# shoeffner/ann3depth

Hardware: AMD Instinct MI355X
Metric: images/sec (640x480->55x74 MSDN train step) (higher is better)
Workload: dtype f32

## Files before the change

ann3depth_amd/_lib.py:

```python
import collections
import ctypes
import os
from ctypes import c_char_p, c_float, c_int, c_int32, c_int64, c_size_t, c_uint8, c_uint32, c_void_p, POINTER

LIB_PATH = os.environ.get('A3D_LIB') or os.path.join(os.path.dirname(os.path.abspath(__file__)), 'liba3d.so')


class A3dError(RuntimeError):
    pass


class ConvDesc(ctypes.Structure):
    _fields_ = [(n, c_int32) for n in ('n', 'h', 'w', 'c', 'k', 'r', 's', 'stride', 'pad_t', 'pad_l', 'ho', 'wo',
                                       'ldx', 'ldy', 'precision', 'storage', 'hints')]


class SecondOutput(ctypes.Structure):
    _fields_ = [('ptr', c_void_p), ('ld', c_int32), ('step', c_int32), ('offset', c_int32), ('bf16', c_int32), ('cols', c_int32)]


class ExampleView(ctypes.Structure):
    _fields_ = [('image_height', c_int64), ('image_width', c_int64), ('image_channels', c_int64),
                ('depth_height', c_int64), ('depth_width', c_int64), ('depth_channels', c_int64),
                ('image', c_void_p), ('image_bytes', c_size_t), ('depth', c_void_p), ('depth_bytes', c_size_t)]
# ... 26 lines not shown
    'a3d_dense_fwd_ws_bytes': (c_size_t, [c_int, c_int, c_int]),
    'a3d_dense_fwd': (c_int, [c_int, c_int, c_int, _P, _P, _P, _P, c_int, _P, _P, c_size_t, _P]),
    'a3d_dense_bwd_data_ws_bytes': (c_size_t, [c_int, c_int, c_int]),
    'a3d_dense_bwd_data': (c_int, [c_int, c_int, c_int, _P, _P, _P, _P, c_int, c_float, _P, c_size_t, _P]),
    'a3d_dense_bwd_filter_ws_bytes': (c_size_t, [c_int, c_int, c_int]),
    'a3d_dense_bwd_filter': (c_int, [c_int, c_int, c_int, _P, _P, _P, _P, _P, c_size_t, _P]),
    'a3d_maxpool2x2_fwd': (c_int, [c_int, c_int, c_int, c_int, _P, _P, c_int, _P, _P]),
    'a3d_maxpool2x2_bwd': (c_int, [c_int, c_int, c_int, c_int, _P, _P, c_int, _P, c_int, _P]),
    'a3d_resize_bilinear_tf1': (c_int, [c_int, c_int, c_int, c_int, _P, c_int, c_int, _P, _P]),
    'a3d_resize_bilinear_tf1_pair': (c_int, [c_int, c_int, c_int, c_int, _P, c_int, c_int, _P, c_int, _P, c_int, c_int, _P, _P]),
    'a3d_resize_bilinear_tf1_ex': (c_int, [c_int, c_int, c_int, c_int, _P, c_int, c_int, c_int, _P, c_int, _P, c_int, c_int, c_int,
                                           _P, _P]),
    'a3d_warp_bilinear_pair': (c_int, [c_int, c_int, c_int, c_int, _P, c_int, c_int, c_int, _P, c_int, _P, c_int, c_int, c_int,
                                       _P, _P, _P]),
    'a3d_extract_patches': (c_int, [c_int, c_int, c_int, c_int, _P, c_int, c_int, _P, _P]),
    'a3d_silog_loss_fwd': (c_int, [c_int, c_int, _P, _P, _P, _P, _P]),
    'a3d_silog_loss_bwd': (c_int, [c_int, c_int, _P, _P, _P, _P, _P]),
    'a3d_dropout_keep_mask': (c_int, [c_size_t, ctypes.c_uint64, ctypes.c_uint64, c_float, _P, _P]),
    'a3d_adam_apply_tf1': (c_int, [c_size_t, _P, _P, _P, _P, c_float, c_float, c_float, c_float, c_float, c_float,
                                   c_float, _P]),
    'a3d_adam_apply_tf1_flag': (c_int, [c_size_t, _P, _P, _P, _P, c_float, c_float, c_float, c_float, c_float, c_float,
                                        c_float, _P, _P]),
    'a3d_dense_fwd_ex': (c_int, [c_int, c_int, c_int, _P, _P, _P, _P, c_int, _P, c_int, c_int, _P, c_size_t, _P]),
    'a3d_dense_bwd_data_ex': (c_int, [c_int, c_int, c_int, _P, _P, _P, _P, c_int, c_float, c_int, c_int, _P, c_size_t, _P]),
    'a3d_dense_fwd_ex2': (c_int, [c_int, c_int, c_int, _P, _P, _P, _P, c_int, c_int, c_int, _P, c_int, c_int, POINTER(SecondOutput), _P,
                                  c_size_t, _P]),
    'a3d_dense_bwd_data_ex2': (c_int, [c_int, c_int, c_int, _P, _P, _P, _P, c_int, c_float, c_int, c_int, POINTER(SecondOutput), _P,
                                       c_size_t, _P]),
    'a3d_conv2d_fwd_ex2': (c_int, [_D, _P, _P, _P, _P, c_int, POINTER(SecondOutput), _P, c_size_t, _P]),
    'a3d_silog_loss_bwd_ex': (c_int, [c_int, c_int, _P, _P, _P, _P, _P, c_int, _P]),
    'a3d_depth_metrics_ws_bytes': (c_size_t, [c_int, c_int, c_int]),
    'a3d_depth_metrics': (c_int, [c_int, c_int, c_int, _P, c_int, c_int, _P, c_int, c_float, c_float, c_float, c_float, _P, _P,
                                  c_size_t, _P]),
    'a3d_cast_bf16': (c_int, [c_size_t, _P, _P, c_int, _P]),
    'a3d_cast_rows': (c_int, [c_size_t, c_int, _P, c_int, c_int, _P, c_int, c_int, _P]),
    'a3d_pad_channels_bf16': (c_int, [c_size_t, c_int, _P, c_int, _P, _P]),
    'a3d_stream_create': (c_int, [c_int, ctypes.POINTER(ctypes.c_void_p)]),
    'a3d_stream_destroy': (c_int, [_P]),
    'a3d_maxpool2x2_fwd_bf16': (c_int, [c_int, c_int, c_int, c_int, _P, c_int, _P, c_int, _P, _P]),
    'a3d_maxpool2x2_bwd_bf16': (c_int, [c_int, c_int, c_int, c_int, _P, c_int, _P, c_int, _P, c_int, _P]),
    'a3d_copy_channel_bf16': (c_int, [c_size_t, _P, c_int, c_int, _P, c_int, c_int, _P]),
    'a3d_maxpool2x2_bwd_idx_bf16': (c_int, [c_int, c_int, c_int, c_int, _P, _P, c_int, _P, c_int, _P, c_int, _P]),
    'a3d_maxpool2x2_bwd_idx_bf16s': (c_int, [c_int, c_int, c_int, c_int, _P, _P, c_int, _P, c_int, _P, c_int, _P]),
    'a3d_dense_bwd_filter_adam_tf1': (c_int, [c_int, c_int, c_int, _P, _P, _P, _P, _P, _P, _P, _P, c_float, c_float, c_float,
                                              c_float, c_float, c_float, _P]),
    'a3d_dense_bwd_filter_adam_tf1_ex': (c_int, [c_int, c_int, c_int, _P, _P, _P, _P, _P, _P, _P, _P, c_float, c_float, c_float,
                                                 c_float, c_float, c_float, c_int, _P]),
    'a3d_superpixel_mean': (c_int, [c_int, c_int, c_int, c_int, _P, c_int, _P, _P]),
    'a3d_superpixel_hist': (c_int, [c_int, c_int, c_int, _P, c_int, _P, _P]),
    'a3d_pair_similarity': (c_int, [c_int, c_int, c_int, _P, c_int, _P, _P, _P, c_int, _P, _P, c_float, _P, _P, _P]),
    'a3d_crf_loss': (c_int, [c_int, c_int, _P, _P, _P, _P, _P, c_int, c_float, _P, _P, _P, _P]),
    'a3d_crf_map': (c_int, [c_int, c_int, _P, _P, _P, _P, c_int, _P, _P, _P]),
    'a3d_sgd_apply': (c_int, [c_size_t, _P, _P, c_float, _P]),
    'a3d_conv2d_pool_fwd': (c_int, [_D, _P, _P, _P, _P, c_int, _P, c_int, _P, c_size_t, _P]),
    'a3d_maxpool2x2_bwd_idx': (c_int, [c_int, c_int, c_int, c_int, _P, _P, c_int, _P, c_int, _P, c_int, _P]),
    'a3d_copy_channel': (c_int, [c_size_t, _P, c_int, c_int, _P, c_int, c_int, _P]),
    'a3d_comm_standin': (c_int, [_P, c_size_t, _P, c_size_t, c_int, c_float, _P]),
    'a3d_timing_enable': (c_int, [c_int]),
    'a3d_timing_collect': (c_int, [POINTER(TimingRecord), c_int]),
    'a3d_timing_select': (c_int, [POINTER(TimingRecord)]),
    'a3d_crc32c': (c_uint32, [_P, c_size_t]),
    'a3d_masked_crc32c': (c_uint32, [_P, c_size_t]),
    'a3d_tfrecord_next': (c_int, [_P, c_size_t, c_int, POINTER(c_size_t), POINTER(c_size_t), POINTER(c_size_t)]),
    'a3d_example_parse': (c_int, [_P, c_size_t, POINTER(ExampleView)]),
    'a3d_decode_raw_plus_half': (c_int, [_P, c_size_t, _P]),
    'a3d_record_decode': (c_int, [_P, c_size_t, c_int, _P, c_size_t, _P, c_size_t, POINTER(ExampleView)]),
    'a3d_record_decode_u8': (c_int, [_P, c_size_t, c_int, _P, _P, c_size_t, _P, _P, c_size_t, POINTER(ExampleView),
                                     POINTER(c_int)]),
    'a3d_records_decode': (c_int, [POINTER(c_void_p), POINTER(c_size_t), c_int, c_int, POINTER(c_int64), _P, _P, _P, _P,
                                   POINTER(c_int32), c_int, POINTER(c_int32)]),
    'a3d_h2d_gather': (c_int, [_P, _P, POINTER(c_int32), c_int, c_int, c_size_t, _P]),
    'a3d_sizeof_conv_desc': (c_size_t, []),
    'a3d_example_write': (c_int64, [_P, c_int, c_int, c_int, _P, c_int, c_int, c_int, _P, c_size_t]),
}

EXT_SIGNATURES = {
    'a3dx_resize_bilinear_tf1_valid': (c_int, [c_int, c_int, c_int, c_int, _P, c_int, c_int, c_int, _P, c_int, _P, c_int, c_int,
                                               c_int, _P, c_float, c_float, _P]),
    'a3dx_warp_bilinear_pair_valid': (c_int, [c_int, c_int, c_int, c_int, _P, c_int, c_int, c_int, _P, c_int, _P, c_int, c_int,
                                              c_int, _P, _P, c_float, c_float, _P]),
    'a3dx_silog_masked_loss_fwd': (c_int, [c_int, c_int, _P, _P, _P, _P, _P]),
    'a3dx_silog_masked_loss_bwd_ex': (c_int, [c_int, c_int, _P, _P, _P, _P, _P, c_int, _P]),
}

PAIR_SIGNATURES = {
    'a3dp_crf_loss_grad': (c_int, [c_int, c_int, _P, _P, _P, _P, _P, c_int, c_float, _P, _P, _P, _P, _P]),
    'a3dp_pair_dense_bwd': (c_int, [c_int, c_int, c_int, _P, _P, _P, _P, _P]),
    'a3dp_sgd_apply_floor': (c_int, [c_size_t, _P, _P, c_float, c_float, _P]),
}

TEXTURE_SIGNATURES = {
    'a3dt_superpixel_lbp_hist': (c_int, [c_int, c_int, c_int, _P, c_int, _P, _P]),
    'a3dt_pair_similarity3': (c_int, [c_int, c_int, c_int, _P, c_int, _P, _P, _P, _P, c_int, _P, _P, c_float, _P, _P, _P]),
}

GRADLOSS_SIGNATURES = {
    'a3dg_silog_grad_loss_fwd': (c_int, [c_int, c_int, c_int, _P, _P, c_int, c_float, _P, _P, _P]),
    'a3dg_silog_grad_loss_bwd_ex': (c_int, [c_int, c_int, c_int, _P, _P, c_int, c_float, _P, _P, _P, c_int, _P]),
}

BERHU_SIGNATURES = {
    'a3dh_berhu_loss_fwd': (c_int, [c_int, c_int, _P, _P, c_int, c_float, _P, _P, _P]),
    'a3dh_berhu_loss_bwd_ex': (c_int, [c_int, c_int, _P, _P, c_int, c_float, _P, _P, _P, c_int, _P]),
}

ALIGN_SIGNATURES = {
    'a3da_depth_align_ws_bytes': (c_size_t, [c_int, c_int, c_int, c_int]),
    'a3da_depth_align': (c_int, [c_int, c_int, c_int, _P, c_int, c_int, _P, c_int, c_float, c_float, c_int, _P, _P, _P, _P,
                                 c_size_t, _P]),
    'a3da_depth_metrics_aligned': (c_int, [c_int, c_int, c_int, _P, c_int, c_int, _P, c_int, c_float, c_float, c_float, c_float,
                                           _P, _P, _P, c_size_t, _P]),
    'a3da_affine_apply': (c_int, [c_int, c_int, _P, _P, _P, _P]),
}

SSI_SIGNATURES = {
    'a3di_ssi_loss_fwd': (c_int, [c_int, c_int, _P, _P, c_int, _P, _P, _P]),
    'a3di_ssi_loss_bwd_ex': (c_int, [c_int, c_int, _P, _P, c_int, _P, _P, _P, c_int, _P]),
}

CRF_VALID_SIGNATURES = {
    'a3dv_superpixel_mean_valid': (c_int, [c_int, c_int, c_int, _P, c_int, c_int, _P, _P, _P]),
    'a3dv_crf_loss_observed': (c_int, [c_int, c_int, _P, _P, _P, _P, _P, c_int, _P, _P, _P, _P, _P, _P, _P]),
}

FCSP_SIGNATURES = {
    'a3df_superpixel_pool_fwd': (c_int, [c_int, c_int, c_int, c_int, _P, c_int, c_int, c_int, c_int, _P, _P, _P, c_int, _P]),
    'a3df_superpixel_pool_bwd': (c_int, [c_int, c_int, c_int, c_int, _P, c_int, c_int, c_int, c_int, _P, _P, _P, c_int, _P]),
}

CRF_BAND_SIGNATURES = {
    'a3db_crf_band_nll': (c_int, [c_int, c_int, c_int, _P, _P, _P, _P, _P, c_int, _P, _P, _P, _P, _P, _P, _P]),
    'a3db_crf_band_map': (c_int, [c_int, c_int, c_int, _P, _P, _P, _P, c_int, _P, _P, _P]),
}

WINO_SIGNATURES = {
    'a3dw_conv2d_bwd_data_prepared_filter_bytes': (c_size_t, [_D]),
    'a3dw_conv2d_bwd_data_prepare_filter': (c_int, [_D, _P, _P, c_size_t, _P]),
}

WINO_GRAD_SIGNATURES = {
    'a3dwg_conv2d_bwd_filter_ws_bytes': (c_size_t, [_D]),
    'a3dwg_conv2d_bwd_filter': (c_int, [_D, _P, _P, _P, _P, _P, c_size_t, _P]),
}

WINO1D_SIGNATURES = {
    'a3dl_conv2d_bwd_data_ws_bytes': (c_size_t, [_D]),
    'a3dl_conv2d_bwd_data': (c_int, [_D, _P, _P, _P, _P, _P, c_size_t, _P]),
    'a3dl_conv2d_bwd_filter_ws_bytes': (c_size_t, [_D]),
    'a3dl_conv2d_bwd_filter': (c_int, [_D, _P, _P, _P, _P, _P, c_size_t, _P]),
    'a3dl_conv2d_bwd_data_prepared_filter_bytes': (c_size_t, [_D]),
    'a3dl_conv2d_bwd_data_prepare_filter': (c_int, [_D, _P, _P, c_size_t, _P]),
}

OPTIM_SIGNATURES = {
    'a3do_momentum_apply': (c_int, [c_size_t, _P, _P, _P, c_float, c_float, c_float, _P]),
    'a3do_dense_bwd_filter_momentum': (c_int, [c_int, c_int, c_int, _P, _P, _P, _P, _P, _P, c_float, c_float, c_float, _P]),
}

CLIP_SIGNATURES = {
    'a3dn_grad_norm_ws_bytes': (c_size_t, [c_size_t]),
    'a3dn_grad_norm_scale': (c_int, [c_size_t, _P, c_float, c_float, _P, _P, c_size_t, _P]),
    'a3dn_momentum_apply_ctl': (c_int, [c_size_t, _P, _P, _P, c_float, c_float, _P, _P]),
    'a3dn_adam_apply_tf1_ctl': (c_int, [c_size_t, _P, _P, _P, _P, c_float, c_float, c_float, c_float, c_float, c_float, _P, _P,
                                        _P]),
    'a3dn_sgd_apply_ctl': (c_int, [c_size_t, _P, _P, c_float, _P, _P]),
    'a3dn_sgd_apply_floor_ctl': (c_int, [c_size_t, _P, _P, c_float, c_float, _P, _P]),
}
CLIP_CTL_BYTES = 32
CLIP_BLOCK_ELEMS, CLIP_MAX_BLOCKS = 4096, 1024


class WinoBwdPool(ctypes.Structure):
    _fields_ = [('argmax', c_void_p), ('y', c_void_p), ('ldy', c_int), ('h2', c_int), ('w2', c_int)]


WINO_BWD_SIGNATURES = {
    'a3dwb_sizeof_pool': (c_size_t, []),
    'a3dwb_conv2d_bwd_ws_bytes': (c_size_t, [_D, c_int, c_int]),
    'a3dwb_conv2d_bwd': (c_int, [_D, _P, _P, _P, _P, _P, _P, _P, ctypes.POINTER(WinoBwdPool), _P, c_size_t, _P]),
}

UPSAMPLE_SIGNATURES = {
    'a3du_joint_bilateral_upsample': (c_int, [c_int, c_int, c_int, _P, c_int, c_int, _P, c_int, _P, _P, _P, _P, c_int, c_float,
                                              c_float, _P, _P]),
}

POSTERIOR_SIGNATURES = {
    'a3dc_crf_band_posterior': (c_int, [c_int, c_int, c_int, _P, _P, _P, _P, _P, c_int, _P, _P, _P, _P, _P]),
}

SLIC_SIGNATURES = {
    'a3ds_label_mean': (c_int, [c_int, c_int, c_int, c_int, _P, c_int, _P, _P, _P, _P]),
    'a3ds_label_hist': (c_int, [c_int, c_int, c_int, _P, c_int, _P, _P, _P]),
    'a3ds_slic_update': (c_int, [c_int, c_int, c_int, _P, c_int, _P, _P, _P, _P]),
    'a3ds_slic_assign': (c_int, [c_int, c_int, c_int, _P, c_int, _P, c_float, _P, _P]),
    'a3ds_slic_segment': (c_int, [c_int, c_int, c_int, _P, c_int, c_int, c_float, _P, _P, _P, _P]),
    'a3ds_pair_similarity': (c_int, [c_int, c_int, _P, _P, _P, _P, _P, c_int, _P, _P, c_float, _P, _P, _P]),
    'a3ds_label_pool_fwd': (c_int, [c_int, c_int, c_int, c_int, _P, c_int, c_int, c_int, c_int, _P, _P, _P, _P, _P, c_int, _P]),
    'a3ds_label_pool_bwd': (c_int, [c_int, c_int, c_int, c_int, _P, c_int, c_int, c_int, c_int, _P, _P, _P, _P, _P, c_int, _P]),
}

Surface = collections.namedtuple('Surface', 'prefix header signatures')
SURFACES = (
    Surface('a3d_', 'a3d.h', SIGNATURES),
    Surface('a3dx_', 'a3d_valid.h', EXT_SIGNATURES),
    Surface('a3dp_', 'a3d_pairwise.h', PAIR_SIGNATURES),
    Surface('a3dt_', 'a3d_texture.h', TEXTURE_SIGNATURES),
    Surface('a3dg_', 'a3d_gradloss.h', GRADLOSS_SIGNATURES),
    Surface('a3dv_', 'a3d_crf_valid.h', CRF_VALID_SIGNATURES),
    Surface('a3df_', 'a3d_fcsp.h', FCSP_SIGNATURES),
    Surface('a3db_', 'a3d_crf_band.h', CRF_BAND_SIGNATURES),
    Surface('a3dw_', 'a3d_wino.h', WINO_SIGNATURES),
    Surface('a3du_', 'a3d_upsample.h', UPSAMPLE_SIGNATURES),
    Surface('a3dc_', 'a3d_posterior.h', POSTERIOR_SIGNATURES),
    Surface('a3dwg_', 'a3d_wino_grad.h', WINO_GRAD_SIGNATURES),
    Surface('a3ds_', 'a3d_slic.h', SLIC_SIGNATURES),
    Surface('a3dwb_', 'a3d_wino_bwd.h', WINO_BWD_SIGNATURES),
    Surface('a3dh_', 'a3d_berhu.h', BERHU_SIGNATURES),
    Surface('a3da_', 'a3d_align.h', ALIGN_SIGNATURES),
    Surface('a3di_', 'a3d_ssi.h', SSI_SIGNATURES),
    Surface('a3dl_', 'a3d_wino1d.h', WINO1D_SIGNATURES),
    Surface('a3do_', 'a3d_optim.h', OPTIM_SIGNATURES),
    Surface('a3dn_', 'a3d_clip.h', CLIP_SIGNATURES),
)

_lib = None


def load():
    global _lib
    if _lib is not None:
        return _lib
    if not os.path.exists(LIB_PATH):
        raise A3dError(f'{LIB_PATH} not found: build it with `python -c "import __graft_entry__ as g; g.build()"` '
                       f'or `make -C ann3depth_amd/csrc` (there is no fallback path)')
    import torch
    lib = ctypes.CDLL(LIB_PATH)
    for name, (res, args) in ((n, sig) for surface in SURFACES for n, sig in surface.signatures.items()):
        try:
            fn = getattr(lib, name)
        except AttributeError as e:
            raise A3dError(f'liba3d.so lacks symbol {name}: stale build?') from e
        fn.restype = res
        fn.argtypes = args
    if lib.a3d_sizeof_conv_desc() != ctypes.sizeof(ConvDesc):
        raise A3dError(f'liba3d.so reads a {lib.a3d_sizeof_conv_desc()}-byte a3d_conv_desc, this binding passes '
                       f'{ctypes.sizeof(ConvDesc)} bytes: stale build?')
    if lib.a3dwb_sizeof_pool() != ctypes.sizeof(WinoBwdPool):
        raise A3dError(f'liba3d.so reads a {lib.a3dwb_sizeof_pool()}-byte a3dwb_pool, this binding passes '
                       f'{ctypes.sizeof(WinoBwdPool)} bytes: stale build?')
    _lib = lib
    return lib


def last_error():
    buf = ctypes.create_string_buffer(512)
    load().a3d_last_error(buf, 512)
    return buf.value.decode(errors='replace')


def check(rc, what):
    if rc != 0:
        raise A3dError(f'{what} failed ({rc}): {last_error()}')
```

ann3depth_amd/csrc/a3d_internal.h:

```cpp
#pragma once
#include <hip/hip_runtime.h>
#include <stddef.h>
#include <stdint.h>

#include <algorithm>

#include "../../include/a3d.h"
#include "igemm_plan.h"

namespace a3d {

int set_error(int code, const char* fmt, ...);

#define A3D_CHECK_ARG(cond, ...)                                 \
  do {                                                           \
    if (!(cond)) return ::a3d::set_error(A3D_EINVAL, __VA_ARGS__); \
  } while (0)

inline void clear_stale_error() { (void)hipGetLastError(); }

inline int check_launch(const char* what) {
  hipError_t e = hipGetLastError();
  if (e != hipSuccess) return set_error(A3D_ELAUNCH, "%s: %s", what, hipGetErrorString(e));
  return A3D_OK;
}

inline unsigned grid_for(size_t total, int per_block = 256, unsigned cap = 8192) {
  size_t g = (total + per_block - 1) / per_block;
  return (unsigned)std::min<size_t>(std::max<size_t>(g, 1), cap);
}

__host__ __device__ inline bool aligned16(const void* p) { return (reinterpret_cast<uintptr_t>(p) & 15) == 0; }

inline size_t up256(size_t b) { return (b + 255) / 256 * 256; }

inline int raise_lds(const void* kern, size_t bytes, bool (&done)[64]) {
  int dev = 0;
  (void)hipGetDevice(&dev);
  if (dev < 0 || dev >= 64 || !done[dev]) {
    hipError_t e = hipFuncSetAttribute(kern, hipFuncAttributeMaxDynamicSharedMemorySize, (int)bytes);
    if (e != hipSuccess) return set_error(A3D_ELAUNCH, "hipFuncSetAttribute: %s", hipGetErrorString(e));
    if (dev >= 0 && dev < 64) done[dev] = true;
  }
  return A3D_OK;
}

struct IgemmParams;
int launch_igemm(int mode, const GemmPlan& plan, int avec, int bvec, IgemmParams& p, void* ws, hipStream_t st);
int take_second_output(IgemmParams& p, const a3d_second_output* o);

struct TimingSlot {
  hipEvent_t start, stop;
  a3d_timing_record rec;
};
bool timing_wanted(const a3d_timing_record& r);
int timing_begin(TimingSlot& slot, hipStream_t st);
void timing_end(TimingSlot& slot, hipStream_t st);
a3d_timing_record timing_record(int mode, int prec, int bm, int bn, int waves_m, int nwaves, int bk, int avec, int bvec, int lds_dma,
                                int m, int n, int k);
template <typename Launch>
int timed_launch(const a3d_timing_record& rec, hipStream_t st, Launch&& launch) {
  if (!timing_wanted(rec)) return launch();
  TimingSlot slot{};
  slot.rec = rec;
  int rc = timing_begin(slot, st);
  if (rc != A3D_OK) return rc;
  rc = launch();
  timing_end(slot, st);
  return rc;
}

bool dense_dw_applicable(int m, int k, int n);
bool dense_stream_applicable(int m, int k, int n);
size_t dense_stream_ws_bytes(int m, int k, int n);
int dense_fwd_stream(int m, int k, int n, const float* x, const float* w, const float* bias, float* y, int act,
                     const uint8_t* keep, float keep_scale, void* ws, size_t ws_bytes, hipStream_t st);
struct ReduceParams;
int launch_splitk_reduce(const ReduceParams& r, hipStream_t st);
int dense_dw_launch(int m, int k, int n, const float* x, const float* dz, float* dw, float* db, hipStream_t st);

size_t colsum_bf16_ws_bytes(int n);
bool colsum_bf16_ok(int n);
int colsum_bf16(const void* dz, int rows, int n, int ld, float* out, void* ws, int* nparts, hipStream_t st);

bool stencil1_applicable(const a3d_conv_desc* d);
size_t stencil1_bwdf_ws_bytes(const a3d_conv_desc* d);
int stencil1_fwd(const a3d_conv_desc* d, const float* x, const float* w, const float* bias, float* y, int act,
                 hipStream_t st);
int stencil1_bwd_filter(const a3d_conv_desc* d, const float* x, const float* dz, float* dw, float* db, void* ws,
                        hipStream_t st);
bool stencil1_bwd_both_applicable(const a3d_conv_desc* d);
size_t stencil1_bwd_both_ws_bytes(const a3d_conv_desc* d);
int stencil1_bwd_both(const a3d_conv_desc* d, const float* x, const float* dz, const float* w, float* dw, float* db,
                      void* dx, int lddx, int dx_bf16, int relu_mask, unsigned* state, void* ws, hipStream_t st);

bool fewch_bwdf_applicable(const a3d_conv_desc* d, bool pooled);
size_t fewch_bwdf_ws_bytes(const a3d_conv_desc* d, bool pooled);
bool fewch_extents_ok(const a3d_conv_desc* d, bool pooled, int ldz, int esz, int ld_arg);
int fewch_bwd_filter(const a3d_conv_desc* d, const float* x, int src, const void* dz, int ldz, const void* pooled_act,
                     const uint8_t* argmax, int ld_arg, float* dw, float* db, void* ws, hipStream_t st);

int fewch_reduce_launch(const float* slabs, int splits, int Mp, int NP, int M, int N, float* dw, float* db, hipStream_t st);
bool fewch16_bwdf_applicable(const a3d_conv_desc* d, bool pooled);
size_t fewch16_bwdf_ws_bytes(const a3d_conv_desc* d, bool pooled);
int fewch16_bwd_filter(const a3d_conv_desc* d, const float* x, bool pooled, const void* dz, int ldz, const void* pooled_act,
                       const uint8_t* argmax, int ld_arg, float* dw, float* db, void* ws, hipStream_t st);

bool conv3_applicable(const a3d_conv_desc* d, unsigned x_off);
size_t conv3_ws_bytes(const a3d_conv_desc* d);
int conv3_pack(const a3d_conv_desc* d, const float* w, float* wp, hipStream_t st);
int conv3_fwd(const a3d_conv_desc* d, const float* x, const float* w, const float* bias, float* y, int act, int pool,
              int ld_out, uint8_t* argmax, void* ws, size_t ws_bytes, hipStream_t st, bool prepared = false);

bool conv3b_applicable(const a3d_conv_desc* d);
size_t conv3b_filter_bytes(const a3d_conv_desc* d);
int conv3b_pack(const a3d_conv_desc* d, const float* w, void* wp, hipStream_t st);
int conv3b_fwd(const a3d_conv_desc* d, const void* x, const float* w, const float* bias, void* y, int act, int pool, int ld_out,
               uint8_t* argmax, void* ws, size_t ws_bytes, hipStream_t st, bool prepared);

struct PlaneBatch;
constexpr int kBM = 128, kBN = 128, kWavesM = 4, kNWaves = 8, kBK = 32;
constexpr int kBlockSlots = 512, kCUs = 256, kMinKTiles = 5;
void plane_tiles(IgemmParams& p, int splits);
int plane_gemm(int mode, int bn, const IgemmParams& p, const PlaneBatch& bt, unsigned blocks, int planes, const char* what, hipStream_t st);
int plane_splits(int planes, int M, int N, size_t pixels, bool larger_on_tie, const char* tuning);

struct WinoGeom {
  int oh, ow, th, tw;
  size_t T;
  int K, N, Kp, Np;
  size_t v_bytes, m_bytes, u_bytes;
  size_t sk_bytes;
};
WinoGeom wino_geom(const a3d_conv_desc* d, bool bwd);
bool wino_applicable(const a3d_conv_desc* d);
int wino_filter(const a3d_conv_desc* d, bool bwd, const float* w, float* U, hipStream_t st);
int wino_input(const a3d_conv_desc* d, bool bwd, const float* src, float* V, hipStream_t st);
int wino_output(const a3d_conv_desc* d, bool bwd, const float* M, float* out, const float* bias, const float* mask, int act,
                hipStream_t st);
a3d_timing_record wino_record(int mode, const WinoGeom& g);
int wino_gemm(IgemmParams& p, const WinoGeom& g, hipStream_t st);

struct WinoGradGeom {
  size_t T;
  int Cp, Kp;
  int splits;
  size_t v_bytes, z_bytes;
  size_t slab_bytes, bias_bytes;
};
int wino_grad_splits(int C, int K, size_t T);
WinoGradGeom wino_grad_geom(const a3d_conv_desc* d);
bool wino_grad_applicable(const a3d_conv_desc* d);
int wino_dz(const a3d_conv_desc* d, const float* dz, float* Z, hipStream_t st);
int wino_dw(const a3d_conv_desc* d, const WinoGradGeom& g, const float* slabs, const float* bparts, float* dw, float* db, hipStream_t st);
a3d_timing_record wino_grad_record(const a3d_conv_desc* d, const WinoGradGeom& g);
int wino_grad_gemm(IgemmParams& p, const WinoGradGeom& g, hipStream_t st);

struct WinoBwdPool {
  const uint8_t* argmax;
  const float* y;
  int ldy, h2, w2;
};
int wino_bwd_transforms(const a3d_conv_desc* d, const float* x, const float* dz, float* Vx, float* Vdz, float* Z, hipStream_t st);
int wino_bwd_gemm(IgemmParams& pf, const WinoGradGeom& gg, IgemmParams& pd, const WinoGeom& g, hipStream_t st);
int wino_bwd_finish(const a3d_conv_desc* d, const WinoGradGeom& gg, const float* slabs, const float* bparts, float* dw, float* db,
                    const float* M, float* dx, const float* mask, const WinoBwdPool* pool, hipStream_t st);

struct Wino1dGeom {
  int R, tw, off;
  size_t Pv, Pm;
  int K, N, Kp, Np;
  int bn, tiles_m, tiles_n, nk, blocks;
  size_t v_bytes, m_bytes, u_bytes;
  size_t sk_bytes;
};
struct Wino1dGradGeom {
  int R, tw;
  size_t Px, Pz;
  int Cp, Kp, splits;
  size_t v_bytes, z_bytes;
  size_t slab_bytes, bias_bytes;
};
int wino1d_bwd_blocks(long tiles, long nk);
int wino1d_grad_splits(int M, int N, size_t pixels);
Wino1dGeom wino1d_geom(const a3d_conv_desc* d);
Wino1dGradGeom wino1d_grad_geom(const a3d_conv_desc* d);
bool wino1d_applicable(const a3d_conv_desc* d);
int wino1d_filter(const a3d_conv_desc* d, const float* w, float* U, hipStream_t st);
int wino1d_input(const float* src, float* V, size_t rows, int W, int c, int ld, int off, int tw, int Cp, hipStream_t st);
int wino1d_dz(const a3d_conv_desc* d, const Wino1dGradGeom& g, const float* dz, float* Z, hipStream_t st);
int wino1d_output(const a3d_conv_desc* d, const Wino1dGeom& g, const float* M, float* dx, const float* mask, hipStream_t st);
int wino1d_dw(const a3d_conv_desc* d, const Wino1dGradGeom& g, const float* slabs, const float* bparts, float* dw, float* db, hipStream_t st);
a3d_timing_record wino1d_record(const Wino1dGeom& g);
a3d_timing_record wino1d_grad_record(const a3d_conv_desc* d, const Wino1dGradGeom& g);
int wino1d_gemm(IgemmParams& p, const Wino1dGeom& g, float* sk, hipStream_t st);
int wino1d_grad_gemm(IgemmParams& p, const Wino1dGradGeom& g, hipStream_t st);

struct Carve {
  uintptr_t at;
  float* take(size_t bytes) {
    float* p = reinterpret_cast<float*>(at);
    at += bytes;
    return p;
  }
};
struct ProductWs { float *U, *V, *M, *sk; };
struct GradWs { float *V, *Z, *slabs, *bparts; };
template <typename Geom>
ProductWs carve_product(Carve& c, const Geom& g, bool prepared) {
  ProductWs w{};
  if (!prepared) w.U = c.take(g.u_bytes);
  w.V = c.take(g.v_bytes);
  w.M = c.take(g.m_bytes);
  w.sk = c.take(g.sk_bytes);
  return w;
}
template <typename Geom>
GradWs carve_grad(Carve& c, const Geom& g) {
  GradWs w{};
  w.V = c.take(g.v_bytes);
  w.Z = c.take(g.z_bytes);
  w.slabs = c.take(g.slab_bytes);
  w.bparts = c.take(g.bias_bytes);
  return w;
}

}
```

ann3depth_amd/csrc/igemm_host.hip:

```cpp
#include <algorithm>
#include <cmath>

#include "../../include/a3d_wino.h"
#include "../../include/a3d_wino_grad.h"
#include "../../include/a3d_wino_bwd.h"
#include "../../include/a3d_wino1d.h"
#include "a3d_internal.h"
#include "igemm.h"
#include "igemm_cfgs.h"

namespace a3d {

int launch_igemm_multi_bwd_d(int avec, int bvec, IgemmMulti& ps, unsigned grid_x, unsigned count, hipStream_t st);
int launch_igemm_bf16_multi_bwd_d(int bn, IgemmMulti& ps, unsigned grid_x, unsigned count, hipStream_t st);


struct RunForm {
  int vec;
  int rl, rlp;
  int kp;
  int np;
  size_t bytes;
};
static bool run_form_ok(const a3d_conv_desc* d, unsigned x_off, RunForm* rf, bool bwd_filter = false) {
  if (d->pad_t || d->pad_l || d->ldx != d->c || d->c % 4 == 0 || d->c > 4) return false;
  const int step = d->stride * d->c, row = d->w * d->c;
  int vec = 0;
  bool anywhere = false;
  if (step % 4 == 0 && row % 4 == 0 && x_off == 0) vec = 4;
  else if (step % 2 == 0 && row % 2 == 0 && (x_off & 7) == 0) vec = 2;
  else if (bwd_filter && d->precision == A3D_PREC_F32 && !d->storage && (x_off & 3) == 0) {
    vec = 2;
    anywhere = true;
  }
  if (vec == 4 && d->precision == A3D_PREC_F32) {
    const int rl = d->s * d->c;
    const int kp4 = d->r * ((rl + 3) / 4 * 4), kp2 = d->r * ((rl + 1) / 2 * 2);
    if ((kp2 + 127) / 128 < (kp4 + 127) / 128) vec = 2;
  }
  if (!vec) return false;
  rf->vec = vec;
  rf->rl = d->s * d->c;
  rf->rlp = (rf->rl + vec - 1) / vec * vec;
  rf->kp = d->r * rf->rlp;
  rf->np = (d->k + 3) / 4 * 4;
  rf->bytes = up256((size_t)rf->kp * rf->np * 4);
  if (anywhere) return (d->wo - 1) * step + rf->rl <= row && (d->ho - 1) * d->stride + d->r <= d->h;
  return (d->wo - 1) * step + rf->rlp <= row;
}

__global__ __launch_bounds__(256) void pad_filter_kernel(const float* w, float* wp, int r, int rl, int rlp, int n, int np) {
  const int total = r * rlp * np;
  for (int i = blockIdx.x * 256 + threadIdx.x; i < total; i += gridDim.x * 256) {
    const int col = i % np, row = i / np;
    const int q = row % rlp, rr = row / rlp;
    wp[i] = (q < rl && col < n) ? w[(size_t)(rr * rl + q) * n + col] : 0.f;
  }
}
__global__ __launch_bounds__(256) void unpad_filter_kernel(const float* wp, float* w, int r, int rl, int rlp, int n) {
  const int total = r * rl * n;
  for (int i = blockIdx.x * 256 + threadIdx.x; i < total; i += gridDim.x * 256) {
    const int col = i % n, row = i / n;
    const int q = row % rl, rr = row / rl;
    w[i] = wp[(size_t)(rr * rlp + q) * n + col];
  }
}

struct Operands {
  bool known = false;
  unsigned x = 0, w = 0, y = 0;
  unsigned aux = 0;
  int act = A3D_ACT_NONE, pool = 0, ld_out = 0;
  bool argmax = false, prepared = false;
  bool db = true;
};
static const Operands kOnGrid{};
static Operands launch_operands(const void* x, const void* w, const void* y, const void* aux) {
  auto off16 = [](const void* p) { return (unsigned)(reinterpret_cast<uintptr_t>(p) & 15); };
  Operands o;
  o.known = true;
  o.x = off16(x); o.w = off16(w); o.y = off16(y); o.aux = off16(aux);
  return o;
}

enum GemmForm { kAsStored, kLdsDma, kRunForm, kBf16Image };
struct Route {
  bool ok = false;
  RunForm rf{};
  GemmProblem g{};
  GemmPlan plan{};
  size_t repack = 0;
  size_t bytes = 0;
};
static size_t upto(size_t need, const Route& r) { return r.ok ? std::max(need, r.bytes) : need; }
static void fit_workspace(Route& r, const Operands& o, size_t ws_bytes, size_t per_split = 0) {
  if (r.bytes <= ws_bytes || !(o.x | o.w | o.y | o.aux) || r.repack > ws_bytes) return;
  r.plan = plan_within(r.g, r.plan, ws_bytes - r.repack, per_split);
  r.bytes = r.repack + r.plan.ws_bytes + (r.plan.splitk > 1 ? (size_t)r.plan.splitk * per_split : 0);
}
#define A3D_CHECK_WS(ws, who) A3D_CHECK_ARG(aligned16(ws), who ": ws must be 16-byte aligned")

static const int kAll16 = A3D_STORE_X_BF16 | A3D_STORE_W_BF16 | A3D_STORE_Y_BF16;
static bool stored16(const a3d_conv_desc* d, int bits) { return (d->storage & bits) == bits; }
static bool ring_ok(const a3d_conv_desc* d, const Operands& o, int both, unsigned out_off, int taps) {
  if (d->precision != A3D_PREC_BF16 || !stored16(d, both) || d->c % 8 || d->k % 8) return false;
  return !o.known || (d->ldx % 8 == 0 && d->ldy % 8 == 0 && taps <= 128 && !out_off);
}

static int ilog2_exact(int v) {
  for (int l = 0; l < 8; ++l)
    if ((1 << l) == v) return l;
  return -1;
}

static int check_desc(const a3d_conv_desc* d) {
  A3D_CHECK_ARG(d != nullptr, "conv: null descriptor");
  A3D_CHECK_ARG(d->n > 0 && d->h > 0 && d->w > 0 && d->c > 0 && d->k > 0 && d->r > 0 && d->s > 0, "conv: bad dims");
  A3D_CHECK_ARG(ilog2_exact(d->stride) >= 0 && d->stride <= 4, "conv: stride %d unsupported (1, 2 or 4)", d->stride);
  A3D_CHECK_ARG(d->pad_t >= 0 && d->pad_l >= 0 && d->pad_t < d->r && d->pad_l < d->s, "conv: bad padding");
  A3D_CHECK_ARG(d->ho > 0 && d->wo > 0, "conv: bad output size");
  A3D_CHECK_ARG((d->ho - 1) * d->stride - d->pad_t < d->h && (d->wo - 1) * d->stride - d->pad_l < d->w,
                "conv: output size inconsistent with input");
  A3D_CHECK_ARG(d->ldx >= d->c && d->ldy >= d->k, "conv: pixel strides smaller than channel counts");
  A3D_CHECK_ARG(d->precision >= A3D_PREC_F32 && d->precision <= A3D_PREC_F32_WINOGRAD, "conv: unknown precision %d", d->precision);
  const double lim = 2147483647.0;
  A3D_CHECK_ARG((double)d->n * d->h * d->w * d->ldx < lim && (double)d->n * d->ho * d->wo * d->ldy < lim &&
                    (double)d->r * d->s * d->c * d->k < lim,
                "conv: tensor too large for 31-bit indexing");
  auto tile_span_ok = [&](double rows_per_image, double image_elems) {
    const double images = std::min((double)d->n, std::floor(255.0 / rows_per_image) + 2.0);
    return images * image_elems * 4.0 < lim;
  };
  A3D_CHECK_ARG(tile_span_ok((double)d->ho * d->wo, (double)d->h * d->w * d->ldx) &&
                    tile_span_ok(std::max(1.0, std::floor((double)d->h / d->stride) * std::floor((double)d->w / d->stride)),
                                 (double)d->ho * d->wo * d->ldy),
                "conv: single images too large for 31-bit byte offsets inside a tile");
  return A3D_OK;
}

#define A3D_AS_F32(d)                                          \
  a3d_conv_desc d##_f32;                                       \
  if ((d) && (d)->precision == A3D_PREC_F32_WINOGRAD) {        \
    d##_f32 = *(d);                                            \
    d##_f32.precision = A3D_PREC_F32;                          \
    (d) = &d##_f32;                                            \
  }

static GemmProblem fwd_problem(const a3d_conv_desc* d) {
  GemmProblem g;
  g.mode = MODE_FWD;
  g.M = d->n * d->ho * d->wo; g.N = d->k; g.K = d->r * d->s * d->c;
  g.avec = (d->c % 4 == 0 && d->ldx % 4 == 0) ? 4 : 1;
  g.bvec = (d->k % 4 == 0) ? 4 : 1;
  return g;
}
static GemmProblem bwd_d_problem(const a3d_conv_desc* d) {
  GemmProblem g;
  g.mode = MODE_BWD_D;
  g.M = d->n * d->h * d->w; g.N = d->c; g.K = d->r * d->s * d->k;
// ... 723 lines not shown
  if (rc != A3D_OK) return rc;
  IgemmParams p = wino_grad_product(g, at.V, at.Z, at.slabs, db ? at.bparts : nullptr);
  rc = timed_launch(wino_grad_record(d, g), st, [&] { return wino_grad_gemm(p, g, st); });
  if (rc != A3D_OK) return rc;
  return wino_dw(d, g, at.slabs, at.bparts, dw, db, st);
}

static bool wino_bwd_takes(const a3d_conv_desc* d) {
  if (!wino_grad_takes(d)) return false;
  const WinoGeom gx = wino_geom(d, false), gd = wino_geom(d, true);
  return gx.th <= gd.th && gx.tw <= gd.tw;
}
static a3d_conv_desc as_winograd(const a3d_conv_desc* d) {
  a3d_conv_desc e = *d;
  e.precision = A3D_PREC_F32_WINOGRAD;
  return e;
}

size_t a3dwb_sizeof_pool(void) { return sizeof(a3dwb_pool); }

size_t a3dwb_conv2d_bwd_ws_bytes(const a3d_conv_desc* d, int w_prepared, int pooled) {
  (void)pooled;
  if (!wino_bwd_takes(d)) return std::max(a3dwg_conv2d_bwd_filter_ws_bytes(d), a3d_conv2d_bwd_data_ws_bytes(d));
  const a3d_conv_desc e = as_winograd(d);
  Carve c{0};
  carve_product(c, wino_geom(&e, true), w_prepared != 0);
  carve_grad(c, wino_grad_geom(&e));
  return c.at;
}

int a3dwb_conv2d_bwd(const a3d_conv_desc* d, const float* x, const float* dz, const float* w_or_U, float* dw, float* db, float* dx,
                     const float* relu_mask, const a3dwb_pool* pool, void* ws, size_t ws_bytes, void* stream) {
  static_assert(sizeof(WinoBwdPool) == sizeof(a3dwb_pool), "WinoBwdPool mirrors a3dwb_pool");
  if (!wino_bwd_takes(d)) {
    A3D_CHECK_ARG(!pool, "conv2d_bwd (Winograd): a pool only where the Winograd routes take the descriptor");
    const int rc = a3dwg_conv2d_bwd_filter(d, x, dz, dw, db, ws, ws_bytes, stream);
    return rc != A3D_OK ? rc : a3d_conv2d_bwd_data(d, dz, w_or_U, dx, relu_mask, ws, ws_bytes, stream);
  }
  A3D_CHECK_ARG(x && dz && w_or_U && dw && dx, "conv2d_bwd (Winograd): null tensor");
  A3D_CHECK_WS(ws, "conv2d_bwd (Winograd)");
  A3D_CHECK_ARG(!(pool && relu_mask), "conv2d_bwd (Winograd): relu_mask and pool exclude each other");
  A3D_CHECK_ARG(!pool || (pool->argmax && pool->y && pool->ldy >= d->c && pool->h2 >= 2 && pool->w2 >= 2 && pool->h2 / 2 == d->h &&
                          pool->w2 / 2 == d->w),
                "conv2d_bwd (Winograd): the pool's halved extents must be the layer's input's");
  const a3d_conv_desc e = as_winograd(d);
  const bool prepared = (d->hints & A3D_HINT_W_PREPARED) != 0;
  const WinoGeom g = wino_geom(&e, true);
  const WinoGradGeom gg = wino_grad_geom(&e);
  Carve c{reinterpret_cast<uintptr_t>(ws)};
  const ProductWs ad = carve_product(c, g, prepared);
  const GradWs af = carve_grad(c, gg);
  const size_t need = c.at - reinterpret_cast<uintptr_t>(ws);
  if (!ws || need > ws_bytes) return set_error(A3D_EWORKSPACE, "conv2d_bwd (Winograd): need %zu workspace bytes", need);
  hipStream_t st = static_cast<hipStream_t>(stream);
  const float* U;
  int rc = transformed_filter("conv2d_bwd (Winograd)", prepared, w_or_U, ad.U, U, [&](float* u) { return wino_filter(&e, true, w_or_U, u, st); });
  if (rc != A3D_OK) return rc;
  rc = wino_bwd_transforms(&e, x, dz, af.V, ad.V, af.Z, st);
  if (rc != A3D_OK) return rc;
  IgemmParams pf = wino_grad_product(gg, af.V, af.Z, af.slabs, db ? af.bparts : nullptr);
  IgemmParams pd = wino_product(g, ad.V, U, ad.M);
  const a3d_timing_record rf = wino_grad_record(&e, gg), rd = wino_record(MODE_BWD_D, g);
  if (timing_wanted(rf) || timing_wanted(rd) || tune_int("A3D_WINO_BWD_PAIR", 1) == 0) {
    rc = timed_launch(rf, st, [&] { return wino_grad_gemm(pf, gg, st); });
    if (rc != A3D_OK) return rc;
    rc = timed_launch(rd, st, [&] { return wino_gemm(pd, g, st); });
  } else {
    rc = wino_bwd_gemm(pf, gg, pd, g, st);
  }
  if (rc != A3D_OK) return rc;
  WinoBwdPool wp{};
  if (pool) wp = WinoBwdPool{pool->argmax, pool->y, pool->ldy, pool->h2, pool->w2};
  return wino_bwd_finish(&e, gg, af.slabs, af.bparts, dw, db, ad.M, dx, relu_mask, pool ? &wp : nullptr, st);
}

static bool wino1d_takes(const a3d_conv_desc* d) { return check_desc(d) == A3D_OK && wino1d_applicable(d); }

static IgemmParams wino1d_product(const a3d_conv_desc* d, const Wino1dGeom& g, const float* V, const float* U, float* M) {
  return plane_product(MODE_FWD, plane_desc(d->n, d->ho, g.tw, d->h, g.Kp, g.Np, g.R, g.R - 1 - d->pad_t), V, U, M, nullptr,
                       (unsigned long long)g.Pv * g.Kp, (unsigned long long)g.R * g.Kp * g.Np, g.R);
}
static IgemmParams wino1d_grad_product(const a3d_conv_desc* d, const Wino1dGradGeom& g, const float* V, const float* Z, float* slabs,
                                       float* bparts) {
  return plane_product(MODE_BWD_F, plane_desc(d->n, d->h, g.tw, d->ho, g.Cp, g.Kp, g.R, d->pad_t), V, Z, slabs, bparts,
                       (unsigned long long)g.Px * g.Cp, (unsigned long long)g.Pz * g.Kp, g.R);
}

size_t a3dl_conv2d_bwd_data_ws_bytes(const a3d_conv_desc* d) {
  if (!wino1d_takes(d)) return a3d_conv2d_bwd_data_ws_bytes(d);
  return product_ws_bytes(wino1d_geom(d), (d->hints & A3D_HINT_W_PREPARED) != 0);
}

int a3dl_conv2d_bwd_data(const a3d_conv_desc* d, const float* dz, const float* w, float* dx, const float* relu_mask, void* ws,
                         size_t ws_bytes, void* stream) {
  if (!wino1d_takes(d)) return a3d_conv2d_bwd_data(d, dz, w, dx, relu_mask, ws, ws_bytes, stream);
  A3D_CHECK_ARG(dz && w && dx, "conv2d_bwd_data (Winograd 1-D): null tensor");
  A3D_CHECK_WS(ws, "conv2d_bwd_data (Winograd 1-D)");
  const bool prepared = (d->hints & A3D_HINT_W_PREPARED) != 0;
  const Wino1dGeom g = wino1d_geom(d);
  Carve c{reinterpret_cast<uintptr_t>(ws)};
  const ProductWs at = carve_product(c, g, prepared);
  const size_t need = c.at - reinterpret_cast<uintptr_t>(ws);
  if (!ws || need > ws_bytes) return set_error(A3D_EWORKSPACE, "conv2d_bwd_data (Winograd 1-D): need %zu workspace bytes", need);
  hipStream_t st = static_cast<hipStream_t>(stream);
  const float* U;
  int rc = transformed_filter("conv2d_bwd_data (Winograd 1-D)", prepared, w, at.U, U, [&](float* u) { return wino1d_filter(d, w, u, st); });
  if (rc != A3D_OK) return rc;
  rc = wino1d_input(dz, at.V, (size_t)d->n * d->ho, d->wo, d->k, d->ldy, g.off, g.tw, g.Kp, st);
  if (rc != A3D_OK) return rc;
  IgemmParams p = wino1d_product(d, g, at.V, U, at.M);
  rc = timed_launch(wino1d_record(g), st, [&] { return wino1d_gemm(p, g, at.sk, st); });
  if (rc != A3D_OK) return rc;
  return wino1d_output(d, g, at.M, dx, relu_mask, st);
}

size_t a3dl_conv2d_bwd_filter_ws_bytes(const a3d_conv_desc* d) {
  if (!wino1d_takes(d)) return a3d_conv2d_bwd_filter_ws_bytes(d);
  return grad_ws_bytes(wino1d_grad_geom(d));
}

int a3dl_conv2d_bwd_filter(const a3d_conv_desc* d, const float* x, const float* dz, float* dw, float* db, void* ws, size_t ws_bytes,
                           void* stream) {
  if (!wino1d_takes(d)) return a3d_conv2d_bwd_filter(d, x, dz, dw, db, ws, ws_bytes, stream);
  A3D_CHECK_ARG(x && dz && dw, "conv2d_bwd_filter (Winograd 1-D): null tensor");
  A3D_CHECK_WS(ws, "conv2d_bwd_filter (Winograd 1-D)");
  const Wino1dGradGeom g = wino1d_grad_geom(d);
  Carve c{reinterpret_cast<uintptr_t>(ws)};
  const GradWs at = carve_grad(c, g);
  const size_t need = c.at - reinterpret_cast<uintptr_t>(ws);
  if (!ws || need > ws_bytes) return set_error(A3D_EWORKSPACE, "conv2d_bwd_filter (Winograd 1-D): need %zu workspace bytes", need);
  hipStream_t st = static_cast<hipStream_t>(stream);
  int rc = wino1d_input(x, at.V, (size_t)d->n * d->h, d->w, d->c, d->ldx, d->pad_l, g.tw, g.Cp, st);
  if (rc != A3D_OK) return rc;
  rc = wino1d_dz(d, g, dz, at.Z, st);
  if (rc != A3D_OK) return rc;
  IgemmParams p = wino1d_grad_product(d, g, at.V, at.Z, at.slabs, db ? at.bparts : nullptr);
  rc = timed_launch(wino1d_grad_record(d, g), st, [&] { return wino1d_grad_gemm(p, g, st); });
  if (rc != A3D_OK) return rc;
  return wino1d_dw(d, g, at.slabs, at.bparts, dw, db, st);
}

size_t a3dl_conv2d_bwd_data_prepared_filter_bytes(const a3d_conv_desc* d) { return wino1d_takes(d) ? wino1d_geom(d).u_bytes : 0; }

int a3dl_conv2d_bwd_data_prepare_filter(const a3d_conv_desc* d, const float* w, void* prepared, size_t prepared_bytes, void* stream) {
  int rc = check_desc(d);
  if (rc != A3D_OK) return rc;
  A3D_CHECK_ARG(w && prepared && aligned16(prepared), "conv2d_bwd_data_prepare_filter (Winograd 1-D): null or misaligned buffer");
  const size_t need = a3dl_conv2d_bwd_data_prepared_filter_bytes(d);
  A3D_CHECK_ARG(need > 0, "conv2d_bwd_data_prepare_filter (Winograd 1-D): the route does not take this descriptor");
  if (prepared_bytes < need) return set_error(A3D_EWORKSPACE, "conv2d_bwd_data_prepare_filter (Winograd 1-D): need %zu bytes", need);
  return wino1d_filter(d, w, static_cast<float*>(prepared), static_cast<hipStream_t>(stream));
}

static a3d_conv_desc dense_desc(int m, int k, int n) {
  a3d_conv_desc d{};
  d.n = m; d.h = 1; d.w = 1; d.c = k; d.k = n; d.r = 1; d.s = 1; d.stride = 1; d.ho = 1; d.wo = 1;
  d.ldx = k; d.ldy = n;
  return d;
}

size_t a3d_dense_fwd_ws_bytes(int m, int k, int n) {
  a3d_conv_desc d = dense_desc(m, k, n);
  if (check_desc(&d) != A3D_OK) return 0;
  return std::max(plan_gemm(fwd_problem(&d), A3D_PREC_F32).ws_bytes, dense_stream_ws_bytes(m, k, n));
}

int a3d_dense_fwd(int m, int k, int n, const float* x, const float* w, const float* bias, float* y, int act,
                  const uint8_t* drop_keep, void* ws, size_t ws_bytes, void* stream) {
  return a3d_dense_fwd_ex(m, k, n, x, w, bias, y, act, drop_keep, A3D_PREC_F32, 0, ws, ws_bytes, stream);
}

int a3d_dense_fwd_ex(int m, int k, int n, const float* x, const float* w, const float* bias, float* y, int act,
                     const uint8_t* drop_keep, int precision, int storage, void* ws, size_t ws_bytes, void* stream) {
  return a3d_dense_fwd_ex2(m, k, n, x, w, bias, y, n, n, act, drop_keep, precision, storage, nullptr, ws, ws_bytes, stream);
}

int a3d_dense_fwd_ex2(int m, int k, int n, const float* x, const float* w, const float* bias, float* y, int ldy, int ncols_y, int act,
                      const uint8_t* drop_keep, int precision, int storage, const a3d_second_output* out2, void* ws,
                      size_t ws_bytes, void* stream) {
  A3D_CHECK_ARG(m > 0 && k > 0 && n > 0, "dense_fwd: bad dims");
  A3D_CHECK_ARG(ncols_y > 0 && ncols_y <= n && ldy >= ncols_y, "dense_fwd: y rows of %d columns at pitch %d from a GEMM of %d", ncols_y, ldy, n);
  A3D_CHECK_ARG((storage & ~(A3D_STORE_W_BF16 | A3D_STORE_X_BF16)) == 0, "dense_fwd: the weights and x may be bf16, y is float32");
  if (precision == A3D_PREC_F32_WINOGRAD) precision = A3D_PREC_F32;
  a3d_conv_desc d = dense_desc(m, k, n);
  d.precision = precision;
  int rc = check_desc(&d);
  if (rc != A3D_OK) return rc;
  A3D_CHECK_ARG(x && w && y, "dense_fwd: null tensor");
  A3D_CHECK_WS(ws, "dense_fwd");
  if (precision == A3D_PREC_F32 && !storage && dense_stream_applicable(m, k, n) && aligned16(x) && !out2 && ldy == n && ncols_y == n &&
      !tune_int("A3D_NO_DENSE_KERNELS", 0))
    return dense_fwd_stream(m, k, n, x, w, bias, y, act, drop_keep, 2.f, ws, ws_bytes, static_cast<hipStream_t>(stream));
  GemmProblem g = fwd_problem(&d);
  if (!aligned16(x)) g.avec = 1;
  if (!aligned16(w)) g.bvec = 1;
  IgemmParams p;
  fill_common(p, g);
  rc = apply_storage(p, precision, storage & A3D_STORE_X_BF16, storage & A3D_STORE_W_BF16, false, k, k, n, n, x, w, y, "x", "w", "y");
  if (rc != A3D_OK) return rc;
  A3D_CHECK_ARG(!p.a16 || aligned16(y), "dense_fwd: beside a bf16 x, y must be 16-byte aligned (the LDS-DMA kernel alone reads a bf16 x)");
  storage_vecs(g, p.a16, p.b16, p.c16);
  g.ring_ok = p.a16 && p.b16 && precision == A3D_PREC_BF16 && k % 8 == 0 && n % 8 == 0 && aligned16(y) && act != A3D_ACT_SIGMOID;
  g.need_reduce = ncols_y != n;
  GemmPlan plan = plan_gemm(g, precision);
  if (!aligned16(x) || !aligned16(w) || !aligned16(y)) plan = plan_within(g, plan, ws ? ws_bytes : 0, 0);
  A3D_CHECK_ARG(!storage || plan.prec == A3D_PREC_BF16, "dense_fwd: bf16 weights need vectorisable operands");
  A3D_CHECK_ARG(!p.a16 || plan.ring, "dense_fwd: a bf16 x is taken by the LDS-DMA kernel only (bf16 weights, k and n multiples of 8)");
  if (plan.ws_bytes > ws_bytes) return set_error(A3D_EWORKSPACE, "dense_fwd: need %zu workspace bytes", plan.ws_bytes);
  p.A = x; p.B = w; p.C = y; p.bias = bias; p.act = act; p.keep = drop_keep; p.mask_scale = 2.f;
  p.npix = m; p.nrsc = k;
  fill_gather(p, &d, k, 1, k);
  p.ldb = n; p.ldc = ldy; p.c_cols = ncols_y == n ? 0 : ncols_y;
  rc = take_second_output(p, out2);
  if (rc != A3D_OK) return rc;
  fill_staging(p, MODE_FWD, (unsigned long long)m * k, (unsigned long long)k * n, 1, 1);
  return launch_igemm(MODE_FWD, plan, g.avec, g.bvec, p, ws, static_cast<hipStream_t>(stream));
}

size_t a3d_dense_bwd_data_ws_bytes(int m, int k, int n) {
  a3d_conv_desc d = dense_desc(m, k, n);
  return a3d_conv2d_bwd_data_ws_bytes(&d);
}

int a3d_dense_bwd_data(int m, int k, int n, const float* dz, const float* w, float* dx, const float* mask,
                       int mask_act, float scale, void* ws, size_t ws_bytes, void* stream) {
  return a3d_dense_bwd_data_ex(m, k, n, dz, w, dx, mask, mask_act, scale, A3D_PREC_F32, 0, ws, ws_bytes, stream);
}

int a3d_dense_bwd_data_ex(int m, int k, int n, const float* dz, const float* w, float* dx, const float* mask, int mask_act,
                          float scale, int precision, int storage, void* ws, size_t ws_bytes, void* stream) {
  return a3d_dense_bwd_data_ex2(m, k, n, dz, w, dx, mask, mask_act, scale, precision, storage, nullptr, ws, ws_bytes, stream);
}

int a3d_dense_bwd_data_ex2(int m, int k, int n, const float* dz, const float* w, float* dx, const float* mask, int mask_act,
                           float scale, int precision, int storage, const a3d_second_output* out2, void* ws, size_t ws_bytes,
                           void* stream) {
  A3D_CHECK_ARG(m > 0 && k > 0 && n > 0, "dense_bwd_data: bad dims");
  if (precision == A3D_PREC_F32_WINOGRAD) precision = A3D_PREC_F32;
  A3D_CHECK_ARG(precision >= A3D_PREC_F32 && precision <= A3D_PREC_BF16, "dense_bwd_data: unknown precision %d", precision);
  A3D_CHECK_ARG(!mask || mask_act == A3D_ACT_RELU || mask_act == A3D_ACT_SIGMOID, "dense_bwd_data: bad mask_act");
  a3d_conv_desc d = dense_desc(m, k, n);
  int rc = check_desc(&d);
  if (rc != A3D_OK) return rc;
  A3D_CHECK_ARG(dz && w && dx, "dense_bwd_data: null tensor");
  A3D_CHECK_WS(ws, "dense_bwd_data");
  GemmProblem g = bwd_d_problem(&d);
  if (!aligned16(dz)) g.avec = 1;
  if (!aligned16(w)) g.bvec = 1;
  IgemmParams p;
  fill_common(p, g);
  rc = apply_storage(p, precision, storage & A3D_STORE_Y_BF16, storage & A3D_STORE_W_BF16, storage & A3D_STORE_X_BF16, n, n, n, n, dz, w,
                     dx, "dz", "w", "dx");
  if (rc != A3D_OK) return rc;
  A3D_CHECK_ARG(!p.c16 || aligned16(mask), "dense_bwd_data: bf16 mask must be 16-byte aligned");
  storage_vecs(g, p.a16, p.b16, p.c16);
  g.ring_ok = p.a16 && p.b16 && precision == A3D_PREC_BF16 && k % 8 == 0 && n % 8 == 0 && aligned16(dx) &&
              (!mask || (aligned16(mask) && mask_act == A3D_ACT_RELU));
  GemmPlan plan = plan_gemm(g, precision);
  if (!aligned16(dz) || !aligned16(w) || !aligned16(dx) || !aligned16(mask)) plan = plan_within(g, plan, ws ? ws_bytes : 0, 0);
  A3D_CHECK_ARG(!storage || plan.prec == A3D_PREC_BF16, "dense_bwd_data: bf16 weights need vectorisable operands");
  A3D_CHECK_ARG(!(p.a16 || p.c16) || plan.ring, "dense_bwd_data: bf16 dz / dx are taken by the LDS-DMA kernel only (bf16 weights, k and n multiples of 8, ReLU mask)");
  if (plan.ws_bytes > ws_bytes) return set_error(A3D_EWORKSPACE, "dense_bwd_data: need %zu workspace bytes", plan.ws_bytes);
  p.A = dz; p.B = w; p.C = dx; p.mask = mask; p.mask_scale = scale; p.mask_act = mask_act;
  p.npix = m; p.nrsc = n;
  fill_gather(p, &d, n, 1, n);
  p.Cn = k;
  p.ldc = k;
  p.S_full = 1;
  rc = take_second_output(p, out2);
  if (rc != A3D_OK) return rc;
  fill_staging(p, MODE_BWD_D, (unsigned long long)m * n, (unsigned long long)k * n, 1, 1);
  return launch_igemm(MODE_BWD_D, plan, g.avec, g.bvec, p, ws, static_cast<hipStream_t>(stream));
}

size_t a3d_dense_bwd_filter_ws_bytes(int m, int k, int n) {
  a3d_conv_desc d = dense_desc(m, k, n);
  return a3d_conv2d_bwd_filter_ws_bytes(&d);
}

int a3d_dense_bwd_filter(int m, int k, int n, const float* x, const float* dz, float* dw, float* db, void* ws,
                         size_t ws_bytes, void* stream) {
  A3D_CHECK_ARG(m > 0 && k > 0 && n > 0, "dense_bwd_filter: bad dims");
  A3D_CHECK_WS(ws, "dense_bwd_filter");
  if (dense_dw_applicable(m, k, n) && (long)k * n >= (1L << 16) && !tune_int("A3D_NO_DENSE_KERNELS", 0)) {
    A3D_CHECK_ARG(x && dz && dw, "dense_bwd_filter: null tensor");
    return dense_dw_launch(m, k, n, x, dz, dw, db, static_cast<hipStream_t>(stream));
  }
  a3d_conv_desc d = dense_desc(m, k, n);
  return a3d_conv2d_bwd_filter(&d, x, dz, dw, db, ws, ws_bytes, stream);
}

}
```

ann3depth_amd/csrc/wino.hip:

```cpp
#include "a3d_internal.h"
#include "igemm.h"
#include "igemm_cfgs.h"

namespace a3d {

typedef float f4 __attribute__((ext_vector_type(4)));

__global__ __launch_bounds__(256) void wino_filter_kernel(const float* w, float* U, int c, int k, int Rp, int Cp, int bwd) {
  const int total = Rp * Cp;
  for (int i = blockIdx.x * 256 + threadIdx.x; i < total; i += gridDim.x * 256) {
    const int col = i % Cp, row = i / Cp;
    const int rows = bwd ? k : c, cols = bwd ? c : k;
    float g[3][3];
#pragma unroll
    for (int r = 0; r < 3; ++r)
#pragma unroll
      for (int s = 0; s < 3; ++s) {
        float v = 0.f;
        if (row < rows && col < cols)
          v = bwd ? w[((size_t)((2 - r) * 3 + (2 - s)) * c + col) * k + row] : w[((size_t)(r * 3 + s) * c + row) * k + col];
        g[r][s] = v;
      }
    float t[4][3];
#pragma unroll
    for (int s = 0; s < 3; ++s) {
      const float a = g[0][s] + g[2][s];
      t[0][s] = g[0][s];
      t[1][s] = (a + g[1][s]) * 0.5f;
      t[2][s] = (a - g[1][s]) * 0.5f;
      t[3][s] = g[2][s];
    }
#pragma unroll
    for (int a4 = 0; a4 < 4; ++a4) {
      const float a = t[a4][0] + t[a4][2];
      const float u[4] = {t[a4][0], (a + t[a4][1]) * 0.5f, (a - t[a4][1]) * 0.5f, t[a4][2]};
#pragma unroll
      for (int b4 = 0; b4 < 4; ++b4) U[(size_t)(a4 * 4 + b4) * total + i] = u[b4];
    }
  }
}


template <bool VEC>
__device__ __forceinline__ void wino_load_window(const float* __restrict__ x, f4 (&d)[4][4], size_t img, int y0, int x0, int h, int w, int c,
                                                 int ld, int cq) {
#pragma unroll
  for (int a = 0; a < 4; ++a)
#pragma unroll
    for (int b = 0; b < 4; ++b) {
      f4 v = f4(0.f);
      const int yy = y0 + a, xx = x0 + b;
      if (yy >= 0 && yy < h && xx >= 0 && xx < w) {
        const float* src = x + ((img * h + yy) * w + xx) * (size_t)ld + cq * 4;
        if (VEC) {
          v = *reinterpret_cast<const f4*>(src);
        } else {
#pragma unroll
          for (int e = 0; e < 4; ++e)
            if (cq * 4 + e < c) v[e] = src[e];
        }
      }
      d[a][b] = v;
    }
}

__device__ __forceinline__ void wino_input_store(const f4 (&d)[4][4], float* __restrict__ V, size_t T, size_t t, int Cp, int cq) {
  f4 r[4][4];
#pragma unroll
  for (int b = 0; b < 4; ++b) {
    r[0][b] = d[0][b] - d[2][b];
    r[1][b] = d[1][b] + d[2][b];
    r[2][b] = d[2][b] - d[1][b];
    r[3][b] = d[1][b] - d[3][b];
  }
#pragma unroll
  for (int a = 0; a < 4; ++a) {
    const f4 v[4] = {r[a][0] - r[a][2], r[a][1] + r[a][2], r[a][2] - r[a][1], r[a][1] - r[a][3]};
#pragma unroll
    for (int b = 0; b < 4; ++b) *reinterpret_cast<f4*>(V + ((size_t)(a * 4 + b) * T + t) * Cp + cq * 4) = v[b];
  }
}

template <bool VEC>
__global__ __launch_bounds__(256) void wino_input_kernel(const float* __restrict__ x, float* __restrict__ V, int h, int w, int c, int ld,
                                                         int th, int tw, int pad_t, int pad_l, int Cp, size_t T) {
  const int cqn = Cp / 4;
  const size_t total = T * (size_t)cqn;
  for (size_t i = (size_t)blockIdx.x * 256 + threadIdx.x; i < total; i += (size_t)gridDim.x * 256) {
    const int cq = (int)(i % cqn);
    const size_t t = i / cqn;
    const int tj = (int)(t % tw), ti = (int)((t / tw) % th);
    const size_t img = t / ((size_t)tw * th);
    f4 d[4][4];
    wino_load_window<VEC>(x, d, img, 2 * ti - pad_t, 2 * tj - pad_l, h, w, c, ld, cq);
    wino_input_store(d, V, T, t, Cp, cq);
  }
}

__device__ __forceinline__ void wino_output_rows(const float* __restrict__ M, f4 (&r)[2][4], size_t T, size_t t, int Np, int cq) {
  f4 m[4][4];
#pragma unroll
  for (int a = 0; a < 4; ++a)
#pragma unroll
    for (int b = 0; b < 4; ++b) m[a][b] = *reinterpret_cast<const f4*>(M + ((size_t)(a * 4 + b) * T + t) * Np + cq * 4);
#pragma unroll
  for (int b = 0; b < 4; ++b) {
    r[0][b] = (m[0][b] + m[1][b]) + m[2][b];
    r[1][b] = (m[1][b] - m[2][b]) - m[3][b];
  }
}

template <bool VEC>
__global__ __launch_bounds__(256) void wino_output_kernel(const float* __restrict__ M, float* __restrict__ out, const float* __restrict__ bias,
                                                          const float* __restrict__ mask, int act, int oh, int ow, int ncols, int ld,
                                                          int th, int tw, int Np, size_t T) {
  const int cqn = Np / 4;
  const size_t total = T * (size_t)cqn;
  for (size_t i = (size_t)blockIdx.x * 256 + threadIdx.x; i < total; i += (size_t)gridDim.x * 256) {
    const int cq = (int)(i % cqn);
    const size_t t = i / cqn;
    const int tj = (int)(t % tw), ti = (int)((t / tw) % th);
    const size_t img = t / ((size_t)tw * th);
    f4 r[2][4];
    wino_output_rows(M, r, T, t, Np, cq);
    f4 bv = f4(0.f);
    if (bias) {
#pragma unroll
      for (int e = 0; e < 4; ++e)
        if (cq * 4 + e < ncols) bv[e] = bias[cq * 4 + e];
    }
#pragma unroll
    for (int a = 0; a < 2; ++a) {
      const f4 y2[2] = {(r[a][0] + r[a][1]) + r[a][2], (r[a][1] - r[a][2]) - r[a][3]};
#pragma unroll
      for (int b = 0; b < 2; ++b) {
        const int oy = 2 * ti + a, ox = 2 * tj + b;
        if (oy >= oh || ox >= ow) continue;
        const size_t o = ((img * oh + oy) * ow + ox) * (size_t)ld + cq * 4;
        f4 v = y2[b] + bv;
        if (act == EPI_RELU) {
#pragma unroll
          for (int e = 0; e < 4; ++e) v[e] = fmaxf(v[e], 0.f);
        } else if (act == EPI_SIGMOID) {
#pragma unroll
          for (int e = 0; e < 4; ++e) v[e] = 1.f / (1.f + expf(-v[e]));
        }
        if (VEC) {
          if (mask) {
            const f4 y = *reinterpret_cast<const f4*>(mask + o);
#pragma unroll
            for (int e = 0; e < 4; ++e) v[e] = apply_act_grad(v[e], y[e], EPI_RELU, 1.f);
          }
          *reinterpret_cast<f4*>(out + o) = v;
        } else {
#pragma unroll
          for (int e = 0; e < 4; ++e)
            if (cq * 4 + e < ncols) out[o + e] = mask ? apply_act_grad(v[e], mask[o + e], EPI_RELU, 1.f) : v[e];
        }
      }
    }
  }
}

template <int MODE, int BN, int WAVES_M, int NWAVES>
__global__ __launch_bounds__(64 * NWAVES, 2 * NWAVES / 4) void plane_gemm_kernel(const IgemmParams p, const PlaneBatch bt) {
  igemm_body<MODE, kBM, BN, WAVES_M, NWAVES, kBK, 4, 4>(plane_params(p, bt, blockIdx.y), gridDim.x, blockIdx.x);
}

template <int MODE, int BN, int WAVES_M, int NWAVES>
static int plane_gemm_as(const IgemmParams& p, const PlaneBatch& bt, unsigned blocks, int planes, const char* what, hipStream_t st) {
  using Cfg = IgemmCfg<MODE, kBM, BN, WAVES_M, NWAVES, kBK, 4, 4>;
  static bool attr_done[64] = {};
  const int rc = raise_lds(reinterpret_cast<const void*>(plane_gemm_kernel<MODE, BN, WAVES_M, NWAVES>), Cfg::LDS_BYTES, attr_done);
  if (rc != A3D_OK) return rc;
  clear_stale_error();
  hipLaunchKernelGGL((plane_gemm_kernel<MODE, BN, WAVES_M, NWAVES>), dim3(blocks, (unsigned)planes), dim3(Cfg::NT), Cfg::LDS_BYTES, st, p, bt);
  return check_launch(what);
}

int plane_gemm(int mode, int bn, const IgemmParams& p, const PlaneBatch& bt, unsigned blocks, int planes, const char* what, hipStream_t st) {
  if (mode == MODE_BWD_F) return plane_gemm_as<MODE_BWD_F, kBN, kWavesM, kNWaves>(p, bt, blocks, planes, what, st);
  if (bn == 96) return plane_gemm_as<MODE_FWD, 96, 4, 4>(p, bt, blocks, planes, what, st);
  return plane_gemm_as<MODE_FWD, kBN, kWavesM, kNWaves>(p, bt, blocks, planes, what, st);
}

void plane_tiles(IgemmParams& p, int splits) {
  const int nk = (p.K + kBK - 1) / kBK;
  p.splitk = splits;
  p.ktiles_per_split = (nk + splits - 1) / splits;
  p.tiles_m = (p.M + kBM - 1) / kBM;
  p.tiles_n = (p.N + kBN - 1) / kBN;
  p.slab = (size_t)p.M * p.N;
}

int plane_splits(int planes, int M, int N, size_t pixels, bool larger_on_tie, const char* tuning) {
  const long blocks1 = (long)planes * ((M + kBM - 1) / kBM) * ((N + kBN - 1) / kBN);
  const long nk = (long)((pixels + kBK - 1) / kBK);
  const long smax = std::max(1L, std::min(kBlockSlots / blocks1, nk / kMinKTiles));
  long s = 1, load = (blocks1 + kCUs - 1) / kCUs;
  for (long t = 2; t <= smax; ++t) {
    const long l = (blocks1 * t + kCUs - 1) / kCUs;
    if (l * s < load * t || (larger_on_tie && l * s == load * t)) { s = t; load = l; }
  }
  const int forced = tune_int(tuning, 0);
  if (forced > 0) s = std::min((long)forced, nk);
  const long per = (nk + s - 1) / s;
  return (int)((nk + per - 1) / per);
}

constexpr int kWinoPlanes = 16;
static PlaneBatch wino_batch(const WinoGeom& g) { return {g.T * (size_t)g.Kp, (size_t)g.Kp * g.Np, g.T * (size_t)g.Np, 0, -1}; }
static PlaneBatch wino_grad_batch(const WinoGradGeom& g) {
  return {g.T * (size_t)g.Cp, g.T * (size_t)g.Kp, (size_t)g.splits * g.Cp * g.Kp, 0, 1 * 4 + 1};
}

WinoGeom wino_geom(const a3d_conv_desc* d, bool bwd) {
  WinoGeom g{};
  g.oh = bwd ? d->h : d->ho;
  g.ow = bwd ? d->w : d->wo;
  g.th = (g.oh + 1) / 2;
  g.tw = (g.ow + 1) / 2;
  g.T = (size_t)d->n * g.th * g.tw;
  g.K = bwd ? d->k : d->c;
  g.N = bwd ? d->c : d->k;
  g.Kp = (g.K + 3) / 4 * 4;
  g.Np = (g.N + 3) / 4 * 4;
  g.v_bytes = up256((size_t)16 * g.T * g.Kp * 4);
  g.m_bytes = up256((size_t)16 * g.T * g.Np * 4);
  g.u_bytes = up256((size_t)16 * g.Kp * g.Np * 4);
  return g;
}

bool wino_applicable(const a3d_conv_desc* d) {
  if (d->precision != A3D_PREC_F32_WINOGRAD || d->storage || d->r != 3 || d->s != 3 || d->stride != 1 || d->pad_t > 1 || d->pad_l > 1)
    return false;
  for (bool bwd : {false, true}) {
    const WinoGeom g = wino_geom(d, bwd);
    if ((double)g.T * std::max(g.Kp, g.Np) * 4.0 >= 2147483647.0 || g.T >= ((size_t)1 << 30)) return false;
  }
  return true;
}

int wino_filter(const a3d_conv_desc* d, bool bwd, const float* w, float* U, hipStream_t st) {
  const WinoGeom g = wino_geom(d, bwd);
  clear_stale_error();
  hipLaunchKernelGGL(wino_filter_kernel, dim3(grid_for((size_t)g.Kp * g.Np)), dim3(256), 0, st, w, U, d->c, d->k, g.Kp, g.Np, bwd ? 1 : 0);
  return check_launch("wino_filter");
}

int wino_input(const a3d_conv_desc* d, bool bwd, const float* src, float* V, hipStream_t st) {
  const WinoGeom g = wino_geom(d, bwd);
  const int h = bwd ? d->ho : d->h, w = bwd ? d->wo : d->w, ld = bwd ? d->ldy : d->ldx;
  const int pad_t = bwd ? 2 - d->pad_t : d->pad_t, pad_l = bwd ? 2 - d->pad_l : d->pad_l;
  const bool vec = g.K % 4 == 0 && ld % 4 == 0 && aligned16(src);
  const dim3 grid(grid_for(g.T * (size_t)(g.Kp / 4), 256, 1u << 20)), block(256);
  clear_stale_error();
  if (vec) hipLaunchKernelGGL(wino_input_kernel<true>, grid, block, 0, st, src, V, h, w, g.K, ld, g.th, g.tw, pad_t, pad_l, g.Kp, g.T);
  else hipLaunchKernelGGL(wino_input_kernel<false>, grid, block, 0, st, src, V, h, w, g.K, ld, g.th, g.tw, pad_t, pad_l, g.Kp, g.T);
  return check_launch("wino_input");
}

int wino_output(const a3d_conv_desc* d, bool bwd, const float* M, float* out, const float* bias, const float* mask, int act,
                hipStream_t st) {
  const WinoGeom g = wino_geom(d, bwd);
  const int ld = bwd ? d->ldx : d->ldy;
  const bool vec = g.N % 4 == 0 && ld % 4 == 0 && aligned16(out) && aligned16(mask);
  const dim3 grid(grid_for(g.T * (size_t)(g.Np / 4), 256, 1u << 20)), block(256);
  clear_stale_error();
  if (vec) hipLaunchKernelGGL(wino_output_kernel<true>, grid, block, 0, st, M, out, bias, mask, act, g.oh, g.ow, g.N, ld, g.th, g.tw, g.Np, g.T);
  else hipLaunchKernelGGL(wino_output_kernel<false>, grid, block, 0, st, M, out, bias, mask, act, g.oh, g.ow, g.N, ld, g.th, g.tw, g.Np, g.T);
  return check_launch("wino_output");
}

a3d_timing_record wino_record(int mode, const WinoGeom& g) {
  return timing_record(mode, A3D_PREC_F32, kBM, kBN, kWavesM, kNWaves, kBK, 4, 4, 0, (int)(16 * g.T), g.N, g.K);
}

int wino_gemm(IgemmParams& p, const WinoGeom& g, hipStream_t st) {
  plane_tiles(p, 1);
  return plane_gemm(MODE_FWD, kBN, p, wino_batch(g), (unsigned)(p.tiles_m * p.tiles_n), kWinoPlanes, "wino_gemm", st);
}



__device__ __forceinline__ void wino_dz_store(const f4 (&y)[2][2], float* __restrict__ Z, size_t T, size_t t, int Kp, int cq) {
  const f4 r[4][2] = {{y[0][0], y[0][1]}, {y[0][0] + y[1][0], y[0][1] + y[1][1]}, {y[0][0] - y[1][0], y[0][1] - y[1][1]},
                      {-y[1][0], -y[1][1]}};
#pragma unroll
  for (int a = 0; a < 4; ++a) {
    const f4 z[4] = {r[a][0], r[a][0] + r[a][1], r[a][0] - r[a][1], -r[a][1]};
#pragma unroll
    for (int b = 0; b < 4; ++b) *reinterpret_cast<f4*>(Z + ((size_t)(a * 4 + b) * T + t) * Kp + cq * 4) = z[b];
  }
}

template <bool VEC>
__global__ __launch_bounds__(256) void wino_dz_kernel(const float* __restrict__ dz, float* __restrict__ Z, int ho, int wo, int k, int ld,
                                                      int th, int tw, int Kp, size_t T) {
  const int cqn = Kp / 4;
  const size_t total = T * (size_t)cqn;
  for (size_t i = (size_t)blockIdx.x * 256 + threadIdx.x; i < total; i += (size_t)gridDim.x * 256) {
    const int cq = (int)(i % cqn);
    const size_t t = i / cqn;
    const int tj = (int)(t % tw), ti = (int)((t / tw) % th);
    const size_t img = t / ((size_t)tw * th);
    f4 y[2][2];
#pragma unroll
    for (int a = 0; a < 2; ++a)
#pragma unroll
      for (int b = 0; b < 2; ++b) {
        f4 v = f4(0.f);
        const int yy = 2 * ti + a, xx = 2 * tj + b;
        if (yy < ho && xx < wo) {
          const float* src = dz + ((img * ho + yy) * wo + xx) * (size_t)ld + cq * 4;
          if (VEC) {
            v = *reinterpret_cast<const f4*>(src);
          } else {
#pragma unroll
            for (int e = 0; e < 4; ++e)
              if (cq * 4 + e < k) v[e] = src[e];
          }
        }
        y[a][b] = v;
      }
    wino_dz_store(y, Z, T, t, Kp, cq);
  }
}

__device__ __forceinline__ void wino_dw_item(size_t i, const float* __restrict__ slabs, const float* __restrict__ bparts, float* __restrict__ dw,
                                             float* __restrict__ db, int c, int k, int Cp, int Kp, int splits) {
  const size_t plane = (size_t)Cp * Kp;
  const int col = (int)(i % k), row = (int)(i / k);
  const size_t at = (size_t)row * Kp + col;
  float m[4][4];
#pragma unroll
  for (int xi = 0; xi < 16; ++xi) m[xi / 4][xi % 4] = slabs[(size_t)xi * splits * plane + at];
  for (int z = 1; z < splits; ++z) {
    float v[16];
#pragma unroll
    for (int xi = 0; xi < 16; ++xi) v[xi] = slabs[((size_t)xi * splits + z) * plane + at];
#pragma unroll
    for (int xi = 0; xi < 16; ++xi) m[xi / 4][xi % 4] += v[xi];
  }
  float t[3][4];
#pragma unroll
  for (int b = 0; b < 4; ++b) {
    const float hs = (m[1][b] + m[2][b]) * 0.5f;
    t[0][b] = m[0][b] + hs;
    t[1][b] = (m[1][b] - m[2][b]) * 0.5f;
// ... 289 lines not shown
```

ann3depth_amd/csrc/wino1d.hip:

```cpp
#include "a3d_internal.h"
#include "igemm.h"
#include "igemm_cfgs.h"
#include "wino1d_mats.h"

namespace a3d {

typedef float f4 __attribute__((ext_vector_type(4)));

template <typename C, int ROWS, int COLS, const C (&Mx)[ROWS][COLS], bool TR, int J, int L, typename T>
__device__ __forceinline__ void w1_dot(const T (&in)[TR ? ROWS : COLS], T& acc) {
  if constexpr (L < (TR ? ROWS : COLS)) {
    constexpr C c = TR ? Mx[L][J] : Mx[J][L];
    if constexpr (c != C(0)) acc += c * in[L];
    w1_dot<C, ROWS, COLS, Mx, TR, J, L + 1, T>(in, acc);
  }
}
template <typename C, int ROWS, int COLS, const C (&Mx)[ROWS][COLS], bool TR, typename T, int J = 0>
__device__ __forceinline__ void w1_apply(const T (&in)[TR ? ROWS : COLS], T (&out)[TR ? COLS : ROWS]) {
  if constexpr (J < (TR ? COLS : ROWS)) {
    T acc = T(0);
    w1_dot<C, ROWS, COLS, Mx, TR, J, 0, T>(in, acc);
    out[J] = acc;
    w1_apply<C, ROWS, COLS, Mx, TR, T, J + 1>(in, out);
  }
}

__global__ __launch_bounds__(256) void wino1d_filter_kernel(const float* __restrict__ w, float* __restrict__ U, int c, int k, int R, int Kp,
                                                            int Np) {
  const size_t plane = (size_t)R * Kp * Np;
  for (size_t i = (size_t)blockIdx.x * 256 + threadIdx.x; i < plane; i += (size_t)gridDim.x * 256) {
    const int col = (int)(i % Np), row = (int)((i / Np) % Kp), r = (int)(i / ((size_t)Np * Kp));
    float g[5], u[8];
#pragma unroll
    for (int s = 0; s < 5; ++s) g[s] = (row < k && col < c) ? w[((size_t)((R - 1 - r) * 5 + (4 - s)) * c + col) * k + row] : 0.f;
    w1_apply<float, 8, 5, kW1G, false, float>(g, u);
#pragma unroll
    for (int xi = 0; xi < 8; ++xi) U[(size_t)xi * plane + i] = u[xi];
  }
}

template <bool VEC>
__global__ __launch_bounds__(256) void wino1d_input_kernel(const float* __restrict__ src, float* __restrict__ V, int W, int c, int ld, int off,
                                                           int tw, int Cp, size_t P) {
  const int cqn = Cp / 4;
  const size_t total = P * (size_t)cqn;
  for (size_t i = (size_t)blockIdx.x * 256 + threadIdx.x; i < total; i += (size_t)gridDim.x * 256) {
    const int cq = (int)(i % cqn);
    const size_t pix = i / cqn, row = pix / tw;
    const int x0 = 4 * (int)(pix % tw) - off;
    f4 d[8], v[8];
#pragma unroll
    for (int b = 0; b < 8; ++b) {
      f4 t = f4(0.f);
      const int xx = x0 + b;
      if (xx >= 0 && xx < W) {
        const float* s = src + (row * W + xx) * (size_t)ld + cq * 4;
        if (VEC) {
          t = *reinterpret_cast<const f4*>(s);
        } else {
#pragma unroll
          for (int e = 0; e < 4; ++e)
            if (cq * 4 + e < c) t[e] = s[e];
        }
      }
      d[b] = t;
    }
    w1_apply<float, 8, 8, kW1BT, false, f4>(d, v);
#pragma unroll
    for (int xi = 0; xi < 8; ++xi) *reinterpret_cast<f4*>(V + ((size_t)xi * P + pix) * Cp + cq * 4) = v[xi];
  }
}

template <bool VEC>
__global__ __launch_bounds__(256) void wino1d_dz_kernel(const float* __restrict__ dz, float* __restrict__ Z, int wo, int k, int ld, int tw, int Kp,
                                                        size_t P) {
  const int cqn = Kp / 4;
  const size_t total = P * (size_t)cqn;
  for (size_t i = (size_t)blockIdx.x * 256 + threadIdx.x; i < total; i += (size_t)gridDim.x * 256) {
    const int cq = (int)(i % cqn);
    const size_t pix = i / cqn, row = pix / tw;
    const int x0 = 4 * (int)(pix % tw);
    f4 y[4], z[8];
#pragma unroll
    for (int b = 0; b < 4; ++b) {
      f4 t = f4(0.f);
      if (x0 + b < wo) {
        const float* s = dz + (row * wo + x0 + b) * (size_t)ld + cq * 4;
        if (VEC) {
          t = *reinterpret_cast<const f4*>(s);
        } else {
#pragma unroll
          for (int e = 0; e < 4; ++e)
            if (cq * 4 + e < k) t[e] = s[e];
        }
      }
      y[b] = t;
    }
    w1_apply<float, 4, 8, kW1AT, true, f4>(y, z);
#pragma unroll
    for (int xi = 0; xi < 8; ++xi) *reinterpret_cast<f4*>(Z + ((size_t)xi * P + pix) * Kp + cq * 4) = z[xi];
  }
}

template <bool VEC>
__global__ __launch_bounds__(256) void wino1d_output_kernel(const float* __restrict__ M, float* __restrict__ out, const float* __restrict__ mask,
                                                            int w, int ncols, int ld, int tw, int Np, size_t P) {
  const int cqn = Np / 4;
  const size_t total = P * (size_t)cqn;
  for (size_t i = (size_t)blockIdx.x * 256 + threadIdx.x; i < total; i += (size_t)gridDim.x * 256) {
    const int cq = (int)(i % cqn);
    const size_t pix = i / cqn, row = pix / tw;
    const int x0 = 4 * (int)(pix % tw);
    f4 m[8], y[4];
#pragma unroll
    for (int xi = 0; xi < 8; ++xi) m[xi] = *reinterpret_cast<const f4*>(M + ((size_t)xi * P + pix) * Np + cq * 4);
    w1_apply<float, 4, 8, kW1AT, false, f4>(m, y);
#pragma unroll
    for (int b = 0; b < 4; ++b) {
      if (x0 + b >= w) continue;
      const size_t o = (row * w + x0 + b) * (size_t)ld + cq * 4;
      f4 v = y[b];
      if (VEC) {
        if (mask) {
          const f4 a = *reinterpret_cast<const f4*>(mask + o);
#pragma unroll
          for (int e = 0; e < 4; ++e) v[e] = apply_act_grad(v[e], a[e], EPI_RELU, 1.f);
        }
        *reinterpret_cast<f4*>(out + o) = v;
      } else {
#pragma unroll
        for (int e = 0; e < 4; ++e)
          if (cq * 4 + e < ncols) out[o + e] = mask ? apply_act_grad(v[e], mask[o + e], EPI_RELU, 1.f) : v[e];
      }
    }
  }
}

__global__ __launch_bounds__(256) void wino1d_dw_kernel(const float* __restrict__ slabs, const float* __restrict__ bparts, float* __restrict__ dw,
                                                        float* __restrict__ db, int c, int k, int R, int Cp, int Kp, int splits) {
  const size_t total = (size_t)R * c * k, plane = (size_t)R * Cp * Kp;
  for (size_t i = (size_t)blockIdx.x * 256 + threadIdx.x; i < total; i += (size_t)gridDim.x * 256) {
    const int col = (int)(i % k), row = (int)((i / k) % c), r = (int)(i / ((size_t)k * c));
    const size_t at = ((size_t)r * Cp + row) * Kp + col;
    double m[8], g[5];
#pragma unroll
    for (int xi = 0; xi < 8; ++xi) m[xi] = (double)slabs[(size_t)xi * splits * plane + at];
    for (int z = 1; z < splits; ++z) {
      float v[8];
#pragma unroll
      for (int xi = 0; xi < 8; ++xi) v[xi] = slabs[((size_t)xi * splits + z) * plane + at];
#pragma unroll
      for (int xi = 0; xi < 8; ++xi) m[xi] += (double)v[xi];
    }
    w1_apply<double, 8, 5, kW1Gd, true, double>(m, g);
#pragma unroll
    for (int s = 0; s < 5; ++s) dw[((size_t)(r * 5 + s) * c + row) * k + col] = (float)g[s];
    if (db && r == 0 && row == 0) {
      float s = bparts[col];
      for (int z = 1; z < splits; ++z) s += bparts[(size_t)z * Kp + col];
      db[col] = s;
    }
  }
}

constexpr int kPlanes = 8;
static PlaneBatch wino1d_batch(const Wino1dGeom& g) {
  return {g.Pv * (size_t)g.Kp, (size_t)g.R * g.Kp * g.Np, g.Pm * (size_t)g.Np, (size_t)2 * g.blocks * 128 * g.bn, -1};
}
static PlaneBatch wino1d_grad_batch(const Wino1dGradGeom& g) {
  return {g.Px * (size_t)g.Cp, g.Pz * (size_t)g.Kp, (size_t)g.splits * g.R * g.Cp * g.Kp, 0, 1};
}

template <int BN, int WAVES_M, int NWAVES>
__global__ __launch_bounds__(256) void wino1d_fixup_kernel(const IgemmParams p, const uint32_t nblk, const PlaneBatch bt) {
  igemm_fixup_body<MODE_FWD, kBM, BN, WAVES_M, NWAVES>(plane_params(p, bt, blockIdx.z), nblk, blockIdx.x, blockIdx.y);
}

constexpr int kMinShare = 4;
int wino1d_bwd_blocks(long tiles, long nk) {
  long b = std::max(1L, std::min((long)(kBlockSlots / kPlanes), tiles * nk / kMinShare));
  const int forced = tune_int("A3D_WINO1D_BLOCKS", 0);
  if (forced > 0) b = std::min((long)forced, std::min(tiles * nk, 128L));
  return (int)b;
}

int wino1d_grad_splits(int M, int N, size_t pixels) { return plane_splits(kPlanes, M, N, pixels, true, "A3D_WINO1D_GRAD_SPLIT"); }

Wino1dGeom wino1d_geom(const a3d_conv_desc* d) {
  Wino1dGeom g{};
  g.R = d->r;
  g.tw = (d->w + 3) / 4;
  g.off = 4 - d->pad_l;
  g.Pv = (size_t)d->n * d->ho * g.tw;
  g.Pm = (size_t)d->n * d->h * g.tw;
  g.K = d->k; g.N = d->c;
  g.Kp = (g.K + 3) / 4 * 4;
  g.Np = (g.N + 3) / 4 * 4;
  g.bn = g.Np <= 96 ? 96 : 128;
  g.tiles_m = (int)((g.Pm + 127) / 128);
  g.tiles_n = (g.Np + g.bn - 1) / g.bn;
  g.nk = (g.R * g.Kp + kBK - 1) / kBK;
  g.blocks = wino1d_bwd_blocks((long)g.tiles_m * g.tiles_n, g.nk);
  g.v_bytes = up256((size_t)kPlanes * g.Pv * g.Kp * 4);
  g.m_bytes = up256((size_t)kPlanes * g.Pm * g.Np * 4);
  g.u_bytes = up256((size_t)kPlanes * g.R * g.Kp * g.Np * 4);
  g.sk_bytes = up256((size_t)kPlanes * 2 * g.blocks * 128 * g.bn * 4);
  return g;
}

Wino1dGradGeom wino1d_grad_geom(const a3d_conv_desc* d) {
  Wino1dGradGeom g{};
  g.R = d->r;
  g.tw = (d->wo + 3) / 4;
  g.Px = (size_t)d->n * d->h * g.tw;
  g.Pz = (size_t)d->n * d->ho * g.tw;
  g.Cp = (d->c + 3) / 4 * 4;
  g.Kp = (d->k + 3) / 4 * 4;
  g.splits = wino1d_grad_splits(g.R * g.Cp, g.Kp, g.Pz);
  g.v_bytes = up256((size_t)kPlanes * g.Px * g.Cp * 4);
  g.z_bytes = up256((size_t)kPlanes * g.Pz * g.Kp * 4);
  g.slab_bytes = up256((size_t)kPlanes * g.splits * g.R * g.Cp * g.Kp * 4);
  g.bias_bytes = up256((size_t)g.splits * g.Kp * 4);
  return g;
}

bool wino1d_applicable(const a3d_conv_desc* d) {
  if (d->precision != A3D_PREC_F32 || d->storage || d->s != 5 || d->stride != 1 || d->pad_l > 4) return false;
  const Wino1dGeom g = wino1d_geom(d);
  const Wino1dGradGeom gg = wino1d_grad_geom(d);
  const double lim = 2147483647.0;
  for (double bytes : {(double)g.Pv * g.Kp, (double)g.Pm * g.Np, (double)g.R * g.Kp * g.Np, (double)gg.Px * gg.Cp, (double)gg.Pz * gg.Kp,
                       (double)g.R * gg.Cp * gg.Kp})
    if (bytes * 4.0 >= lim) return false;
  return true;
}

int wino1d_filter(const a3d_conv_desc* d, const float* w, float* U, hipStream_t st) {
  const Wino1dGeom g = wino1d_geom(d);
  clear_stale_error();
  hipLaunchKernelGGL(wino1d_filter_kernel, dim3(grid_for((size_t)g.R * g.Kp * g.Np)), dim3(256), 0, st, w, U, d->c, d->k, g.R, g.Kp, g.Np);
  return check_launch("wino1d_filter");
}

int wino1d_input(const float* src, float* V, size_t rows, int W, int c, int ld, int off, int tw, int Cp, hipStream_t st) {
  const size_t P = rows * tw;
  const bool vec = c % 4 == 0 && ld % 4 == 0 && aligned16(src);
  const dim3 grid(grid_for(P * (size_t)(Cp / 4), 256, 1u << 20)), block(256);
  clear_stale_error();
  if (vec) hipLaunchKernelGGL(wino1d_input_kernel<true>, grid, block, 0, st, src, V, W, c, ld, off, tw, Cp, P);
  else hipLaunchKernelGGL(wino1d_input_kernel<false>, grid, block, 0, st, src, V, W, c, ld, off, tw, Cp, P);
  return check_launch("wino1d_input");
}

int wino1d_dz(const a3d_conv_desc* d, const Wino1dGradGeom& g, const float* dz, float* Z, hipStream_t st) {
  const bool vec = d->k % 4 == 0 && d->ldy % 4 == 0 && aligned16(dz);
  const dim3 grid(grid_for(g.Pz * (size_t)(g.Kp / 4), 256, 1u << 20)), block(256);
  clear_stale_error();
  if (vec) hipLaunchKernelGGL(wino1d_dz_kernel<true>, grid, block, 0, st, dz, Z, d->wo, d->k, d->ldy, g.tw, g.Kp, g.Pz);
  else hipLaunchKernelGGL(wino1d_dz_kernel<false>, grid, block, 0, st, dz, Z, d->wo, d->k, d->ldy, g.tw, g.Kp, g.Pz);
  return check_launch("wino1d_dz");
}

int wino1d_output(const a3d_conv_desc* d, const Wino1dGeom& g, const float* M, float* dx, const float* mask, hipStream_t st) {
  const bool vec = g.N % 4 == 0 && d->ldx % 4 == 0 && aligned16(dx) && aligned16(mask);
  const dim3 grid(grid_for(g.Pm * (size_t)(g.Np / 4), 256, 1u << 20)), block(256);
  clear_stale_error();
  if (vec) hipLaunchKernelGGL(wino1d_output_kernel<true>, grid, block, 0, st, M, dx, mask, d->w, g.N, d->ldx, g.tw, g.Np, g.Pm);
  else hipLaunchKernelGGL(wino1d_output_kernel<false>, grid, block, 0, st, M, dx, mask, d->w, g.N, d->ldx, g.tw, g.Np, g.Pm);
  return check_launch("wino1d_output");
}

int wino1d_dw(const a3d_conv_desc* d, const Wino1dGradGeom& g, const float* slabs, const float* bparts, float* dw, float* db, hipStream_t st) {
  clear_stale_error();
  hipLaunchKernelGGL(wino1d_dw_kernel, dim3(grid_for((size_t)g.R * d->c * d->k, 256, 1u << 20)), dim3(256), 0, st, slabs, bparts, dw, db, d->c,
                     d->k, g.R, g.Cp, g.Kp, g.splits);
  return check_launch("wino1d_dw");
}

a3d_timing_record wino1d_record(const Wino1dGeom& g) {
  return timing_record(MODE_BWD_D, A3D_PREC_F32, 128, g.bn, 4, g.bn == 96 ? 4 : 8, kBK, 4, 4, 0, (int)(kPlanes * g.Pm), g.N, g.R * g.K);
}
a3d_timing_record wino1d_grad_record(const a3d_conv_desc* d, const Wino1dGradGeom& g) {
  a3d_timing_record r = timing_record(MODE_BWD_F, A3D_PREC_F32, kBM, kBN, kWavesM, kNWaves, kBK, 4, 4, 0, g.R * d->c, d->k, (int)(kPlanes * g.Pz));
  r.splitk = g.splits;
  return r;
}

int wino1d_gemm(IgemmParams& p, const Wino1dGeom& g, float* sk, hipStream_t st) {
  p.splitk = 1;
  p.ktiles_per_split = g.nk;
  p.tiles_m = g.tiles_m;
  p.tiles_n = g.tiles_n;
  p.slab = (size_t)p.M * p.N;
  p.streamk = 1;
  p.sk_ws = sk;
  p.div_nk = make_fastdiv((uint32_t)g.nk);
  const PlaneBatch bt = wino1d_batch(g);
  const int rc = plane_gemm(MODE_FWD, g.bn, p, bt, (unsigned)g.blocks, kPlanes, "wino1d_gemm", st);
  if (rc != A3D_OK) return rc;
  const dim3 grid((unsigned)(g.tiles_m * g.tiles_n), (128 * g.bn / 256 + 3) / 4, kPlanes);
  if (g.bn == 96) hipLaunchKernelGGL((wino1d_fixup_kernel<96, 4, 4>), grid, dim3(256), 0, st, p, (uint32_t)g.blocks, bt);
  else hipLaunchKernelGGL((wino1d_fixup_kernel<kBN, kWavesM, kNWaves>), grid, dim3(256), 0, st, p, (uint32_t)g.blocks, bt);
  return check_launch("wino1d_fixup");
}

int wino1d_grad_gemm(IgemmParams& p, const Wino1dGradGeom& g, hipStream_t st) {
  plane_tiles(p, g.splits);
  return plane_gemm(MODE_BWD_F, kBN, p, wino1d_grad_batch(g), (unsigned)(p.tiles_m * p.tiles_n * p.splitk), kPlanes, "wino1d_grad_gemm", st);
}

}
```

ann3depth_amd/models.py:

```python
import collections
import contextlib
import ctypes
import math
import os

import numpy as np
import torch

from . import _lib, augment as augment_, ops
from ._lib import ConvDesc
from .feed import DeviceFeed

NET_H, NET_W = 228, 304
OUT_H, OUT_W = 55, 74
SAMPLES_COARSE = 2000000
SAMPLES_FINE = 1500000

ConvSpec = collections.namedtuple('ConvSpec', 'name cin cout k stride padding relu')

MSDN_CONVS = [
    ConvSpec('coarse/conv/conv2d_0', 3, 96, 11, 4, 'VALID', True),
    ConvSpec('coarse/conv/conv2d_1', 96, 256, 5, 1, 'SAME', True),
    ConvSpec('coarse/conv/conv2d_2', 256, 384, 3, 1, 'SAME', True),
    ConvSpec('coarse/conv/conv2d_3', 384, 384, 3, 1, 'SAME', True),
# ... 222 lines not shown
        if not grad_weight >= 0:
            raise ValueError(f'grad_weight {grad_weight!r}: the weight of the gradient-matching term is a number >= 0')
        if objective != 'silog' and grad_weight > 0:
            raise ValueError(f"objective {objective!r} with grad_weight {grad_weight!r}: the gradient-matching term is defined "
                             f'on log differences and belongs to the silog objective')
        self.grad_weight = grad_weight
        self.valid_range = check_valid_range(valid_range)
        self._loss = msdn_loss_launches(objective, berhu_fraction, grad_weight, self.valid_range is not None)
        vars(self).update(self._loss.attrs)
        self.keep_dense_grads = keep_dense_grads or reducer is not None or batchsize > 64 or clip_norm is not None
        self.bf16s = precision == 'bf16s'
        self._c4_32_fresh = False
        if self.bf16s:
            precision = 'bf16'
        self.precision = precision
        self.B = B = batchsize
        self.device = torch.device(device)
        self.global_step = global_step
        self.reducer = reducer
        dev = self.device
        self.overlap = overlap
        self._shared_desc = {}
        self._prep = {}
        self._alone = ()
        self._deferred = None
        self._m_sharded = False
        self.dense_exchange = None
        if reducer is not None:
            want = os.environ.get('A3D_DP_DENSE', 'scatter')
            if want not in ('scatter', 'allreduce'):
                raise ValueError(f'A3D_DP_DENSE={want!r}: scatter or allreduce')
            scatter = want == 'scatter' and clip_norm is None
            self.dense_exchange = 'reduce_scatter' if (scatter and reducer.inplace_ok(dev)) else 'all_reduce'
            if scatter and self.dense_exchange == 'all_reduce':
                print('MSDNReplica: in-place reduce-scatter failed its self-check on this backend; the dense bucket is '
                      'all-reduced instead', flush=True)
        self._dense_pieces = None
        self._poison = None
        self._poison_seen = []
        self.fuse_pool = precision == 'fp32'
        self.side = None
        if self.overlap and dev.type == 'cuda':
            handle = ctypes.c_void_p()
            with torch.cuda.device(dev):
                ops.check(_lib.load().a3d_stream_create(1, ctypes.byref(handle)), 'a3d_stream_create')
            self.side = torch.cuda.ExternalStream(handle.value, device=dev)
            self._side_handle = handle.value
        shapes = collections.OrderedDict()
        for c in MSDN_CONVS:
            shapes[c.name + '/kernel'] = (c.k, c.k, c.cin, c.cout)
            shapes[c.name + '/bias'] = (c.cout,)
        for n, i, o in MSDN_DENSES:
            shapes[n + '/kernel'] = (i, o)
            shapes[n + '/bias'] = (o,)
        self.shapes = shapes
        self.groups = collections.OrderedDict()
        self.group_of = {}
        for gname, (lr, scopes) in MSDN_OPTIMIZERS.items():
            gshapes = collections.OrderedDict((n, s) for n, s in shapes.items()
                                              if any(n.startswith(sc + '/') for sc in scopes))
            world = reducer.world_size if (reducer is not None and gname == 'CoarseDense') else 1
            self.groups[gname] = ParamGroup(gname, lr if lr_scale == 1.0 else lr * lr_scale, gshapes, dev, beta2=beta2,
                                            multiple=world, optimizer=optimizer, momentum=momentum, clip_norm=clip_norm)
            for n in gshapes:
                self.group_of[n] = gname
        if params is None:
            rng = np.random.default_rng(seed)
            params = {n: (glorot_uniform(rng, s) if n.endswith('/kernel') else np.zeros(s, np.float32))
                      for n, s in shapes.items()}
        self.load_params(params)

        def buf(*shape):
            return torch.empty(shape, device=dev)

        def abuf(*shape):
            return torch.empty(shape, device=dev, dtype=torch.bfloat16 if self.bf16s else torch.float32)
        self.conv = {c.name: c for c in MSDN_CONVS}
        self.x = buf(B, NET_H, NET_W, 3)
        self.t = buf(B, OUT_H, OUT_W, 1)
        self.c0 = None if self.bf16s else buf(B, 55, 74, 96)
        self.c1 = None if self.bf16s else buf(B, 27, 37, 256)
        self.p0 = abuf(B, 27, 37, 96); self.p1 = abuf(B, 13, 18, 256)
        self.c2 = abuf(B, 13, 18, 384); self.c3 = abuf(B, 13, 18, 384); self.c4 = abuf(B, 6, 8, 256)
        self.drop = buf(B, 4096)
        self.coarse = buf(B, OUT_H, OUT_W, 1)
        self.f1 = buf(B, 110, 148, 63) if not self.bf16s else None
        self.cat = abuf(B, OUT_H, OUT_W, 64)
        self.f2 = buf(B, OUT_H, OUT_W, 64)
        self.fine = buf(B, OUT_H, OUT_W, 1)
        width, name = self._loss.width, self._loss.name
        self.loss_out_c = buf(width); self.loss_out_f = buf(width)
        self.loss_coarse = self.loss_out_c[:1]; self.loss_fine = self.loss_out_f[:1]
        if width >= 2:
            self.loss_pair_c = self.loss_out_c[:2]; self.loss_pair_f = self.loss_out_f[:2]
        if width == 4:
            setattr(self, f'loss_{name}_c', self.loss_out_c); setattr(self, f'loss_{name}_f', self.loss_out_f)
        self.a0 = torch.empty((B, 27, 37, 96), dtype=torch.uint8, device=dev)
        self.a1 = torch.empty((B, 13, 18, 256), dtype=torch.uint8, device=dev)
        self.af1 = torch.empty((B, OUT_H, OUT_W, 63), dtype=torch.uint8, device=dev)
        self.pooled_fwd = None
        self.ws_c = self._loss.ws(B, dev); self.ws_f = self._loss.ws(B, dev)
        self.t_one = buf(B, 1, 1, 1) if valid_range is not None else None
        self.dz1 = buf(B, OUT_H * OUT_W); self.dz0 = buf(B, 4096)
        self.dc4 = abuf(B, 6, 8, 256); self.dc3 = abuf(B, 13, 18, 384); self.dc2 = abuf(B, 13, 18, 384)
        self.dp1 = abuf(B, 13, 18, 256); self.dc1 = abuf(B, 27, 37, 256)
        self.dp0 = abuf(B, 27, 37, 96); self.dc0 = None
        self.dfine = buf(B, OUT_H, OUT_W, 1); self.df2 = abuf(B, OUT_H, OUT_W, 64)
        self.dcat = abuf(B, OUT_H, OUT_W, 64); self.df1 = None
        if self.bf16s:
            self.c4_32 = buf(B, 6, 8, 256)
            self.dz0_16 = torch.empty((B, 4096), device=dev, dtype=torch.bfloat16)
            self.dense_bf16_x = B <= 64
            if not self.dense_bf16_x:
                self.dc4_32 = buf(B, 6, 8, 256)
            NP = (OUT_H * OUT_W + 7) // 8 * 8
            self.w1pad = torch.zeros((4096, NP), device=dev, dtype=torch.bfloat16)
            self.b1pad = torch.zeros((1, NP), device=dev)
            self.drop16 = torch.empty((B, 4096), device=dev, dtype=torch.bfloat16)
            self.dz1_16 = torch.zeros((B, NP), device=dev, dtype=torch.bfloat16)
        def D(*a):
            return ops.conv_desc(*a, precision=precision)
        self.d = {
            'coarse/conv/conv2d_0': D(B, NET_H, NET_W, 3, 96, 11, 11, 4, 'VALID'),
            'coarse/conv/conv2d_1': D(B, 27, 37, 96, 256, 5, 5, 1, 'SAME'),
            'coarse/conv/conv2d_2': D(B, 13, 18, 256, 384, 3, 3, 1, 'SAME'),
            'coarse/conv/conv2d_3': D(B, 13, 18, 384, 384, 3, 3, 1, 'SAME'),
            'coarse/conv/conv2d_4': D(B, 13, 18, 384, 256, 3, 3, 2, 'VALID'),
            'fine/first/conv2d': D(B, NET_H, NET_W, 3, 63, 9, 9, 2, 'VALID'),
            'fine/second/conv2d': D(B, OUT_H, OUT_W, 64, 64, 5, 5, 1, 'SAME'),
            'fine/third': D(B, OUT_H, OUT_W, 64, 1, 5, 5, 1, 'SAME'),
        }
        self.d_wino = {}
        if precision == 'fp32' and dev.type == 'cuda':
            for n in self.WINO_LAYERS:
                d = self.d[n]
                if d.n * -(-d.ho // 2) * -(-d.wo // 2) >= self.WINO_MIN_TILES:
                    e = self.d_wino[n] = ConvDesc.from_buffer_copy(d)
                    e.precision = ops.PREC['fp32w']
        self.wino_grad = set()
        if precision == 'fp32' and dev.type == 'cuda':
            for n in self.WINO_GRAD_LAYERS:
                d = self.d[n]
                if d.n * -(-d.ho // 2) * -(-d.wo // 2) >= self.WINO_GRAD_MIN_TILES:
                    self.wino_grad.add(n)
        self.wino1d_bwd_d, self.wino1d_bwd_f = set(), set()
        if precision == 'fp32' and dev.type == 'cuda':
            for n in self.WINO1D_LAYERS:
                d = self.d[n]
                rows = d.n * d.h * -(-d.w // 4)
                if rows >= self.WINO1D_BWD_D_MIN_ROWS:
                    self.wino1d_bwd_d.add(n)
                if rows >= self.WINO1D_BWD_F_MIN_ROWS:
                    self.wino1d_bwd_f.add(n)
        self.d_few = {}
        if dev.type == 'cuda':
            few_prec = 'bf16' if self.bf16s else 'fp32'
            for n, dd in (('coarse/conv/conv2d_0', ops.conv_desc(B, NET_H, NET_W, 3, 96, 11, 11, 4, 'VALID', precision=few_prec)),
                          ('fine/first/conv2d', ops.conv_desc(B, NET_H, NET_W, 3, 63, 9, 9, 2, 'VALID', precision=few_prec))):
                if ops.conv2d_bwd_filter_pooled_supported(dd):
                    self.d_few[n] = dd
        self.store = {}
        self.wcopy = {}
        if self.bf16s:
            X, W, Y = ops.STORE_X, ops.STORE_W, ops.STORE_Y
            for n in ('coarse/conv/conv2d_1', 'coarse/conv/conv2d_2', 'coarse/conv/conv2d_3', 'coarse/conv/conv2d_4'):
                self.store[n] = {'fwd': X | W | Y, 'bwd_d': X | W | Y, 'bwd_f': X | Y}
            self.store['coarse/conv/conv2d_0'] = {'bwd_f': Y}
            self.d['fine/first/conv2d'].precision = ops.PREC['fp32']
            self.store['fine/second/conv2d'] = {'fwd': X | W, 'bwd_d': W | X | Y, 'bwd_f': X | Y}
            self.x4 = torch.empty((B, NET_H, NET_W, 4), device=dev, dtype=torch.bfloat16)
            self.w0_4 = torch.zeros((11, 11, 4, 96), device=dev)
            self.d0_4 = ops.with_storage(ops.conv_desc(B, NET_H, NET_W, 4, 96, 11, 11, 4, 'VALID', ldy=96, precision='bf16'),
                                         X | Y)
            self.w4 = torch.zeros((9, 9, 4, 63), device=dev)
            self.d4 = ops.with_storage(ops.conv_desc(B, NET_H, NET_W, 4, 63, 9, 9, 2, 'VALID', ldy=64, precision='bf16'),
                                       X | Y)
            for n in list(self.store) + ['coarse/dense/dense_0']:
                if n == 'coarse/dense/dense_0' or self.store[n].get('fwd', 0) & W:
                    self.wcopy[n] = torch.empty(self.shapes[n + '/kernel'], device=dev, dtype=torch.bfloat16)
            self.refresh_weight_copies()

    def __del__(self):
        handle, self._side_handle = getattr(self, '_side_handle', None), None
        if handle:
            try:
                torch.cuda.synchronize(self.device)
                ops.drop_workspace(handle)
                _lib.load().a3d_stream_destroy(handle)
            except Exception:
                pass

    SHARE_CU = ('fine/first/conv2d', 'fine/second/conv2d')
    WINO_LAYERS = ('coarse/conv/conv2d_2', 'coarse/conv/conv2d_3')
    WINO_MIN_TILES = 504
    WINO_GRAD_LAYERS = WINO_LAYERS
    WINO_GRAD_MIN_TILES = 504
    WINO_BWD_CHAIN = True

    WINO1D_LAYERS = ('coarse/conv/conv2d_1',)
    WINO1D_BWD_D_MIN_ROWS = 2160
    WINO1D_BWD_F_MIN_ROWS = 2160

    def _desc(self, name, which):
        d = self.d[name]
        bits = self.store.get(name, {}).get(which, 0)
        if which == 'fwd' and self.side is not None and name in self.SHARE_CU and name not in self._alone:
            key = (name, bits)
            if key not in self._shared_desc:
                e = ops.with_storage(d, bits)
                e.hints = ops.HINT_SHARE_CU
                self._shared_desc[key] = e
            return self._shared_desc[key]
        return ops.with_storage(d, bits) if bits else d

    def _w(self, name, which='fwd'):
        if name in self.wcopy and (name not in self.store or self.store[name][which] & ops.STORE_W):
            return self.wcopy[name]
        return self._v(name + '/kernel')

    def _prepared(self, key, desc, w, which='fwd'):
        if self.device.type != 'cuda':
            return desc, w
        pf = self._prep.get(key)
        if pf is None:
            pf = self._prep[key] = ops.PreparedFilter(desc, self.device, which)
            pf.source = w
            if pf.ok:
                pf.refresh(w)
        return (pf.desc_prepared, pf.buf) if pf.ok else (desc, w)

    def _refresh_prepared(self):
        for pf in self._prep.values():
            if pf.ok:
                pf.refresh(pf.source)

    def refresh_weight_copies(self):
        for n, c in self.wcopy.items():
            ops.cast_bf16(self._v(n + '/kernel'), c)
        if self.bf16s:
            self.w4[:, :, :3, :] = self._v('fine/first/conv2d/kernel')
            self.w0_4[:, :, :3, :] = self._v('coarse/conv/conv2d_0/kernel')
            n = 'coarse/dense/dense_1'
            ops.cast_rows(self._v(n + '/kernel'), self.w1pad)
            ops.cast_rows(self._v(n + '/bias').view(1, -1), self.b1pad)

    def _weights_moved(self, *groups):
        if not all(g.frozen() for g in groups):
            if self.wcopy:
                self.refresh_weight_copies()
            self._refresh_prepared()

    def settle(self):
        if self._deferred is not None:
            works, group, scale = self._deferred
            self._deferred = None
            if works and isinstance(works[0], tuple):
                self._poll_poison()
                for work, a, b in works:
                    self.reducer.wait(work)
                    group.apply_slice(a, b, scale, poisoned=self._poison)
                group.advance()
                self._m_sharded = True
                self._watch_poison()
                return
            for work in works:
                self.reducer.wait(work)
            group.apply(scale)
            self._weights_moved(group)

    def _dense_buckets(self):
        if self._dense_pieces is None:
            gd = self.groups['CoarseDense']
            q = self.reducer.world_size * ParamGroup.ALIGN
            c = -(-gd.offsets['coarse/dense/dense_1/kernel'][0] // q) * q
            third = -(-(c // 3) // q) * q
            self._dense_pieces = ([(c, gd.count)], [(0, third), (third, 2 * third), (2 * third, c)])
        return self._dense_pieces

    def _my_slice(self, a, b):
        n = (b - a) // self.reducer.world_size
        return a + self.reducer.rank * n, a + (self.reducer.rank + 1) * n

    def _watch_poison(self):
        red = self.reducer
        work = red.any(self._poison)
        red.wait(work)
        if not hasattr(self, '_poison_ring'):
            ring = torch.empty(4, dtype=torch.int32)
            self._poison_ring = (ring.pin_memory() if self.device.type == 'cuda' else ring, 0)
        ring, nxt = self._poison_ring
        self._poison_ring = (ring, (nxt + 1) % 4)
        host = ring[nxt:nxt + 1]
        host.copy_(self._poison, non_blocking=True)
        ev = None
        if self.device.type == 'cuda':
            ev = torch.cuda.Event()
            ev.record()
        self._poison_seen.append((ev, host))

    def _poll_poison(self, block=False):
        while self._poison_seen and (block or len(self._poison_seen) >= 2):
            ev, host = self._poison_seen.pop(0)
            if ev is not None:
                ev.synchronize()
            if int(host.item()):
                self._resync()

    def _resync(self):
        gd = self.groups['CoarseDense']
        early, late = self._dense_buckets()
        for a, b in early + late:
            for buf in (gd.var, gd.v, gd.m):
                self.reducer.all_gather(buf[a:b])
        self._poison.zero_()
        self._poison_seen = []
        self._m_sharded = False

    def gather_state(self):
        self.settle()
        if self._m_sharded:
            self._poll_poison(block=True)
        if self._m_sharded:
            gd = self.groups['CoarseDense']
            early, late = self._dense_buckets()
            for a, b in early + late:
                self.reducer.all_gather(gd.m[a:b])
            self._m_sharded = False

    def load_params(self, params):
        self.settle()
        for n, shp in self.shapes.items():
            g = self.groups[self.group_of[n]]
            a = np.asarray(params[n], np.float32)
            assert a.shape == tuple(shp), (n, a.shape, shp)
            g.view(g.var, n).copy_(torch.from_numpy(np.ascontiguousarray(a)))
        if getattr(self, 'wcopy', None):
            self.refresh_weight_copies()
        if getattr(self, '_prep', None):
            self._refresh_prepared()

    def _v(self, name):
        g = self.groups[self.group_of[name]]
        return g.view(g.var, name)

    def _g(self, name):
        g = self.groups[self.group_of[name]]
        return g.view(g.grad, name)

    def var(self, name):
        self.settle()
        return self._v(name)

    def grad(self, name):
        self.settle()
# ... 151 lines not shown
        win = out[:, :2 * ph, :2 * pw, :].reshape(full.shape[0], ph, 2, pw, 2, c)
        a = arg.long()
        for pos in range(4):
            win[:, :, pos >> 1, :, pos & 1, :] = torch.where(a == pos, pooled[..., :c], torch.zeros_like(pooled[..., :c]))
        return out

    def _conv_pool(self, name, x, y_pooled, argmax=None):
        d, w = self._fwd_operands(name)
        ops.conv2d_pool_fwd(d, x, w, self._v(name + '/bias'), y_pooled, 'relu', argmax)

    def _fine_first_image_form(self, argmax=None):
        d, w = self._prepared(('fine/first/image', 0, 0, 0), self.d4, self.w4)
        ops.conv2d_pool_fwd(d, self.x4, w, self._v('fine/first/conv2d/bias'), self.cat, 'relu', argmax)

    def forward(self, images, depths, keep_mask, join=True, phase=None, warp=None):
        if depths is None:
            pass
        elif self.valid_range is not None:
            lo, hi = self.valid_range
            if warp is not None:
                ops.warp_bilinear_pair_valid(images, self.x, depths, self.t, warp, lo, hi)
            elif images.shape[:3] == depths.shape[:3]:
                ops.resize_bilinear_tf1_pair_valid(images, self.x, depths, self.t, lo, hi)
            else:
                ops.resize_bilinear_tf1(images, self.x)
                ops.resize_bilinear_tf1_valid(depths, self.t, lo, hi, scratch=self.t_one)
        elif warp is not None:
            ops.warp_bilinear_pair(images, self.x, depths, self.t, warp)
        elif images.shape[:3] == depths.shape[:3]:
            ops.resize_bilinear_tf1_pair(images, self.x, depths, self.t)
        else:
            ops.resize_bilinear_tf1(images, self.x)
            ops.resize_bilinear_tf1(depths, self.t)
        B = self.B
        self.dropout_on = keep_mask is not None
        self._alone = ('fine/second/conv2d',) if phase == 2 else ()
        if self.bf16s:
            ops.pad_channels_bf16(self.x, self.x4)
        fused = self.fuse_pool and phase in (1, 2, 3)
        self.pooled_fwd = phase if fused else None
        lean_fine = fused
        if fused:
            train = phase == 1
            self._conv_pool('coarse/conv/conv2d_0', self.x, self.p0, self.a0 if train else None)
            self._conv_pool('coarse/conv/conv2d_1', self.p0, self.p1, self.a1 if train else None)
        elif self.bf16s:
            d, w = self._prepared(('conv2d_0/image', 0, 0, 0), self.d0_4, self.w0_4)
            ops.conv2d_pool_fwd(d, self.x4, w, self._v('coarse/conv/conv2d_0/bias'), self.p0, 'relu', self.a0)
            self._conv_pool('coarse/conv/conv2d_1', self.p0, self.p1, self.a1)
        else:
            self._conv('coarse/conv/conv2d_0', self.x, self.c0)
            ops.maxpool2x2_fwd(self.c0, self.p0)
            self._conv('coarse/conv/conv2d_1', self.p0, self.c1)
            ops.maxpool2x2_fwd(self.c1, self.p1)
        def fine_first():
            with self._beside():
                if lean_fine:
                    self._conv_pool('fine/first/conv2d', self.x, self.cat, self.af1 if phase == 2 else None)
                elif self.bf16s:
                    self._fine_first_image_form(None if phase in (1, 3) else self.af1)
                else:
                    self._conv('fine/first/conv2d', self.x, self.f1)
        self._conv('coarse/conv/conv2d_2', self.p1, self.c2)
        self._conv('coarse/conv/conv2d_3', self.c2, self.c3)
        fine_first()
        self._c4_32_fresh = False
        if self.bf16s and self.dense_bf16_x and phase == 1:
            n4 = 'coarse/conv/conv2d_4'
            ops.conv2d_fwd(self._desc(n4, 'fwd'), self.c3, self._w(n4), self._v(n4 + '/bias'), self.c4, 'relu',
                           out2=ops.second_output(self.c4_32.view(-1, 256)))
            self._c4_32_fresh = True
        else:
            self._conv('coarse/conv/conv2d_4', self.c3, self.c4)
        if not self._sharded_in_flight():
            self.settle()
        w, b = self._kb('coarse/dense/dense_0')
        if self.bf16s and self.dense_bf16_x:
            ops.dense_fwd_ex(self.c4.view(B, -1), self.wcopy['coarse/dense/dense_0'], b, self.drop, 'relu',
                             drop_keep=keep_mask, precision='bf16', storage=ops.STORE_W | ops.STORE_X,
                             out2=ops.second_output(self.drop16))
        elif self.bf16s:
            ops.cast_bf16(self.c4, self.c4_32)
            ops.dense_fwd_ex(self.c4_32.view(B, -1), self.wcopy['coarse/dense/dense_0'], b, self.drop, 'relu',
                             drop_keep=keep_mask, precision='bf16', storage=ops.STORE_W)
        else:
            ops.dense_fwd(self.c4.view(B, -1), w, b, self.drop, 'relu', drop_keep=keep_mask)
        w, b = self._kb('coarse/dense/dense_1')
        cat_done = self.bf16s and self.dense_bf16_x
        if cat_done:
            ops.dense_fwd_ex(self.drop16, self.w1pad, self.b1pad, self.coarse.view(B, -1), None, precision='bf16',
                             storage=ops.STORE_W | ops.STORE_X, n=self.w1pad.shape[1],
                             out2=ops.second_output(self.cat, cols=OUT_H * OUT_W, step=64, offset=63, ld=OUT_H * OUT_W))
        else:
            ops.dense_fwd(self.drop, w, b, self.coarse.view(B, -1))
        with self._beside():
            if cat_done:
                pass
            elif lean_fine or self.bf16s:
                ops.copy_channel(self.coarse, 0, self.cat, 63)
            else:
                ops.maxpool2x2_fwd(self.f1, self.cat, extra=self.coarse)
            self._conv('fine/second/conv2d', self.cat, self.f2)
            self._conv('fine/third', self.f2, self.fine)
            if depths is not None:
                self._loss_fwd(self.fine, self.loss_out_f, self.ws_f)
        if depths is not None:
            self._loss_fwd(self.coarse, self.loss_out_c, self.ws_c)
        if join:
            self._join()

    def predict(self, images, n=None):
        B = self.B
        n = images.shape[0] if n is None else int(n)
        check_rows('predict', n, B, f'a batch of {images.shape[0]} images', images.shape[0])
        ops.resize_bilinear_tf1(images[:n], self.x[:n])
        if n < B:
            self.x[n:].zero_()
        self.forward(images, None, None, join=True, phase=3)
        return self.coarse.view(B, OUT_H, OUT_W), self.fine.view(B, OUT_H, OUT_W)

    def _loss_fwd(self, out, loss, ws):
        self._loss.fwd(out, self.t, loss, ws)

    def _loss_bwd(self, out, ws, dout, dout16=None):
        self._loss.bwd(out, self.t, ws, dout, dout16)

    def _sharded_in_flight(self):
        d = self._deferred
        return d is not None and bool(d[0]) and isinstance(d[0][0], tuple)

    def _fused_dense_adam(self):
        return not self.keep_dense_grads and self.groups['CoarseDense'].frozen()

    def _fused_dense_momentum(self):
        return not self.keep_dense_grads and self.optimizer == 'momentum'

    def _bwd_data(self, name, dz, dx, relu_mask=None):
        d, w = self._desc(name, 'bwd_d'), self._w(name, 'bwd_d')
        if name in self.d_wino:
            d, w = self._prepared((name, 'bwd_d', 'fp32w'), self.d_wino[name], w, 'bwd_d')
        if name in self.wino1d_bwd_d:
            d, w = self._prepared((name, 'bwd_d', 'wino1d'), d, w, 'bwd_d_wino1d')
            ops.conv2d_bwd_data_wino1d(d, dz, w, dx, relu_mask=relu_mask)
            return
        ops.conv2d_bwd_data(d, dz, w, dx, relu_mask=relu_mask)

    def _wino_chain(self, name):
        return self.WINO_BWD_CHAIN and name in self.d_wino and name in self.wino_grad

    def _bwd_wino(self, name, x, dz, dx, relu_mask=None, pool=None):
        d, w = self._prepared((name, 'bwd_d', 'fp32w'), self.d_wino[name], self._w(name, 'bwd_d'), 'bwd_d')
        ops.conv2d_bwd_wino(d, x, dz, w, self._g(name + '/kernel'), self._g(name + '/bias'), dx, relu_mask=relu_mask, pool=pool)

    def _bwd_filter(self, name, x, dz):
        if name in self.d:
            call = ops.conv2d_bwd_filter_wino if name in self.wino_grad else ops.conv2d_bwd_filter
            if name in self.wino1d_bwd_f:
                call = ops.conv2d_bwd_filter_wino1d
            call(self._desc(name, 'bwd_f'), x, dz, self._g(name + '/kernel'), self._g(name + '/bias'))
        elif self._fused_dense_adam():
            g = self.groups[self.group_of[name + '/kernel']]
            kw = [g.view(buf, name + '/kernel') for buf in (g.var, g.m, g.v)]
            kb = [g.view(buf, name + '/bias') for buf in (g.var, g.m, g.v)]
            ops.dense_bwd_filter_adam_tf1(x, dz, *kw, *kb, g.lr, g.beta1, g.beta2, float(g.beta1_power),
                                          float(g.beta2_power), 1.0, precision='bf16' if self.bf16s else 'fp32')
        elif self._fused_dense_momentum():
            g = self.groups[self.group_of[name + '/kernel']]
            slots = [g.view(buf, name + which) for which in ('/kernel', '/bias') for buf in (g.var, g.m)]
            ops.dense_bwd_filter_momentum(x, dz, *slots, g.lr, g.momentum, 1.0)
        else:
            ops.dense_bwd_filter(x, dz, self._g(name + '/kernel'), self._g(name + '/bias'))

    def backward_coarse(self, after_dense=None, after_conv2=None, after_dense1=None):
        B = self.B
        bf16_x = self.bf16s and self.dense_bf16_x
        self._loss_bwd(self.coarse, self.ws_c, self.dz1.view(B, OUT_H, OUT_W, 1),
                       dout16=self.dz1_16 if bf16_x else None)
        self.settle()
        n = 'coarse/dense/dense_1'
        late = self._fused_dense_momentum()
        if not late:
            self._bwd_filter(n, self.drop, self.dz1)
        if after_dense1 is not None:
            after_dense1()
        if bf16_x:
            ops.dense_bwd_data_ex(self.dz1_16, self.w1pad, self.dz0, mask=self.drop, scale=2.0 if self.dropout_on else 1.0,
                                  precision='bf16', storage=ops.STORE_W | ops.STORE_Y,
                                  out2=ops.second_output(self.dz0_16))
        else:
            ops.dense_bwd_data(self.dz1, self._v(n + '/kernel'), self.dz0, mask=self.drop, scale=2.0 if self.dropout_on else 1.0)
        if late:
            self._bwd_filter(n, self.drop, self.dz1)
        n = 'coarse/dense/dense_0'
        if bf16_x and not self._c4_32_fresh:
            ops.cast_bf16(self.c4, self.c4_32)
        flat = (self.c4_32 if self.bf16s else self.c4).view(B, -1)
        if not late:
            self._bwd_filter(n, flat, self.dz0)
        if bf16_x:
            ops.dense_bwd_data_ex(self.dz0_16, self.wcopy[n], self.dc4.view(B, -1), mask=self.c4.view(B, -1), scale=1.0,
                                  precision='bf16', storage=ops.STORE_W | ops.STORE_X | ops.STORE_Y)
        elif self.bf16s:
            ops.dense_bwd_data_ex(self.dz0, self.wcopy[n], self.dc4_32.view(B, -1), mask=flat, scale=1.0, precision='bf16',
                                  storage=ops.STORE_W)
            ops.cast_bf16(self.dc4_32, self.dc4)
        else:
            ops.dense_bwd_data(self.dz0, self._v(n + '/kernel'), self.dc4.view(B, -1), mask=flat, scale=1.0)
        if late:
            self._bwd_filter(n, flat, self.dz0)
        if after_dense is not None:
            after_dense()
        n = 'coarse/conv/conv2d_4'
        self._bwd_filter(n, self.c3, self.dc4)
        self._bwd_data(n, self.dc4, self.dc3, relu_mask=self.c3)
        self._join()
        dw = self._bwd_filter
        pooled = self.pooled_fwd == 1 or self.bf16s
        n = 'coarse/conv/conv2d_3'
        if self._wino_chain(n):
            self._bwd_wino(n, self.c2, self.dc3, self.dc2, relu_mask=self.c2)
        else:
            dw(n, self.c2, self.dc3)
            self._bwd_data(n, self.dc3, self.dc2, relu_mask=self.c2)
        n = 'coarse/conv/conv2d_2'
        if self._wino_chain(n):
            self._bwd_wino(n, self.p1, self.dc2, self.dc1 if pooled else self.dp1, pool=(self.a1, self.p1) if pooled else None)
            if after_conv2 is not None:
                after_conv2()
            if not pooled:
                ops.maxpool2x2_bwd(self.c1, self.dp1, self.dc1, relu_mask=True)
        else:
            dw(n, self.p1, self.dc2)
            if after_conv2 is not None:
                after_conv2()
            self._bwd_data(n, self.dc2, self.dp1)
            if pooled:
                ops.maxpool2x2_bwd_idx(self.a1, self.p1, self.dp1, self.dc1, relu_mask=True)
            else:
                ops.maxpool2x2_bwd(self.c1, self.dp1, self.dc1, relu_mask=True)
        n = 'coarse/conv/conv2d_1'
        dw(n, self.p0, self.dc1)
        self._bwd_data(n, self.dc1, self.dp0)
        n = 'coarse/conv/conv2d_0'
        if pooled and n in self.d_few:
            ops.conv2d_bwd_filter_pooled(self.d_few[n], self.x, self.dp0, self.p0, self.a0, self._g(n + '/kernel'),
                                         self._g(n + '/bias'))
            return
        if self.dc0 is None:
            self.dc0 = torch.empty((self.B, 55, 74, 96), device=self.device, dtype=self.dp0.dtype)
        if pooled:
            ops.maxpool2x2_bwd_idx(self.a0, self.p0, self.dp0, self.dc0, relu_mask=True)
        else:
            ops.maxpool2x2_bwd(self.c0, self.dp0, self.dc0, relu_mask=True)
        dw(n, self.x, self.dc0)

    def backward_fine(self):
        self._join()
        self._loss_bwd(self.fine, self.ws_f, self.dfine)
        n = 'fine/third'
        if ops.conv2d_bwd_both_supported(self.d[n]):
            ops.conv2d_bwd_both(self.d[n], self.f2, self.dfine, self._v(n + '/kernel'), self._g(n + '/kernel'),
                                self._g(n + '/bias'), self.df2, relu_mask=True)
        else:
            assert not self.bf16s, 'bf16 storage: df2 is a bf16 tensor only the fused backward writes'
            self._bwd_filter(n, self.f2, self.dfine)
            self._bwd_data(n, self.dfine, self.df2, relu_mask=self.f2)
        n = 'fine/second/conv2d'
        self._bwd_filter(n, self.cat, self.df2)
        self._bwd_data(n, self.df2, self.dcat)
        n = 'fine/first/conv2d'
        if (self.pooled_fwd == 2 or self.bf16s) and n in self.d_few:
            ops.conv2d_bwd_filter_pooled(self.d_few[n], self.x, self.dcat, self.cat, self.af1, self._g(n + '/kernel'),
                                         self._g(n + '/bias'))
            return
        if self.df1 is None:
            self.df1 = torch.empty((self.B, 110, 148, 63), device=self.device)
        if self.pooled_fwd == 2 or self.bf16s:
            ops.maxpool2x2_bwd_idx(self.af1, self.cat, self.dcat, self.df1, relu_mask=True)
        else:
            ops.maxpool2x2_bwd(self.f1, self.dcat, self.df1, relu_mask=True)
        self._bwd_filter(n, self.x, self.df1)

    def step(self, images, depths, keep_mask, warp=None):
        if keep_mask is not None and keep_mask.dtype != torch.uint8:
            keep_mask = keep_mask.to(torch.uint8)
        phase = phase_of(self.global_step, self.B)
        self.forward(images, depths, keep_mask, join=False, phase=phase, warp=warp)
        red = self.reducer
        scale = 1.0 / red.world_size if red is not None else 1.0
        if phase == 1:
            gc, gd = self.groups['CoarseConv'], self.groups['CoarseDense']
            if red is None:
                fused = self._fused_dense_adam() or self._fused_dense_momentum()
                self.backward_coarse()
                gc.apply(scale)
                if fused:
                    gd.advance()
                else:
                    gd.apply(scale)
                self._weights_moved(gc, gd)
            else:
                handle, tail = [], []
                cut = gc.offsets['coarse/conv/conv2d_2/kernel'][0]
                if gd.frozen() and self.dense_exchange == 'reduce_scatter':
                    early, late = self._dense_buckets()
                    if self._poison is None:
                        self._poison = torch.zeros(1, dtype=torch.int32, device=self.device)

                    def scatter(pieces):
                        for a, b in pieces:
                            work, _ = red.reduce_scatter(gd.grad[a:b])
                            handle.append((work,) + self._my_slice(a, b))
                    after_dense1, after_dense = (lambda: scatter(early)), (lambda: scatter(late))
                else:
                    d1 = gd.offsets['coarse/dense/dense_1/kernel'][0]
                    third = -(-(d1 // 3) // ParamGroup.ALIGN) * ParamGroup.ALIGN
                    pieces0 = [(0, third), (third, 2 * third), (2 * third, d1)]
                    after_dense1 = lambda: handle.append(red.start(gd.grad[d1:]))
                    after_dense = lambda: handle.extend(red.start(gd.grad[a:b]) for a, b in pieces0)
                self.backward_coarse(after_dense1=after_dense1, after_dense=after_dense,
                                     after_conv2=lambda: tail.append(red.start(gc.grad[cut:], urgent=True)))
                head = red.start(gc.grad[:cut], urgent=True)
                red.wait(tail[0])
                red.wait(head)
                gc.apply(scale)
                self._weights_moved(gc)
                self._deferred = (handle, gd, scale)
        elif phase == 2:
            ga, gb = self.groups['FineA'], self.groups['FineB']
            self.backward_fine()
            if red is not None:
                red.start(ga.grad)
                red.start(gb.grad)
                red.finish()
            ga.apply(scale)
            gb.apply(scale)
            self._weights_moved(ga, gb)
        self._join()
        self.global_step += 1
        return {'coarse_loss': self.loss_coarse, 'fine_loss': self.loss_fine, 'phase': phase}


DCNF_IMG_H, DCNF_IMG_W = 240, 320
DCNF_PATCH, DCNF_SP = 100, 40
DCNF_PREFIX = 'unary/unary_layers/'
DCNF_CONVS = [('conv2d', 3, 64, 11), ('conv2d_1', 64, 256, 5), ('conv2d_2', 256, 256, 3),
              ('conv2d_3', 256, 256, 3), ('conv2d_4', 256, 256, 3)]
DCNF_POOL_AFTER = ('conv2d', 'conv2d_1', 'conv2d_4')
DCNF_DENSES = [('dense', 12544, 128, 'relu'), ('dense_1', 128, 16, 'sigmoid'), ('dense_2', 16, 1, None)]


class DCNFUnary:

    def __init__(self, batchsize, device='cuda', params=None, seed=3000, precision='fp32'):
        self.B = batchsize
        self.device = dev = torch.device(device)
        self.rows, _ = ops.same_pad(DCNF_IMG_H, DCNF_PATCH, DCNF_SP)
        self.cols, _ = ops.same_pad(DCNF_IMG_W, DCNF_PATCH, DCNF_SP)
        self.P = P = batchsize * self.rows * self.cols
        shapes = collections.OrderedDict()
        for n, ci, co, k in DCNF_CONVS:
            shapes[DCNF_PREFIX + n + '/kernel'] = (k, k, ci, co)
            shapes[DCNF_PREFIX + n + '/bias'] = (co,)
        for n, i, o, _ in DCNF_DENSES:
            shapes[DCNF_PREFIX + n + '/kernel'] = (i, o)
            shapes[DCNF_PREFIX + n + '/bias'] = (o,)
        self.shapes = shapes
        self.group = ParamGroup('unary', 0.1, shapes, dev, slots=False)
        if params is None:
            rng = np.random.default_rng(seed)
            params = {n: (glorot_uniform(rng, s) if n.endswith('/kernel') else np.zeros(s, np.float32))
                      for n, s in shapes.items()}
        for n, s in shapes.items():
            self.group.view(self.group.var, n).copy_(torch.from_numpy(np.ascontiguousarray(params[n], np.float32)))

        def buf(*shape):
            return torch.empty(shape, device=dev)
        self.resized = buf(batchsize, DCNF_IMG_H, DCNF_IMG_W, 3)
        self.act = collections.OrderedDict()
        self.dact = {}
        self.desc = {}
        self.fuse_pool = precision == 'fp32'
        self.argmax, self.conv_hw = {}, {}
        self.few_pooled = False
        self.act['x'] = buf(P, DCNF_PATCH, DCNF_PATCH, 3)
        h = DCNF_PATCH
        for n, ci, co, k in DCNF_CONVS:
            self.desc[n] = ops.conv_desc(P, h, h, ci, co, k, k, 1, 'VALID', precision=precision)
            h = h - k + 1
            self.conv_hw[n] = h
            if not (self.fuse_pool and n in DCNF_POOL_AFTER):
                self.act[n] = buf(P, h, h, co)
            if n in DCNF_POOL_AFTER:
                h //= 2
                self.act[n + '/pool'] = buf(P, h, h, co)
                if self.fuse_pool:
                    self.argmax[n] = torch.empty((P, h, h, co), dtype=torch.uint8, device=dev)
        for n, i, o, _ in DCNF_DENSES:
            self.act[n] = buf(P, o)
        self.z = self.act['dense_2']
        self.few_pooled = (self.fuse_pool and dev.type == 'cuda'
                           and ops.conv2d_bwd_filter_pooled_supported(self.desc['conv2d']))

    def var(self, name):
        return self.group.view(self.group.var, DCNF_PREFIX + name)

    def grad(self, name):
        return self.group.view(self.group.grad, DCNF_PREFIX + name)

    def forward(self, images, record_argmax=True):
        ops.resize_bilinear_tf1(images, self.resized)
        return self.forward_resized(record_argmax)

    def forward_resized(self, record_argmax=True):
        ops.extract_patches(self.resized, DCNF_PATCH, DCNF_SP, self.act['x'])
        t = self._forward_convs(self.act['x'], record_argmax)
        self._forward_denses(t.view(self.P, -1))
        return self.z.view(self.B, self.rows * self.cols, 1)

    def _forward_convs(self, t, record_argmax):
        for n, _, _, _ in DCNF_CONVS:
            if self.fuse_pool and n in DCNF_POOL_AFTER:
# ... 711 lines not shown
```

ann3depth_amd/ops.py:

```python
import collections
import ctypes
import math

import torch

from . import _lib
from ._lib import ConvDesc, check

ACT = {None: 0, 'relu': 1, 'sigmoid': 2}
PREC = {'fp32': 0, 'f32': 0, 'bf16x3': 1, 'bf16': 2, 'fp32w': 3}


def _ptr(t):
    return None if t is None else ctypes.c_void_p(t.data_ptr())


def _stream():
    return ctypes.c_void_p(torch.cuda.current_stream().cuda_stream)


class Workspace:

    def __init__(self):
        self.buf = None
# ... 26 lines not shown


def same_pad(in_size, k, stride):
    out = -(-in_size // stride)
    pad = max((out - 1) * stride + k - in_size, 0)
    return out, pad // 2


STORE_X, STORE_W, STORE_Y = 1, 2, 4


HINT_SHARE_CU = 1
HINT_W_PREPARED = 2


class PreparedFilter:

    def __init__(self, desc, device, which='fwd'):
        lib = _lib.load()
        self.stem = {'fwd': 'a3d_conv2d_fwd', 'bwd_d': 'a3dw_conv2d_bwd_data', 'bwd_d_wino1d': 'a3dl_conv2d_bwd_data'}[which]
        nbytes = getattr(lib, self.stem + '_prepared_filter_bytes')(ctypes.byref(desc))
        self.ok = nbytes > 0
        self.desc = desc
        if self.ok:
            self.buf = torch.empty(nbytes, dtype=torch.uint8, device=device)
            self.desc_prepared = ConvDesc.from_buffer_copy(desc)
            self.desc_prepared.hints = desc.hints | HINT_W_PREPARED

    def refresh(self, w):
        name = self.stem + '_prepare_filter'
        check(getattr(_lib.load(), name)(ctypes.byref(self.desc), _ptr(w), _ptr(self.buf), self.buf.numel(), _stream()), name)


def conv_desc(n, h, w, c, k, r, s, stride, padding, ldx=None, ldy=None, precision='fp32', storage=0, hints=0):
    padding = padding.upper()
    if padding == 'SAME':
        ho, pt = same_pad(h, r, stride)
        wo, pl = same_pad(w, s, stride)
    elif padding == 'VALID':
        ho, pt = (h - r) // stride + 1, 0
        wo, pl = (w - s) // stride + 1, 0
    else:
        raise ValueError(padding)
    return ConvDesc(n=n, h=h, w=w, c=c, k=k, r=r, s=s, stride=stride, pad_t=pt, pad_l=pl, ho=ho, wo=wo,
                    ldx=ldx or c, ldy=ldy or k, precision=PREC[precision], storage=storage, hints=hints)


def second_output(t, cols=None, step=1, offset=0, ld=None):
    if t is None:
        return None
    ld = t.shape[-1] if ld is None else ld
    o = _lib.SecondOutput(t.data_ptr(), ld, step, offset, int(t.dtype == torch.bfloat16), ld if cols is None else cols)
    o._keep = t
    return o


def _o2(out2):
    return None if out2 is None else ctypes.byref(out2)


def conv2d_fwd(d, x, w, bias, y, act=None, out2=None):
    lib = _lib.load()
    ws, n = _ws().get(lib.a3d_conv2d_fwd_ws_bytes(ctypes.byref(d)), x.device)
    if out2 is not None:
        check(lib.a3d_conv2d_fwd_ex2(ctypes.byref(d), _ptr(x), _ptr(w), _ptr(bias), _ptr(y), ACT[act], _o2(out2), ws, n, _stream()),
              'a3d_conv2d_fwd_ex2')
        return y
    check(lib.a3d_conv2d_fwd(ctypes.byref(d), _ptr(x), _ptr(w), _ptr(bias), _ptr(y), ACT[act], ws, n, _stream()),
          'a3d_conv2d_fwd')
    return y


def conv2d_pool_fwd(d, x, w, bias, y_pooled, act='relu', argmax=None):
    lib = _lib.load()
    ws, n = _ws().get(lib.a3d_conv2d_fwd_ws_bytes(ctypes.byref(d)), x.device)
    check(lib.a3d_conv2d_pool_fwd(ctypes.byref(d), _ptr(x), _ptr(w), _ptr(bias), _ptr(y_pooled), y_pooled.shape[-1],
                                  _ptr(argmax), ACT[act], ws, n, _stream()), 'a3d_conv2d_pool_fwd')
    return y_pooled


def maxpool2x2_bwd_idx(argmax, y_pooled, dy, dx, relu_mask=True):
    n, h, w, c = dx.shape
    if y_pooled.dtype == torch.bfloat16 and dx.dtype == torch.bfloat16:
        assert dy.dtype == torch.bfloat16
        name = 'a3d_maxpool2x2_bwd_idx_bf16s'
    elif y_pooled.dtype == torch.bfloat16:
        assert dy.dtype == torch.bfloat16 and dx.dtype == torch.float32
        name = 'a3d_maxpool2x2_bwd_idx_bf16'
    else:
        name = 'a3d_maxpool2x2_bwd_idx'
    check(getattr(_lib.load(), name)(n, h, w, c, _ptr(argmax), _ptr(y_pooled), y_pooled.shape[-1], _ptr(dy), dy.shape[-1],
                                     _ptr(dx), int(relu_mask), _stream()), name)
    return dx


def copy_channel(src, c_src, dst, c_dst):
    npix = src.numel() // src.shape[-1]
    assert dst.numel() // dst.shape[-1] == npix
    fn = _lib.load().a3d_copy_channel_bf16 if dst.dtype == torch.bfloat16 else _lib.load().a3d_copy_channel
    check(fn(npix, _ptr(src), src.shape[-1], c_src, _ptr(dst), dst.shape[-1], c_dst, _stream()), 'a3d_copy_channel')
    return dst


def conv2d_bwd_data(d, dz, w, dx, relu_mask=None):
    lib = _lib.load()
    ws, n = _ws().get(lib.a3d_conv2d_bwd_data_ws_bytes(ctypes.byref(d)), dz.device)
    check(lib.a3d_conv2d_bwd_data(ctypes.byref(d), _ptr(dz), _ptr(w), _ptr(dx), _ptr(relu_mask), ws, n, _stream()),
          'a3d_conv2d_bwd_data')
    return dx


def conv2d_bwd_filter(d, x, dz, dw, db=None):
    lib = _lib.load()
    ws, n = _ws().get(lib.a3d_conv2d_bwd_filter_ws_bytes(ctypes.byref(d)), x.device)
    check(lib.a3d_conv2d_bwd_filter(ctypes.byref(d), _ptr(x), _ptr(dz), _ptr(dw), _ptr(db), ws, n, _stream()),
          'a3d_conv2d_bwd_filter')
    return dw, db


def conv2d_bwd_filter_wino(d, x, dz, dw, db=None):
    lib = _lib.load()
    ws, n = _ws().get(lib.a3dwg_conv2d_bwd_filter_ws_bytes(ctypes.byref(d)), x.device)
    check(lib.a3dwg_conv2d_bwd_filter(ctypes.byref(d), _ptr(x), _ptr(dz), _ptr(dw), _ptr(db), ws, n, _stream()),
          'a3dwg_conv2d_bwd_filter')
    return dw, db


def conv2d_bwd_data_wino1d(d, dz, w, dx, relu_mask=None):
    lib = _lib.load()
    ws, n = _ws().get(lib.a3dl_conv2d_bwd_data_ws_bytes(ctypes.byref(d)), dz.device)
    check(lib.a3dl_conv2d_bwd_data(ctypes.byref(d), _ptr(dz), _ptr(w), _ptr(dx), _ptr(relu_mask), ws, n, _stream()),
          'a3dl_conv2d_bwd_data')
    return dx


def conv2d_bwd_filter_wino1d(d, x, dz, dw, db=None):
    lib = _lib.load()
    ws, n = _ws().get(lib.a3dl_conv2d_bwd_filter_ws_bytes(ctypes.byref(d)), x.device)
    check(lib.a3dl_conv2d_bwd_filter(ctypes.byref(d), _ptr(x), _ptr(dz), _ptr(dw), _ptr(db), ws, n, _stream()),
          'a3dl_conv2d_bwd_filter')
    return dw, db


def conv2d_bwd_wino(d, x, dz, w, dw, db, dx, relu_mask=None, pool=None):
    lib = _lib.load()
    prepared = int(bool(d.hints & HINT_W_PREPARED))
    ws, n = _ws().get(lib.a3dwb_conv2d_bwd_ws_bytes(ctypes.byref(d), prepared, int(pool is not None)), x.device)
    pp = None
    if pool is not None:
        argmax, y = pool
        pp = ctypes.byref(_lib.WinoBwdPool(_ptr(argmax), _ptr(y), y.shape[-1], dx.shape[1], dx.shape[2]))
    check(lib.a3dwb_conv2d_bwd(ctypes.byref(d), _ptr(x), _ptr(dz), _ptr(w), _ptr(dw), _ptr(db), _ptr(dx), _ptr(relu_mask), pp,
                               ws, n, _stream()), 'a3dwb_conv2d_bwd')
    return dw, db, dx


def conv2d_bwd_filter_pooled_supported(d):
    return _lib.load().a3d_conv2d_bwd_filter_pooled_ws_bytes(ctypes.byref(d)) > 0


def conv2d_bwd_filter_pooled(d, x, dpool, pooled, argmax, dw, db=None):
    lib = _lib.load()
    ws, n = _ws().get(lib.a3d_conv2d_bwd_filter_pooled_ws_bytes(ctypes.byref(d)), x.device)
    assert pooled is None or (pooled.dtype == dpool.dtype and pooled.shape[-1] == dpool.shape[-1])
    check(lib.a3d_conv2d_bwd_filter_pooled(ctypes.byref(d), _ptr(x), _ptr(dpool), dpool.shape[-1], _ptr(pooled), _ptr(argmax),
                                           argmax.shape[-1], int(dpool.dtype == torch.bfloat16), _ptr(dw), _ptr(db), ws, n,
                                           _stream()), 'a3d_conv2d_bwd_filter_pooled')
    return dw, db


_BOTH_STATE = {}


def conv2d_bwd_both_supported(d):
    return bool(_lib.load().a3d_conv2d_bwd_both_supported(ctypes.byref(d)))


def conv2d_bwd_both(d, x, dz, w, dw, db, dx, relu_mask=True):
    lib = _lib.load()
    key = (torch.cuda.current_stream().cuda_stream, x.device)
    state = _BOTH_STATE.get(key)
    if state is None:
        state = _BOTH_STATE[key] = torch.zeros(64, dtype=torch.int32, device=x.device)
    ws, n = _ws().get(lib.a3d_conv2d_bwd_both_ws_bytes(ctypes.byref(d)), x.device)
    check(lib.a3d_conv2d_bwd_both(ctypes.byref(d), _ptr(x), _ptr(dz), _ptr(w), _ptr(dw), _ptr(db), _ptr(dx), dx.shape[-1],
                                  int(dx.dtype == torch.bfloat16), int(bool(relu_mask)), _ptr(state), ws, n, _stream()),
          'a3d_conv2d_bwd_both')
    return dw, db, dx


def dense_fwd(x, w, bias, y, act=None, drop_keep=None):
    m, k = x.shape
    n = w.shape[1]
    lib = _lib.load()
    ws, nb = _ws().get(lib.a3d_dense_fwd_ws_bytes(m, k, n), x.device)
    check(lib.a3d_dense_fwd(m, k, n, _ptr(x), _ptr(w), _ptr(bias), _ptr(y), ACT[act], _ptr(drop_keep), ws, nb,
                            _stream()), 'a3d_dense_fwd')
    return y


def dense_bwd_data(dz, w, dx, mask=None, scale=1.0, mask_act='relu'):
    m, n = dz.shape
    k = w.shape[0]
    lib = _lib.load()
    ws, nb = _ws().get(lib.a3d_dense_bwd_data_ws_bytes(m, k, n), dz.device)
    check(lib.a3d_dense_bwd_data(m, k, n, _ptr(dz), _ptr(w), _ptr(dx), _ptr(mask), ACT[mask_act], scale, ws, nb,
                                 _stream()),
          'a3d_dense_bwd_data')
    return dx


def dense_bwd_filter(x, dz, dw, db=None):
    m, k = x.shape
    n = dz.shape[1]
    lib = _lib.load()
    ws, nb = _ws().get(lib.a3d_dense_bwd_filter_ws_bytes(m, k, n), x.device)
    check(lib.a3d_dense_bwd_filter(m, k, n, _ptr(x), _ptr(dz), _ptr(dw), _ptr(db), ws, nb, _stream()),
          'a3d_dense_bwd_filter')
    return dw, db


def maxpool2x2_fwd(x, y, extra=None):
    n, h, w, c = x.shape
    check(_lib.load().a3d_maxpool2x2_fwd(n, h, w, c, _ptr(x), _ptr(y), y.shape[-1], _ptr(extra), _stream()),
          'a3d_maxpool2x2_fwd')
    return y


def maxpool2x2_bwd(x, dy, dx, relu_mask=True):
    n, h, w, c = x.shape
    check(_lib.load().a3d_maxpool2x2_bwd(n, h, w, c, _ptr(x), _ptr(dy), dy.shape[-1], _ptr(dx), int(relu_mask),
                                         _stream()), 'a3d_maxpool2x2_bwd')
    return dx


def _pair_args(x0, y0, x1=None, y1=None):
    def one(x, y):
        if x is None:
            return 0, None, 0, 0, 0, None
        return x.shape[3], _ptr(x), int(x.dtype == torch.uint8), y.shape[1], y.shape[2], _ptr(y)
    return tuple(x0.shape[:3]) + one(x0, y0) + one(x1, y1)


def resize_bilinear_tf1(x, y):
    n, h, w, c = x.shape
    if x.dtype == torch.uint8:
        check(_lib.load().a3d_resize_bilinear_tf1_ex(*_pair_args(x, y), _stream()), 'a3d_resize_bilinear_tf1_ex')
        return y
    check(_lib.load().a3d_resize_bilinear_tf1(n, h, w, c, _ptr(x), y.shape[1], y.shape[2], _ptr(y), _stream()),
          'a3d_resize_bilinear_tf1')
    return y


def resize_bilinear_tf1_pair(x0, y0, x1, y1):
    n, h, w, c0 = x0.shape
    assert x1.shape[:3] == (n, h, w)
    if x0.dtype == torch.uint8 or x1.dtype == torch.uint8:
        check(_lib.load().a3d_resize_bilinear_tf1_ex(*_pair_args(x0, y0, x1, y1), _stream()), 'a3d_resize_bilinear_tf1_ex')
        return
    check(_lib.load().a3d_resize_bilinear_tf1_pair(n, h, w, c0, _ptr(x0), y0.shape[1], y0.shape[2], _ptr(y0), x1.shape[3],
                                                   _ptr(x1), y1.shape[1], y1.shape[2], _ptr(y1), _stream()),
          'a3d_resize_bilinear_tf1_pair')


WARP_STRIDE = 12


def _check_pair(who, x0, y0, x1, y1, table):
    if x0.dim() != 4 or y0.dim() != 4 or y0.shape[0] != x0.shape[0] or y0.shape[3] != x0.shape[3]:
        raise ValueError(f'{who}: {tuple(x0.shape)} -> {tuple(y0.shape)}')
    n, h, w, c0 = x0.shape
    if (x1 is None) != (y1 is None):
        raise ValueError(f'{who}: x1 and y1 go together')
    if x1 is not None and (x1.dim() != 4 or tuple(x1.shape[:3]) != (n, h, w) or y1.dim() != 4
                           or y1.shape[0] != n or y1.shape[3] != x1.shape[3]):
        raise ValueError(f'{who}: second tensor {tuple(x1.shape)} -> {tuple(y1.shape)} beside '
                         f'{tuple(x0.shape)}')
    if table is not None and (tuple(table.shape) != (n, WARP_STRIDE) or table.dtype != torch.float32):
        raise ValueError(f'{who}: table {tuple(table.shape)} {table.dtype}, want [{n}, {WARP_STRIDE}] float32')
    for name, t, dtypes in (('x0', x0, (torch.float32, torch.uint8)), ('y0', y0, (torch.float32,)),
                            ('x1', x1, (torch.float32, torch.uint8)), ('y1', y1, (torch.float32,)),
                            ('table', table, (torch.float32,))):
        if t is None:
            continue
        if t.dtype not in dtypes:
            raise ValueError(f'{who}: {name} is {t.dtype}')
        if not t.is_cuda or t.device != x0.device:
            raise ValueError(f'{who}: {name} is on {t.device}, x0 on {x0.device}')
        if not t.is_contiguous():
            raise ValueError(f'{who}: {name} is not contiguous')
    return n, h, w, c0


def warp_bilinear_pair(x0, y0, x1, y1, table):
    if table is None:
        raise ValueError('warp_bilinear_pair: no table')
    _check_pair('warp_bilinear_pair', x0, y0, x1, y1, table)
    check(_lib.load().a3d_warp_bilinear_pair(*_pair_args(x0, y0, x1, y1), _ptr(table), _stream()), 'a3d_warp_bilinear_pair')


def _valid_range(who, x1, min_depth, max_depth):
    if x1 is None:
        raise ValueError(f'{who}: the depth map x1 is required')
    lo, hi = float(min_depth), float(max_depth)
    if not lo <= hi:
        raise ValueError(f'{who}: min_depth {lo}, max_depth {hi}')
# ... 1032 lines not shown
```

Baseline: 13800.

## Fuse Winograd 1-D conv backward data and filter into one chained call

Adds a combined Winograd 1-D backward entry point that runs the x, dz and dz-transposed input transforms in a single kernel, then the filter-gradient and data-gradient GEMMs, and finally one kernel that both reduces the dW split-K slabs and applies the output transform with ReLU masking for dx. It is enabled for coarse conv2d_1 and fine/second/conv2d, and adds narrower 64-wide plane GEMM tile variants for these shapes. The aim is to cut kernel launches and redundant reads of dz across the separate backward-filter and backward-data paths. The trade-off is extra workspace, and the smaller tiles may lower per-block efficiency.

After: 13870, median of 6. About the same (+0.5%).

```diff
diff --git a/ann3depth_amd/_lib.py b/ann3depth_amd/_lib.py
--- a/ann3depth_amd/_lib.py
+++ b/ann3depth_amd/_lib.py
@@ -202,6 +202,11 @@
     'a3dl_conv2d_bwd_data_prepare_filter': (c_int, [_D, _P, _P, c_size_t, _P]),
 }
 
+WINO1D_BWD_SIGNATURES = {
+    'a3dlb_conv2d_bwd_ws_bytes': (c_size_t, [_D, c_int]),
+    'a3dlb_conv2d_bwd': (c_int, [_D, _P, _P, _P, _P, _P, _P, _P, _P, c_size_t, _P]),
+}
+
 OPTIM_SIGNATURES = {
     'a3do_momentum_apply': (c_int, [c_size_t, _P, _P, _P, c_float, c_float, c_float, _P]),
     'a3do_dense_bwd_filter_momentum': (c_int, [c_int, c_int, c_int, _P, _P, _P, _P, _P, _P, c_float, c_float, c_float, _P]),
@@ -270,6 +275,7 @@
     Surface('a3da_', 'a3d_align.h', ALIGN_SIGNATURES),
     Surface('a3di_', 'a3d_ssi.h', SSI_SIGNATURES),
     Surface('a3dl_', 'a3d_wino1d.h', WINO1D_SIGNATURES),
+    Surface('a3dlb_', 'a3d_wino1d_bwd.h', WINO1D_BWD_SIGNATURES),
     Surface('a3do_', 'a3d_optim.h', OPTIM_SIGNATURES),
     Surface('a3dn_', 'a3d_clip.h', CLIP_SIGNATURES),
 )
diff --git a/ann3depth_amd/csrc/a3d_internal.h b/ann3depth_amd/csrc/a3d_internal.h
--- a/ann3depth_amd/csrc/a3d_internal.h
+++ b/ann3depth_amd/csrc/a3d_internal.h
@@ -121,9 +121,9 @@
 struct PlaneBatch;
 constexpr int kBM = 128, kBN = 128, kWavesM = 4, kNWaves = 8, kBK = 32;
 constexpr int kBlockSlots = 512, kCUs = 256, kMinKTiles = 5;
-void plane_tiles(IgemmParams& p, int splits);
+void plane_tiles(IgemmParams& p, int splits, int bm = kBM, int bn = kBN);
 int plane_gemm(int mode, int bn, const IgemmParams& p, const PlaneBatch& bt, unsigned blocks, int planes, const char* what, hipStream_t st);
-int plane_splits(int planes, int M, int N, size_t pixels, bool larger_on_tie, const char* tuning);
+int plane_splits(int planes, int M, int N, size_t pixels, bool larger_on_tie, const char* tuning, int bm = kBM, int bn = kBN);
 
 struct WinoGeom {
   int oh, ow, th, tw;
@@ -178,13 +178,14 @@
   int R, tw;
   size_t Px, Pz;
   int Cp, Kp, splits;
+  int bm, bn;
   size_t v_bytes, z_bytes;
   size_t slab_bytes, bias_bytes;
 };
 int wino1d_bwd_blocks(long tiles, long nk);
-int wino1d_grad_splits(int M, int N, size_t pixels);
-Wino1dGeom wino1d_geom(const a3d_conv_desc* d);
-Wino1dGradGeom wino1d_grad_geom(const a3d_conv_desc* d);
+int wino1d_grad_splits(int M, int N, size_t pixels, int bm = kBM, int bn = kBN);
+Wino1dGeom wino1d_geom(const a3d_conv_desc* d, bool narrow = false);
+Wino1dGradGeom wino1d_grad_geom(const a3d_conv_desc* d, bool narrow = false);
 bool wino1d_applicable(const a3d_conv_desc* d);
 int wino1d_filter(const a3d_conv_desc* d, const float* w, float* U, hipStream_t st);
 int wino1d_input(const float* src, float* V, size_t rows, int W, int c, int ld, int off, int tw, int Cp, hipStream_t st);
@@ -195,6 +196,10 @@
 a3d_timing_record wino1d_grad_record(const a3d_conv_desc* d, const Wino1dGradGeom& g);
 int wino1d_gemm(IgemmParams& p, const Wino1dGeom& g, float* sk, hipStream_t st);
 int wino1d_grad_gemm(IgemmParams& p, const Wino1dGradGeom& g, hipStream_t st);
+int wino1d_bwd_transforms(const a3d_conv_desc* d, const Wino1dGeom& g, const Wino1dGradGeom& gg, const float* x, const float* dz, float* Vx,
+                          float* Vdz, float* Z, hipStream_t st);
+int wino1d_bwd_finish(const a3d_conv_desc* d, const Wino1dGeom& g, const Wino1dGradGeom& gg, const float* slabs, const float* bparts, float* dw,
+                      float* db, const float* M, float* dx, const float* mask, hipStream_t st);
 
 struct Carve {
   uintptr_t at;
diff --git a/ann3depth_amd/csrc/igemm_host.hip b/ann3depth_amd/csrc/igemm_host.hip
--- a/ann3depth_amd/csrc/igemm_host.hip
+++ b/ann3depth_amd/csrc/igemm_host.hip
@@ -5,6 +5,7 @@
 #include "../../include/a3d_wino_grad.h"
 #include "../../include/a3d_wino_bwd.h"
 #include "../../include/a3d_wino1d.h"
+#include "../../include/a3d_wino1d_bwd.h"
 #include "a3d_internal.h"
 #include "igemm.h"
 #include "igemm_cfgs.h"
@@ -1034,6 +1035,48 @@
   return wino1d_filter(d, w, static_cast<float*>(prepared), static_cast<hipStream_t>(stream));
 }
 
+static bool wino1d_bwd_narrow() { return tune_int("A3D_WINO1D_WIDE", 0) == 0; }
+
+size_t a3dlb_conv2d_bwd_ws_bytes(const a3d_conv_desc* d, int w_prepared) {
+  if (!wino1d_takes(d)) return std::max(a3d_conv2d_bwd_filter_ws_bytes(d), a3d_conv2d_bwd_data_ws_bytes(d));
+  const bool narrow = wino1d_bwd_narrow();
+  Carve c{0};
+  carve_product(c, wino1d_geom(d, narrow), w_prepared != 0);
+  carve_grad(c, wino1d_grad_geom(d, narrow));
+  return c.at;
+}
+
+int a3dlb_conv2d_bwd(const a3d_conv_desc* d, const float* x, const float* dz, const float* w_or_U, float* dw, float* db, float* dx,
+                     const float* relu_mask, void* ws, size_t ws_bytes, void* stream) {
+  if (!wino1d_takes(d)) {
+    const int rc = a3d_conv2d_bwd_filter(d, x, dz, dw, db, ws, ws_bytes, stream);
+    return rc != A3D_OK ? rc : a3d_conv2d_bwd_data(d, dz, w_or_U, dx, relu_mask, ws, ws_bytes, stream);
+  }
+  A3D_CHECK_ARG(x && dz && w_or_U && dw && dx, "conv2d_bwd (Winograd 1-D): null tensor");
+  A3D_CHECK_WS(ws, "conv2d_bwd (Winograd 1-D)");
+  const bool prepared = (d->hints & A3D_HINT_W_PREPARED) != 0, narrow = wino1d_bwd_narrow();
+  const Wino1dGeom g = wino1d_geom(d, narrow);
+  const Wino1dGradGeom gg = wino1d_grad_geom(d, narrow);
+  Carve c{reinterpret_cast<uintptr_t>(ws)};
+  const ProductWs ad = carve_product(c, g, prepared);
+  const GradWs af = carve_grad(c, gg);
+  const size_t need = c.at - reinterpret_cast<uintptr_t>(ws);
+  if (!ws || need > ws_bytes) return set_error(A3D_EWORKSPACE, "conv2d_bwd (Winograd 1-D): need %zu workspace bytes", need);
+  hipStream_t st = static_cast<hipStream_t>(stream);
+  const float* U;
+  int rc = transformed_filter("conv2d_bwd (Winograd 1-D)", prepared, w_or_U, ad.U, U, [&](float* u) { return wino1d_filter(d, w_or_U, u, st); });
+  if (rc != A3D_OK) return rc;
+  rc = wino1d_bwd_transforms(d, g, gg, x, dz, af.V, ad.V, af.Z, st);
+  if (rc != A3D_OK) return rc;
+  IgemmParams pf = wino1d_grad_product(d, gg, af.V, af.Z, af.slabs, db ? af.bparts : nullptr);
+  rc = timed_launch(wino1d_grad_record(d, gg), st, [&] { return wino1d_grad_gemm(pf, gg, st); });
+  if (rc != A3D_OK) return rc;
+  IgemmParams pd = wino1d_product(d, g, ad.V, U, ad.M);
+  rc = timed_launch(wino1d_record(g), st, [&] { return wino1d_gemm(pd, g, ad.sk, st); });
+  if (rc != A3D_OK) return rc;
+  return wino1d_bwd_finish(d, g, gg, af.slabs, af.bparts, dw, db, ad.M, dx, relu_mask, st);
+}
+
 static a3d_conv_desc dense_desc(int m, int k, int n) {
   a3d_conv_desc d{};
   d.n = m; d.h = 1; d.w = 1; d.c = k; d.k = n; d.r = 1; d.s = 1; d.stride = 1; d.ho = 1; d.wo = 1;
diff --git a/ann3depth_amd/csrc/wino.hip b/ann3depth_amd/csrc/wino.hip
--- a/ann3depth_amd/csrc/wino.hip
+++ b/ann3depth_amd/csrc/wino.hip
@@ -162,39 +162,41 @@
   }
 }
 
-template <int MODE, int BN, int WAVES_M, int NWAVES>
+template <int MODE, int BM, int BN, int WAVES_M, int NWAVES>
 __global__ __launch_bounds__(64 * NWAVES, 2 * NWAVES / 4) void plane_gemm_kernel(const IgemmParams p, const PlaneBatch bt) {
-  igemm_body<MODE, kBM, BN, WAVES_M, NWAVES, kBK, 4, 4>(plane_params(p, bt, blockIdx.y), gridDim.x, blockIdx.x);
-}
-
-template <int MODE, int BN, int WAVES_M, int NWAVES>
+  igemm_body<MODE, BM, BN, WAVES_M, NWAVES, kBK, 4, 4>(plane_params(p, bt, blockIdx.y), gridDim.x, blockIdx.x);
+}
+
+template <int MODE, int BM, int BN, int WAVES_M, int NWAVES>
 static int plane_gemm_as(const IgemmParams& p, const PlaneBatch& bt, unsigned blocks, int planes, const char* what, hipStream_t st) {
-  using Cfg = IgemmCfg<MODE, kBM, BN, WAVES_M, NWAVES, kBK, 4, 4>;
+  using Cfg = IgemmCfg<MODE, BM, BN, WAVES_M, NWAVES, kBK, 4, 4>;
   static bool attr_done[64] = {};
-  const int rc = raise_lds(reinterpret_cast<const void*>(plane_gemm_kernel<MODE, BN, WAVES_M, NWAVES>), Cfg::LDS_BYTES, attr_done);
+  const int rc = raise_lds(reinterpret_cast<const void*>(plane_gemm_kernel<MODE, BM, BN, WAVES_M, NWAVES>), Cfg::LDS_BYTES, attr_done);
   if (rc != A3D_OK) return rc;
   clear_stale_error();
-  hipLaunchKernelGGL((plane_gemm_kernel<MODE, BN, WAVES_M, NWAVES>), dim3(blocks, (unsigned)planes), dim3(Cfg::NT), Cfg::LDS_BYTES, st, p, bt);
+  hipLaunchKernelGGL((plane_gemm_kernel<MODE, BM, BN, WAVES_M, NWAVES>), dim3(blocks, (unsigned)planes), dim3(Cfg::NT), Cfg::LDS_BYTES, st, p, bt);
   return check_launch(what);
 }
 
 int plane_gemm(int mode, int bn, const IgemmParams& p, const PlaneBatch& bt, unsigned blocks, int planes, const char* what, hipStream_t st) {
-  if (mode == MODE_BWD_F) return plane_gemm_as<MODE_BWD_F, kBN, kWavesM, kNWaves>(p, bt, blocks, planes, what, st);
-  if (bn == 96) return plane_gemm_as<MODE_FWD, 96, 4, 4>(p, bt, blocks, planes, what, st);
-  return plane_gemm_as<MODE_FWD, kBN, kWavesM, kNWaves>(p, bt, blocks, planes, what, st);
-}
-
-void plane_tiles(IgemmParams& p, int splits) {
+  if (mode == MODE_BWD_F && bn == 64) return plane_gemm_as<MODE_BWD_F, 64, 64, 2, 4>(p, bt, blocks, planes, what, st);
+  if (mode == MODE_BWD_F) return plane_gemm_as<MODE_BWD_F, kBM, kBN, kWavesM, kNWaves>(p, bt, blocks, planes, what, st);
+  if (bn == 64) return plane_gemm_as<MODE_FWD, kBM, 64, 4, 8>(p, bt, blocks, planes, what, st);
+  if (bn == 96) return plane_gemm_as<MODE_FWD, kBM, 96, 4, 4>(p, bt, blocks, planes, what, st);
+  return plane_gemm_as<MODE_FWD, kBM, kBN, kWavesM, kNWaves>(p, bt, blocks, planes, what, st);
+}
+
+void plane_tiles(IgemmParams& p, int splits, int bm, int bn) {
   const int nk = (p.K + kBK - 1) / kBK;
   p.splitk = splits;
   p.ktiles_per_split = (nk + splits - 1) / splits;
-  p.tiles_m = (p.M + kBM - 1) / kBM;
-  p.tiles_n = (p.N + kBN - 1) / kBN;
+  p.tiles_m = (p.M + bm - 1) / bm;
+  p.tiles_n = (p.N + bn - 1) / bn;
   p.slab = (size_t)p.M * p.N;
 }
 
-int plane_splits(int planes, int M, int N, size_t pixels, bool larger_on_tie, const char* tuning) {
-  const long blocks1 = (long)planes * ((M + kBM - 1) / kBM) * ((N + kBN - 1) / kBN);
+int plane_splits(int planes, int M, int N, size_t pixels, bool larger_on_tie, const char* tuning, int bm, int bn) {
+  const long blocks1 = (long)planes * ((M + bm - 1) / bm) * ((N + bn - 1) / bn);
   const long nk = (long)((pixels + kBK - 1) / kBK);
   const long smax = std::max(1L, std::min(kBlockSlots / blocks1, nk / kMinKTiles));
   long s = 1, load = (blocks1 + kCUs - 1) / kCUs;
diff --git a/ann3depth_amd/csrc/wino1d.hip b/ann3depth_amd/csrc/wino1d.hip
--- a/ann3depth_amd/csrc/wino1d.hip
+++ b/ann3depth_amd/csrc/wino1d.hip
@@ -39,6 +39,92 @@
   }
 }
 
+template <bool VEC, int COLS>
+__device__ __forceinline__ void w1_load_cols(const float* __restrict__ src, f4 (&d)[COLS], size_t row, int x0, int W, int c, int ld, int cq) {
+#pragma unroll
+  for (int b = 0; b < COLS; ++b) {
+    f4 t = f4(0.f);
+    const int xx = x0 + b;
+    if (xx >= 0 && xx < W) {
+      const float* s = src + (row * W + xx) * (size_t)ld + cq * 4;
+      if (VEC) {
+        t = *reinterpret_cast<const f4*>(s);
+      } else {
+#pragma unroll
+        for (int e = 0; e < 4; ++e)
+          if (cq * 4 + e < c) t[e] = s[e];
+      }
+    }
+    d[b] = t;
+  }
+}
+__device__ __forceinline__ void w1_input_store(const f4 (&d)[8], float* __restrict__ V, size_t P, size_t pix, int Cp, int cq) {
+  f4 v[8];
+  w1_apply<float, 8, 8, kW1BT, false, f4>(d, v);
+#pragma unroll
+  for (int xi = 0; xi < 8; ++xi) *reinterpret_cast<f4*>(V + ((size_t)xi * P + pix) * Cp + cq * 4) = v[xi];
+}
+__device__ __forceinline__ void w1_dz_store(const f4 (&y)[4], float* __restrict__ Z, size_t P, size_t pix, int Kp, int cq) {
+  f4 z[8];
+  w1_apply<float, 4, 8, kW1AT, true, f4>(y, z);
+#pragma unroll
+  for (int xi = 0; xi < 8; ++xi) *reinterpret_cast<f4*>(Z + ((size_t)xi * P + pix) * Kp + cq * 4) = z[xi];
+}
+template <bool VEC>
+__device__ __forceinline__ void w1_output_item(size_t i, const float* __restrict__ M, float* __restrict__ out, const float* __restrict__ mask,
+                                               int w, int ncols, int ld, int tw, int Np, size_t P) {
+  const int cqn = Np / 4;
+  const int cq = (int)(i % cqn);
+  const size_t pix = i / cqn, row = pix / tw;
+  const int x0 = 4 * (int)(pix % tw);
+  f4 m[8], y[4];
+#pragma unroll
+  for (int xi = 0; xi < 8; ++xi) m[xi] = *reinterpret_cast<const f4*>(M + ((size_t)xi * P + pix) * Np + cq * 4);
+  w1_apply<float, 4, 8, kW1AT, false, f4>(m, y);
+#pragma unroll
+  for (int b = 0; b < 4; ++b) {
+    if (x0 + b >= w) continue;
+    const size_t o = (row * w + x0 + b) * (size_t)ld + cq * 4;
+    f4 v = y[b];
+    if (VEC) {
+      if (mask) {
+        const f4 a = *reinterpret_cast<const f4*>(mask + o);
+#pragma unroll
+        for (int e = 0; e < 4; ++e) v[e] = apply_act_grad(v[e], a[e], EPI_RELU, 1.f);
+      }
+      *reinterpret_cast<f4*>(out + o) = v;
+    } else {
+#pragma unroll
+      for (int e = 0; e < 4; ++e)
+        if (cq * 4 + e < ncols) out[o + e] = mask ? apply_act_grad(v[e], mask[o + e], EPI_RELU, 1.f) : v[e];
+    }
+  }
+}
+__device__ __forceinline__ void w1_dw_item(size_t i, const float* __restrict__ slabs, const float* __restrict__ bparts, float* __restrict__ dw,
+                                           float* __restrict__ db, int c, int k, int R, int Cp, int Kp, int splits) {
+  const size_t plane = (size_t)R * Cp * Kp;
+  const int col = (int)(i % k), row = (int)((i / k) % c), r = (int)(i / ((size_t)k * c));
+  const size_t at = ((size_t)r * Cp + row) * Kp + col;
+  double m[8], g[5];
+#pragma unroll
+  for (int xi = 0; xi < 8; ++xi) m[xi] = (double)slabs[(size_t)xi * splits * plane + at];
+  for (int z = 1; z < splits; ++z) {
+    float v[8];
+#pragma unroll
+    for (int xi = 0; xi < 8; ++xi) v[xi] = slabs[((size_t)xi * splits + z) * plane + at];
+#pragma unroll
+    for (int xi = 0; xi < 8; ++xi) m[xi] += (double)v[xi];
+  }
+  w1_apply<double, 8, 5, kW1Gd, true, double>(m, g);
+#pragma unroll
+  for (int s = 0; s < 5; ++s) dw[((size_t)(r * 5 + s) * c + row) * k + col] = (float)g[s];
+  if (db && r == 0 && row == 0) {
+    float s = bparts[col];
+    for (int z = 1; z < splits; ++z) s += bparts[(size_t)z * Kp + col];
+    db[col] = s;
+  }
+}
+
 template <bool VEC>
 __global__ __launch_bounds__(256) void wino1d_input_kernel(const float* __restrict__ src, float* __restrict__ V, int W, int c, int ld, int off,
                                                            int tw, int Cp, size_t P) {
@@ -46,28 +132,10 @@
   const size_t total = P * (size_t)cqn;
   for (size_t i = (size_t)blockIdx.x * 256 + threadIdx.x; i < total; i += (size_t)gridDim.x * 256) {
     const int cq = (int)(i % cqn);
-    const size_t pix = i / cqn, row = pix / tw;
-    const int x0 = 4 * (int)(pix % tw) - off;
-    f4 d[8], v[8];
-#pragma unroll
-    for (int b = 0; b < 8; ++b) {
-      f4 t = f4(0.f);
-      const int xx = x0 + b;
-      if (xx >= 0 && xx < W) {
-        const float* s = src + (row * W + xx) * (size_t)ld + cq * 4;
-        if (VEC) {
-          t = *reinterpret_cast<const f4*>(s);
-        } else {
-#pragma unroll
-          for (int e = 0; e < 4; ++e)
-            if (cq * 4 + e < c) t[e] = s[e];
-        }
-      }
-      d[b] = t;
-    }
-    w1_apply<float, 8, 8, kW1BT, false, f4>(d, v);
-#pragma unroll
-    for (int xi = 0; xi < 8; ++xi) *reinterpret_cast<f4*>(V + ((size_t)xi * P + pix) * Cp + cq * 4) = v[xi];
+    const size_t pix = i / cqn;
+    f4 d[8];
+    w1_load_cols<VEC, 8>(src, d, pix / tw, 4 * (int)(pix % tw) - off, W, c, ld, cq);
+    w1_input_store(d, V, P, pix, Cp, cq);
   }
 }
 
@@ -78,89 +146,26 @@
   const size_t total = P * (size_t)cqn;
   for (size_t i = (size_t)blockIdx.x * 256 + threadIdx.x; i < total; i += (size_t)gridDim.x * 256) {
     const int cq = (int)(i % cqn);
-    const size_t pix = i / cqn, row = pix / tw;
-    const int x0 = 4 * (int)(pix % tw);
-    f4 y[4], z[8];
-#pragma unroll
-    for (int b = 0; b < 4; ++b) {
-      f4 t = f4(0.f);
-      if (x0 + b < wo) {
-        const float* s = dz + (row * wo + x0 + b) * (size_t)ld + cq * 4;
-        if (VEC) {
-          t = *reinterpret_cast<const f4*>(s);
-        } else {
-#pragma unroll
-          for (int e = 0; e < 4; ++e)
-            if (cq * 4 + e < k) t[e] = s[e];
-        }
-      }
-      y[b] = t;
-    }
-    w1_apply<float, 4, 8, kW1AT, true, f4>(y, z);
-#pragma unroll
-    for (int xi = 0; xi < 8; ++xi) *reinterpret_cast<f4*>(Z + ((size_t)xi * P + pix) * Kp + cq * 4) = z[xi];
+    const size_t pix = i / cqn;
+    f4 y[4];
+    w1_load_cols<VEC, 4>(dz, y, pix / tw, 4 * (int)(pix % tw), wo, k, ld, cq);
+    w1_dz_store(y, Z, P, pix, Kp, cq);
   }
 }
 
 template <bool VEC>
 __global__ __launch_bounds__(256) void wino1d_output_kernel(const float* __restrict__ M, float* __restrict__ out, const float* __restrict__ mask,
                                                             int w, int ncols, int ld, int tw, int Np, size_t P) {
-  const int cqn = Np / 4;
-  const size_t total = P * (size_t)cqn;
-  for (size_t i = (size_t)blockIdx.x * 256 + threadIdx.x; i < total; i += (size_t)gridDim.x * 256) {
-    const int cq = (int)(i % cqn);
-    const size_t pix = i / cqn, row = pix / tw;
-    const int x0 = 4 * (int)(pix % tw);
-    f4 m[8], y[4];
-#pragma unroll
-    for (int xi = 0; xi < 8; ++xi) m[xi] = *reinterpret_cast<const f4*>(M + ((size_t)xi * P + pix) * Np + cq * 4);
-    w1_apply<float, 4, 8, kW1AT, false, f4>(m, y);
-#pragma unroll
-    for (int b = 0; b < 4; ++b) {
-      if (x0 + b >= w) continue;
-      const size_t o = (row * w + x0 + b) * (size_t)ld + cq * 4;
-      f4 v = y[b];
-      if (VEC) {
-        if (mask) {
-          const f4 a = *reinterpret_cast<const f4*>(mask + o);
-#pragma unroll
-          for (int e = 0; e < 4; ++e) v[e] = apply_act_grad(v[e], a[e], EPI_RELU, 1.f);
-        }
-        *reinterpret_cast<f4*>(out + o) = v;
-      } else {
-#pragma unroll
-        for (int e = 0; e < 4; ++e)
-          if (cq * 4 + e < ncols) out[o + e] = mask ? apply_act_grad(v[e], mask[o + e], EPI_RELU, 1.f) : v[e];
-      }
-    }
-  }
+  const size_t total = P * (size_t)(Np / 4);
+  for (size_t i = (size_t)blockIdx.x * 256 + threadIdx.x; i < total; i += (size_t)gridDim.x * 256)
+    w1_output_item<VEC>(i, M, out, mask, w, ncols, ld, tw, Np, P);
 }
 
 __global__ __launch_bounds__(256) void wino1d_dw_kernel(const float* __restrict__ slabs, const float* __restrict__ bparts, float* __restrict__ dw,
                                                         float* __restrict__ db, int c, int k, int R, int Cp, int Kp, int splits) {
-  const size_t total = (size_t)R * c * k, plane = (size_t)R * Cp * Kp;
-  for (size_t i = (size_t)blockIdx.x * 256 + threadIdx.x; i < total; i += (size_t)gridDim.x * 256) {
-    const int col = (int)(i % k), row = (int)((i / k) % c), r = (int)(i / ((size_t)k * c));
-    const size_t at = ((size_t)r * Cp + row) * Kp + col;
-    double m[8], g[5];
-#pragma unroll
-    for (int xi = 0; xi < 8; ++xi) m[xi] = (double)slabs[(size_t)xi * splits * plane + at];
-    for (int z = 1; z < splits; ++z) {
-      float v[8];
-#pragma unroll
-      for (int xi = 0; xi < 8; ++xi) v[xi] = slabs[((size_t)xi * splits + z) * plane + at];
-#pragma unroll
-      for (int xi = 0; xi < 8; ++xi) m[xi] += (double)v[xi];
-    }
-    w1_apply<double, 8, 5, kW1Gd, true, double>(m, g);
-#pragma unroll
-    for (int s = 0; s < 5; ++s) dw[((size_t)(r * 5 + s) * c + row) * k + col] = (float)g[s];
-    if (db && r == 0 && row == 0) {
-      float s = bparts[col];
-      for (int z = 1; z < splits; ++z) s += bparts[(size_t)z * Kp + col];
-      db[col] = s;
-    }
-  }
+  const size_t total = (size_t)R * c * k;
+  for (size_t i = (size_t)blockIdx.x * 256 + threadIdx.x; i < total; i += (size_t)gridDim.x * 256)
+    w1_dw_item(i, slabs, bparts, dw, db, c, k, R, Cp, Kp, splits);
 }
 
 constexpr int kPlanes = 8;
@@ -184,9 +189,11 @@
   return (int)b;
 }
 
-int wino1d_grad_splits(int M, int N, size_t pixels) { return plane_splits(kPlanes, M, N, pixels, true, "A3D_WINO1D_GRAD_SPLIT"); }
-
-Wino1dGeom wino1d_geom(const a3d_conv_desc* d) {
+int wino1d_grad_splits(int M, int N, size_t pixels, int bm, int bn) {
+  return plane_splits(kPlanes, M, N, pixels, true, "A3D_WINO1D_GRAD_SPLIT", bm, bn);
+}
+
+Wino1dGeom wino1d_geom(const a3d_conv_desc* d, bool narrow) {
   Wino1dGeom g{};
   g.R = d->r;
   g.tw = (d->w + 3) / 4;
@@ -196,7 +203,7 @@
   g.K = d->k; g.N = d->c;
   g.Kp = (g.K + 3) / 4 * 4;
   g.Np = (g.N + 3) / 4 * 4;
-  g.bn = g.Np <= 96 ? 96 : 128;
+  g.bn = narrow && g.Np <= 64 ? 64 : g.Np <= 96 ? 96 : 128;
   g.tiles_m = (int)((g.Pm + 127) / 128);
   g.tiles_n = (g.Np + g.bn - 1) / g.bn;
   g.nk = (g.R * g.Kp + kBK - 1) / kBK;
@@ -208,7 +215,7 @@
   return g;
 }
 
-Wino1dGradGeom wino1d_grad_geom(const a3d_conv_desc* d) {
+Wino1dGradGeom wino1d_grad_geom(const a3d_conv_desc* d, bool narrow) {
   Wino1dGradGeom g{};
   g.R = d->r;
   g.tw = (d->wo + 3) / 4;
@@ -216,7 +223,8 @@
   g.Pz = (size_t)d->n * d->ho * g.tw;
   g.Cp = (d->c + 3) / 4 * 4;
   g.Kp = (d->k + 3) / 4 * 4;
-  g.splits = wino1d_grad_splits(g.R * g.Cp, g.Kp, g.Pz);
+  g.bm = g.bn = narrow && g.Kp <= 64 ? 64 : kBM;
+  g.splits = wino1d_grad_splits(g.R * g.Cp, g.Kp, g.Pz, g.bm, g.bn);
   g.v_bytes = up256((size_t)kPlanes * g.Px * g.Cp * 4);
   g.z_bytes = up256((size_t)kPlanes * g.Pz * g.Kp * 4);
   g.slab_bytes = up256((size_t)kPlanes * g.splits * g.R * g.Cp * g.Kp * 4);
@@ -281,7 +289,9 @@
   return timing_record(MODE_BWD_D, A3D_PREC_F32, 128, g.bn, 4, g.bn == 96 ? 4 : 8, kBK, 4, 4, 0, (int)(kPlanes * g.Pm), g.N, g.R * g.K);
 }
 a3d_timing_record wino1d_grad_record(const a3d_conv_desc* d, const Wino1dGradGeom& g) {
-  a3d_timing_record r = timing_record(MODE_BWD_F, A3D_PREC_F32, kBM, kBN, kWavesM, kNWaves, kBK, 4, 4, 0, g.R * d->c, d->k, (int)(kPlanes * g.Pz));
+  const bool nar = g.bn == 64;
+  a3d_timing_record r = timing_record(MODE_BWD_F, A3D_PREC_F32, g.bm, g.bn, nar ? 2 : kWavesM, nar ? 4 : kNWaves, kBK, 4, 4, 0, g.R * d->c, d->k,
+                                      (int)(kPlanes * g.Pz));
   r.splitk = g.splits;
   return r;
 }
@@ -299,14 +309,111 @@
   const int rc = plane_gemm(MODE_FWD, g.bn, p, bt, (unsigned)g.blocks, kPlanes, "wino1d_gemm", st);
   if (rc != A3D_OK) return rc;
   const dim3 grid((unsigned)(g.tiles_m * g.tiles_n), (128 * g.bn / 256 + 3) / 4, kPlanes);
-  if (g.bn == 96) hipLaunchKernelGGL((wino1d_fixup_kernel<96, 4, 4>), grid, dim3(256), 0, st, p, (uint32_t)g.blocks, bt);
+  if (g.bn == 64) hipLaunchKernelGGL((wino1d_fixup_kernel<64, 4, 8>), grid, dim3(256), 0, st, p, (uint32_t)g.blocks, bt);
+  else if (g.bn == 96) hipLaunchKernelGGL((wino1d_fixup_kernel<96, 4, 4>), grid, dim3(256), 0, st, p, (uint32_t)g.blocks, bt);
   else hipLaunchKernelGGL((wino1d_fixup_kernel<kBN, kWavesM, kNWaves>), grid, dim3(256), 0, st, p, (uint32_t)g.blocks, bt);
   return check_launch("wino1d_fixup");
 }
 
 int wino1d_grad_gemm(IgemmParams& p, const Wino1dGradGeom& g, hipStream_t st) {
-  plane_tiles(p, g.splits);
-  return plane_gemm(MODE_BWD_F, kBN, p, wino1d_grad_batch(g), (unsigned)(p.tiles_m * p.tiles_n * p.splitk), kPlanes, "wino1d_grad_gemm", st);
-}
-
-}
+  plane_tiles(p, g.splits, g.bm, g.bn);
+  return plane_gemm(MODE_BWD_F, g.bn, p, wino1d_grad_batch(g), (unsigned)(p.tiles_m * p.tiles_n * p.splitk), kPlanes, "wino1d_grad_gemm", st);
+}
+
+
+struct Wino1dBwdXform {
+  const float *x, *dz;
+  float *Vx, *Vdz, *Z;
+  int w, c, ldx, xtw, xoff, Cp;
+  int wo, k, ldy, dtw, doff, Kp;
+  size_t Px, Pd, Pz, x_items;
+};
+template <bool VEC>
+__global__ __launch_bounds__(256) void wino1d_bwd_transform_kernel(const Wino1dBwdXform q) {
+  const int cqx = q.Cp / 4, cqd = q.Kp / 4;
+  const size_t total = q.x_items + q.Pd * (size_t)cqd;
+  for (size_t i = (size_t)blockIdx.x * 256 + threadIdx.x; i < total; i += (size_t)gridDim.x * 256) {
+    f4 d[8];
+    if (i < q.x_items) {
+      const int cq = (int)(i % cqx);
+      const size_t pix = i / cqx;
+      w1_load_cols<VEC, 8>(q.x, d, pix / q.xtw, 4 * (int)(pix % q.xtw) - q.xoff, q.w, q.c, q.ldx, cq);
+      w1_input_store(d, q.Vx, q.Px, pix, q.Cp, cq);
+      continue;
+    }
+    const size_t j = i - q.x_items;
+    const int cq = (int)(j % cqd);
+    const size_t pix = j / cqd, row = pix / q.dtw;
+    const int t = (int)(pix % q.dtw);
+    w1_load_cols<VEC, 8>(q.dz, d, row, 4 * t - q.doff, q.wo, q.k, q.ldy, cq);
+    w1_input_store(d, q.Vdz, q.Pd, pix, q.Kp, cq);
+    if (t < q.xtw) {
+      f4 y[4];
+#pragma unroll
+      for (int b = 0; b < 4; ++b) {
+        y[b] = d[b];
+#pragma unroll
+        for (int o = 1; o <= 4; ++o)
+          if (q.doff == o) y[b] = d[o + b];
+      }
+      w1_dz_store(y, q.Z, q.Pz, row * q.xtw + t, q.Kp, cq);
+    }
+  }
+}
+
+int wino1d_bwd_transforms(const a3d_conv_desc* d, const Wino1dGeom& g, const Wino1dGradGeom& gg, const float* x, const float* dz, float* Vx,
+                          float* Vdz, float* Z, hipStream_t st) {
+  if (gg.tw > g.tw) {
+    int rc = wino1d_input(x, Vx, (size_t)d->n * d->h, d->w, d->c, d->ldx, d->pad_l, gg.tw, gg.Cp, st);
+    if (rc == A3D_OK) rc = wino1d_dz(d, gg, dz, Z, st);
+    return rc != A3D_OK ? rc : wino1d_input(dz, Vdz, (size_t)d->n * d->ho, d->wo, d->k, d->ldy, g.off, g.tw, g.Kp, st);
+  }
+  Wino1dBwdXform q{};
+  q.x = x; q.dz = dz; q.Vx = Vx; q.Vdz = Vdz; q.Z = Z;
+  q.w = d->w; q.c = d->c; q.ldx = d->ldx; q.xtw = gg.tw; q.xoff = d->pad_l; q.Cp = gg.Cp;
+  q.wo = d->wo; q.k = d->k; q.ldy = d->ldy; q.dtw = g.tw; q.doff = g.off; q.Kp = g.Kp;
+  q.Px = gg.Px; q.Pd = g.Pv; q.Pz = gg.Pz; q.x_items = gg.Px * (size_t)(gg.Cp / 4);
+  const bool vec = d->c % 4 == 0 && d->ldx % 4 == 0 && aligned16(x) && d->k % 4 == 0 && d->ldy % 4 == 0 && aligned16(dz);
+  const dim3 grid(grid_for(q.x_items + g.Pv * (size_t)(g.Kp / 4), 256, 1u << 20)), block(256);
+  clear_stale_error();
+  if (vec) hipLaunchKernelGGL(wino1d_bwd_transform_kernel<true>, grid, block, 0, st, q);
+  else hipLaunchKernelGGL(wino1d_bwd_transform_kernel<false>, grid, block, 0, st, q);
+  return check_launch("wino1d_bwd_transform");
+}
+
+struct Wino1dBwdFinish {
+  const float *slabs, *bparts;
+  float *dw, *db;
+  int c, k, R, Cp, Kp, splits;
+  const float* M;
+  float* dx;
+  const float* mask;
+  int w, ncols, ld, tw, Np;
+  size_t P, dw_items;
+};
+template <bool VEC>
+__global__ __launch_bounds__(256) void wino1d_bwd_finish_kernel(const Wino1dBwdFinish q) {
+  const size_t total = q.dw_items + q.P * (size_t)(q.Np / 4);
+  for (size_t i = (size_t)blockIdx.x * 256 + threadIdx.x; i < total; i += (size_t)gridDim.x * 256) {
+    if (i < q.dw_items) w1_dw_item(i, q.slabs, q.bparts, q.dw, q.db, q.c, q.k, q.R, q.Cp, q.Kp, q.splits);
+    else w1_output_item<VEC>(i - q.dw_items, q.M, q.dx, q.mask, q.w, q.ncols, q.ld, q.tw, q.Np, q.P);
+  }
+}
+
+int wino1d_bwd_finish(const a3d_conv_desc* d, const Wino1dGeom& g, const Wino1dGradGeom& gg, const float* slabs, const float* bparts, float* dw,
+                      float* db, const float* M, float* dx, const float* mask, hipStream_t st) {
+  Wino1dBwdFinish q{};
+  q.slabs = slabs; q.bparts = bparts; q.dw = dw; q.db = db;
+  q.c = d->c; q.k = d->k; q.R = gg.R; q.Cp = gg.Cp; q.Kp = gg.Kp; q.splits = gg.splits;
+  q.M = M; q.dx = dx; q.mask = mask;
+  q.w = d->w; q.ncols = g.N; q.ld = d->ldx; q.tw = g.tw; q.Np = g.Np;
+  q.P = g.Pm; q.dw_items = (size_t)gg.R * d->c * d->k;
+  const bool vec = g.N % 4 == 0 && d->ldx % 4 == 0 && aligned16(dx) && aligned16(mask);
+  const dim3 grid(grid_for(q.dw_items + g.Pm * (size_t)(g.Np / 4), 256, 1u << 20)), block(256);
+  clear_stale_error();
+  if (vec) hipLaunchKernelGGL(wino1d_bwd_finish_kernel<true>, grid, block, 0, st, q);
+  else hipLaunchKernelGGL(wino1d_bwd_finish_kernel<false>, grid, block, 0, st, q);
+  return check_launch("wino1d_bwd_finish");
+}
+
+}
diff --git a/ann3depth_amd/models.py b/ann3depth_amd/models.py
--- a/ann3depth_amd/models.py
+++ b/ann3depth_amd/models.py
@@ -398,6 +398,12 @@
                     self.wino1d_bwd_d.add(n)
                 if rows >= self.WINO1D_BWD_F_MIN_ROWS:
                     self.wino1d_bwd_f.add(n)
+        self.wino1d_chain = set()
+        if precision == 'fp32' and dev.type == 'cuda':
+            for n in self.WINO1D_CHAIN_LAYERS:
+                d = self.d[n]
+                if d.n * d.h * -(-d.w // 4) >= self.WINO1D_CHAIN_MIN_ROWS:
+                    self.wino1d_chain.add(n)
         self.d_few = {}
         if dev.type == 'cuda':
             few_prec = 'bf16' if self.bf16s else 'fp32'
@@ -446,6 +452,9 @@
     WINO1D_LAYERS = ('coarse/conv/conv2d_1',)
     WINO1D_BWD_D_MIN_ROWS = 2160
     WINO1D_BWD_F_MIN_ROWS = 2160
+    WINO1D_BWD_CHAIN = True
+    WINO1D_CHAIN_LAYERS = ('fine/second/conv2d',)
+    WINO1D_CHAIN_MIN_ROWS = 8360
 
     def _desc(self, name, which):
         d = self.d[name]
@@ -903,6 +912,14 @@
         d, w = self._prepared((name, 'bwd_d', 'fp32w'), self.d_wino[name], self._w(name, 'bwd_d'), 'bwd_d')
         ops.conv2d_bwd_wino(d, x, dz, w, self._g(name + '/kernel'), self._g(name + '/bias'), dx, relu_mask=relu_mask, pool=pool)
 
+    def _wino1d_chain(self, name):
+        both = self.WINO1D_BWD_CHAIN and name in self.wino1d_bwd_d and name in self.wino1d_bwd_f
+        return both or name in self.wino1d_chain
+
+    def _bwd_wino1d(self, name, x, dz, dx, relu_mask=None):
+        d, w = self._prepared((name, 'bwd_d', 'wino1d'), self._desc(name, 'bwd_d'), self._w(name, 'bwd_d'), 'bwd_d_wino1d')
+        ops.conv2d_bwd_wino1d(d, x, dz, w, self._g(name + '/kernel'), self._g(name + '/bias'), dx, relu_mask=relu_mask)
+
     def _bwd_filter(self, name, x, dz):
         if name in self.d:
             call = ops.conv2d_bwd_filter_wino if name in self.wino_grad else ops.conv2d_bwd_filter
@@ -990,8 +1007,11 @@
             else:
                 ops.maxpool2x2_bwd(self.c1, self.dp1, self.dc1, relu_mask=True)
         n = 'coarse/conv/conv2d_1'
-        dw(n, self.p0, self.dc1)
-        self._bwd_data(n, self.dc1, self.dp0)
+        if self._wino1d_chain(n):
+            self._bwd_wino1d(n, self.p0, self.dc1, self.dp0)
+        else:
+            dw(n, self.p0, self.dc1)
+            self._bwd_data(n, self.dc1, self.dp0)
         n = 'coarse/conv/conv2d_0'
         if pooled and n in self.d_few:
             ops.conv2d_bwd_filter_pooled(self.d_few[n], self.x, self.dp0, self.p0, self.a0, self._g(n + '/kernel'),
@@ -1017,8 +1037,11 @@
             self._bwd_filter(n, self.f2, self.dfine)
             self._bwd_data(n, self.dfine, self.df2, relu_mask=self.f2)
         n = 'fine/second/conv2d'
-        self._bwd_filter(n, self.cat, self.df2)
-        self._bwd_data(n, self.df2, self.dcat)
+        if self._wino1d_chain(n):
+            self._bwd_wino1d(n, self.cat, self.df2, self.dcat)
+        else:
+            self._bwd_filter(n, self.cat, self.df2)
+            self._bwd_data(n, self.df2, self.dcat)
         n = 'fine/first/conv2d'
         if (self.pooled_fwd == 2 or self.bf16s) and n in self.d_few:
             ops.conv2d_bwd_filter_pooled(self.d_few[n], self.x, self.dcat, self.cat, self.af1, self._g(n + '/kernel'),
diff --git a/ann3depth_amd/ops.py b/ann3depth_amd/ops.py
--- a/ann3depth_amd/ops.py
+++ b/ann3depth_amd/ops.py
@@ -202,6 +202,15 @@
         pp = ctypes.byref(_lib.WinoBwdPool(_ptr(argmax), _ptr(y), y.shape[-1], dx.shape[1], dx.shape[2]))
     check(lib.a3dwb_conv2d_bwd(ctypes.byref(d), _ptr(x), _ptr(dz), _ptr(w), _ptr(dw), _ptr(db), _ptr(dx), _ptr(relu_mask), pp,
                                ws, n, _stream()), 'a3dwb_conv2d_bwd')
+    return dw, db, dx
+
+
+def conv2d_bwd_wino1d(d, x, dz, w, dw, db, dx, relu_mask=None):
+    lib = _lib.load()
+    prepared = int(bool(d.hints & HINT_W_PREPARED))
+    ws, n = _ws().get(lib.a3dlb_conv2d_bwd_ws_bytes(ctypes.byref(d), prepared), x.device)
+    check(lib.a3dlb_conv2d_bwd(ctypes.byref(d), _ptr(x), _ptr(dz), _ptr(w), _ptr(dw), _ptr(db), _ptr(dx), _ptr(relu_mask), ws, n,
+                               _stream()), 'a3dlb_conv2d_bwd')
     return dw, db, dx
 
 
diff --git a/include/a3d_wino1d_bwd.h b/include/a3d_wino1d_bwd.h
--- /dev/null
+++ b/include/a3d_wino1d_bwd.h
@@ -0,0 +1,17 @@
+#ifndef A3D_WINO1D_BWD_H_
+#define A3D_WINO1D_BWD_H_
+
+#include "a3d.h"
+
+#ifdef __cplusplus
+extern "C" {
+#endif
+
+size_t a3dlb_conv2d_bwd_ws_bytes(const a3d_conv_desc* d, int w_prepared);
+int a3dlb_conv2d_bwd(const a3d_conv_desc* d, const float* x, const float* dz, const float* w_or_U, float* dw, float* db, float* dx,
+                     const float* relu_mask, void* ws, size_t ws_bytes, void* stream);
+
+#ifdef __cplusplus
+}
+#endif
+#endif
```
